# eglrp/PSBA

Hardware: AMD Instinct MI355X
Metric: M-observations/sec through Jacobian+Schur build+solve (ms/LM-iter in ms_per_step) (higher is better)
Workload: dtype f64; 1 GPU; venice-shaped; n_cams=52, n_pts=64053, n_obs=345364, lm=levmar, TR hand-off disabled, parallelism=points sharded x1

## Files before the change

### include/psba_hip.h

```cpp
#ifndef PSBA_HIP_H
#define PSBA_HIP_H

#ifdef __cplusplus
extern "C" {
#endif

typedef struct psba_ctx *psba_handle;

#define PSBA_OK 0
#define PSBA_NOT_SPD 1
#define PSBA_SINGULAR_V 2
#define PSBA_PCG_MAXIT 4
#define PSBA_E_INVALID (-1)
#define PSBA_E_HIP (-2)
#define PSBA_E_RCCL (-3)
#define PSBA_E_IO (-4)
#define PSBA_E_NOMEM (-5)
#define PSBA_E_STATE (-6)

#define PSBA_ITER_TURN_TO_LM 1
#define PSBA_ITER_TURN_TO_TR 2
#define PSBA_ITER_CONTINUE 3
#define PSBA_ITER_ERR 4
#define PSBA_ITER_DP_NO_CHANGE 5
#define PSBA_ITER_ERR_SMALL_ENOUGH 6
#define PSBA_ITER_PASS 7

#define PSBA_PARAMS_CUR 0
#define PSBA_PARAMS_NEW 1

int psba_create(int device, psba_handle *out);
int psba_destroy(psba_handle h);
const char *psba_last_error(psba_handle h);
const char *psba_version(void);

int psba_upload_problem(psba_handle h, int nCams, int n3Dpts, int n2Dprojs, const double *Kparas,
                        const double *impts, const double *initrot, const double *camsEx,
                        const double *pts3D, const int *iidx, const int *jidx);
int psba_set_params(psba_handle h, const double *camsEx, const double *pts3D);
int psba_reset_params(psba_handle h);
int psba_get_params(psba_handle h, int which, double *camsEx, double *pts3D);
int psba_get_dims(psba_handle h, int *nCams, int *n3Dpts, int *n2Dprojs);

#define PSBA_CAMERA_FIXED_K 0
#define PSBA_CAMERA_FREE_K 1
int psba_set_camera_model(psba_handle h, int model);
int psba_camera_block(psba_handle h, int *cnp);

int psba_set_distortion(psba_handle h, const double *kc);
int psba_set_obs_covariance(psba_handle h, const double *cov);
int psba_lens_model(psba_handle h, int *has_distortion, int *has_covariance);

#define PSBA_LOSS_NONE 0
#define PSBA_LOSS_HUBER 1
#define PSBA_LOSS_CAUCHY 2
#define PSBA_LOSS_SOFT_L1 3
int psba_set_robust_loss(psba_handle h, int kind, double scale);
int psba_robust_loss(psba_handle h, int *kind, double *scale);
int psba_obs_sq_residuals(psba_handle h, int which, double *s);
int psba_schur_path(psba_handle h, int *path);


int psba_residual(psba_handle h, int which, double *cost);
int psba_linearize(psba_handle h, double coeff, double coeff_g);
int psba_max_diag(psba_handle h, double *out);
int psba_begin(psba_handle h, double coeff, double coeff_g, double *cost, double *max_diag);
int psba_schur_assemble(psba_handle h, double mu);
int psba_schur_reduce(psba_handle h);
int psba_schur_solve(psba_handle h);

typedef struct {
  int status;
  double dp_l2;
  double gain_den;
  double new_cost;
  double newp_l2;
} psba_try_scalars;

int psba_backsub(psba_handle h, double mu, psba_try_scalars *out);
int psba_backsub_async(psba_handle h, double mu);
int psba_linearize_ahead(psba_handle h);
int psba_backsub_wait(psba_handle h, psba_try_scalars *out);
int psba_accept(psba_handle h);

int psba_compute_exQT(psba_handle h, int which, double *ex);
int psba_compute_jacobiQT(psba_handle h, double *jac_A, double *jac_B);
int psba_compute_U(psba_handle h, double coeff, double *out);
int psba_compute_V(psba_handle h, double coeff, double *out);
int psba_maxElmOfUV(psba_handle h, double *out);
int psba_update_UV(psba_handle h, double mu, double *U, double *V);
int psba_restore_UVdiag(psba_handle h);
int psba_compute_Vinv(psba_handle h, double *Vinv );
int psba_compute_Wblks(psba_handle h, double coeff, double *Wblks);
int psba_compute_Yblks(psba_handle h, double *Yblks);
int psba_compute_S(psba_handle h, double *S );
// ... 35 lines not shown
int psba_set_step(psba_handle h, const double *dp);
int psba_cholmod_lambda(psba_handle h, int reassemble, double *lambda, double *info3);

typedef struct {
  int max_iter;
  int start_itno;
  int verbose;
  int log_cap;
  double init_lambda;
} psba_tr_options;

typedef struct {
  int flag;
  int iters;
  int tries;
  int chol_fail;
  double init_err, final_err, lambda, delta;
  int n_log;
  double seconds;
} psba_tr_result;

void psba_tr_default_options(psba_tr_options *o);
int psba_trust_region(psba_handle h, const psba_tr_options *opts, psba_tr_result *res, double *log);

typedef struct {
  int flag, iters, lm_calls, tr_calls;
  double init_err, final_err, seconds;
} psba_solve_result;
int psba_solve(psba_handle h, int max_iter, int verbose, psba_solve_result *res);

int psba_partition_points(int n3Dpts, const int *iidx, int n2Dprojs, int nranks, int *pt_begin);
int psba_comm_unique_id(void *id128);
int psba_comm_init(psba_handle h, int nranks, int rank, const void *id128);
int psba_comm_rank(psba_handle h, int *nranks, int *rank);
int psba_set_rank_layout(psba_handle h, int nranks, int rank);
int psba_reduce_buffer_size(psba_handle h, long long *n_doubles);
int psba_get_reduce_buffer(psba_handle h, double *out);
int psba_set_reduce_buffer(psba_handle h, const double *in);

typedef struct {
  int nCams, n3Dpts, n2Dprojs;
  double *Kparas, *impts, *initrot, *camsEx, *pts3D;
  int *iidx, *jidx;
} psba_problem;
int psba_read_problem(const char *cams_file, const char *pts_file, const double *fixedK,
                      psba_problem *out);
void psba_free_problem(psba_problem *p);
typedef struct {
  psba_problem base;
  double *kc, *cov;
} psba_problem_ex;
int psba_read_problem_ex(const char *cams_file, const char *pts_file, const double *fixedK, psba_problem_ex *out);
void psba_free_problem_ex(psba_problem_ex *p);
int psba_write_problem(const char *cams_file, const char *pts_file, int nCams, int n3Dpts, int n2Dprojs,
                       const double *Kparas, const double *initrot, const double *camsEx, const double *pts3D,
                       const double *impts, const int *iidx, const int *jidx, int with_K);
int psba_convert_bal(const char *bal_file, const char *cams_out, const char *pts_out, double *max_abs_k);
int psba_convert_bal_kd(const char *bal_file, const char *cams_out, const char *pts_out);

#define PSBA_K_LINEARIZE 0
#define PSBA_K_SCHUR 1
#define PSBA_K_CHOLESKY 2
#define PSBA_K_BACKSUB 3
#define PSBA_K_RESIDUAL 4
#define PSBA_K_ALLREDUCE 5
#define PSBA_K_SCHUR_REDUCE 6
#define PSBA_K_COUNT 7
int psba_profile_enable(psba_handle h, int on);
int psba_profile_reset(psba_handle h);
int psba_profile_get(psba_handle h, int kernel, double *total_ms, int *launches);
int psba_algorithmic_bytes(psba_handle h, int kernel, double *bytes);

#define PSBA_SOLVER_DENSE 0
#define PSBA_SOLVER_PCG 1
int psba_set_solver(psba_handle h, int solver, double tol, int max_iter);
int psba_pcg_info(psba_handle h, int *iters, double *relres, long long *blocks, long long *dense_blocks);
int psba_get_sparse_S(psba_handle h, int *jk, double *val, double *ea);
int psba_set_sparse_S(psba_handle h, const double *val, const double *ea);
int psba_sparse_pattern(int nCams, int n3Dpts, int n2Dprojs, const int *iidx, const int *jidx, unsigned char *flags);
int psba_set_sparse_pattern(psba_handle h, const unsigned char *flags, long long n);

int psba_chol_dist_shape(psba_handle h, int *n32, int *NB, int *sharded);
int psba_chol_shape(psba_handle h, int *out8);
int psba_chol_dist_exchange_plan(int n32, int NB, int nranks, int JE, long long *out4, int cap);
int psba_chol_dist_begin(psba_handle h);
int psba_chol_dist_superpanel(psba_handle h, int J);
int psba_chol_dist_block(psba_handle h, int B, int set, double *buf, long long *n_doubles);
int psba_chol_dist_finish(psba_handle h);

typedef struct psba_schur_plan *psba_schur_plan_t;
psba_schur_plan_t psba_schur_plan_create(int nCams, int n3Dpts, int n2Dprojs, const int *iidx,
                                         const int *jidx);
int psba_schur_plan_info(psba_schur_plan_t p, long long info[8]);
int psba_schur_plan_copy(psba_schur_plan_t p, unsigned long long *items, long long *wg,
                         int *blockpos, int *glo);
void psba_schur_plan_destroy(psba_schur_plan_t p);

typedef struct psba_owner_plan *psba_owner_plan_t;
psba_owner_plan_t psba_owner_plan_create(int nCams, int n3Dpts, int n2Dprojs, const int *iidx, const int *jidx,
                                         const unsigned char *pattern);
int psba_owner_plan_info(psba_owner_plan_t p, long long info[4]);
int psba_owner_plan_copy(psba_owner_plan_t p, long long *waves, int *units, int *prod, int *blocks, int *diag_slot);
void psba_owner_plan_destroy(psba_owner_plan_t p);

#ifdef PSBA_BUILD_EXPERIMENTS
typedef struct psba_ring_plan *psba_ring_plan_t;
psba_ring_plan_t psba_ring_plan_create(int nCams, int n3Dpts, int n2Dprojs, const int *iidx,
                                       const int *jidx);
int psba_ring_plan_info(psba_ring_plan_t p, long long info[16]);
int psba_ring_plan_copy(psba_ring_plan_t p, long long *wg, int *steps, unsigned *entries, int *ops,
                        int *jobs, int *lane_blk, int *blk_lane0, int *rb);
void psba_ring_plan_destroy(psba_ring_plan_t p);
#endif

#ifdef __cplusplus
}
#endif
#endif
```

### psba_amd/capi.py

```python
import ctypes as C
import os

import numpy as np

_HERE = os.path.dirname(os.path.abspath(__file__))
lib_path = os.environ.get("PSBA_LIB") or os.path.join(_HERE, "libpsba_hip.so")

if not os.path.exists(lib_path):
    raise ImportError(
        f"{lib_path} is missing: build the HIP extension first (python -m psba_amd.build, or "
        "__graft_entry__.build()). psba_amd has no CPU fallback.")
lib = C.CDLL(lib_path)

PSBA_OK, PSBA_NOT_SPD, PSBA_SINGULAR_V = 0, 1, 2
PARAMS_CUR, PARAMS_NEW = 0, 1
LOSS_NONE, LOSS_HUBER, LOSS_CAUCHY, LOSS_SOFT_L1 = 0, 1, 2, 3
ITER_TURN_TO_LM, ITER_TURN_TO_TR, ITER_CONTINUE, ITER_ERR = 1, 2, 3, 4
ITER_DP_NO_CHANGE, ITER_ERR_SMALL_ENOUGH, ITER_PASS = 5, 6, 7
K_LINEARIZE, K_SCHUR, K_CHOLESKY, K_BACKSUB, K_RESIDUAL, K_ALLREDUCE, K_SCHUR_REDUCE = range(7)
KERNEL_NAMES = ["linearize", "schur", "cholesky", "backsub", "residual", "allreduce", "schur_reduce"]

_h = C.c_void_p
_dp = C.POINTER(C.c_double)
_ip = C.POINTER(C.c_int)
# ... 50 lines not shown
    ("psba_set_params", C.c_int, [_h, _dp, _dp]),
    ("psba_reset_params", C.c_int, [_h]),
    ("psba_get_params", C.c_int, [_h, C.c_int, _dp, _dp]),
    ("psba_get_dims", C.c_int, [_h, _ip, _ip, _ip]),
    ("psba_schur_path", C.c_int, [_h, C.POINTER(C.c_int)]),
    ("psba_residual", C.c_int, [_h, C.c_int, _dp]),
    ("psba_linearize", C.c_int, [_h, C.c_double, C.c_double]),
    ("psba_max_diag", C.c_int, [_h, _dp]),
    ("psba_begin", C.c_int, [_h, C.c_double, C.c_double, _dp, _dp]),
    ("psba_schur_assemble", C.c_int, [_h, C.c_double]),
    ("psba_schur_reduce", C.c_int, [_h]),
    ("psba_schur_solve", C.c_int, [_h]),
    ("psba_backsub", C.c_int, [_h, C.c_double, C.POINTER(TryScalars)]),
    ("psba_backsub_async", C.c_int, [_h, C.c_double]),
    ("psba_linearize_ahead", C.c_int, [_h]),
    ("psba_backsub_wait", C.c_int, [_h, C.POINTER(TryScalars)]),
    ("psba_accept", C.c_int, [_h]),
    ("psba_compute_exQT", C.c_int, [_h, C.c_int, _dp]),
    ("psba_compute_jacobiQT", C.c_int, [_h, _dp, _dp]),
    ("psba_compute_U", C.c_int, [_h, C.c_double, _dp]),
    ("psba_compute_V", C.c_int, [_h, C.c_double, _dp]),
    ("psba_maxElmOfUV", C.c_int, [_h, _dp]),
    ("psba_update_UV", C.c_int, [_h, C.c_double, _dp, _dp]),
    ("psba_restore_UVdiag", C.c_int, [_h]),
    ("psba_compute_Vinv", C.c_int, [_h, _dp]),
    ("psba_compute_Wblks", C.c_int, [_h, C.c_double, _dp]),
    ("psba_compute_Yblks", C.c_int, [_h, _dp]),
    ("psba_compute_S", C.c_int, [_h, _dp]),
    ("psba_compute_g", C.c_int, [_h, C.c_double, _dp]),
    ("psba_compute_ea", C.c_int, [_h, _dp]),
    ("psba_SPDinv_matVec", C.c_int, [_h, _dp]),
    ("psba_compute_eb", C.c_int, [_h, _dp]),
    ("psba_compute_dpb", C.c_int, [_h, _dp]),
    ("psba_compute_newp", C.c_int, [_h, _dp]),
    ("psba_update_p", C.c_int, [_h, _dp]),
    ("psba_lm_default_options", None, [C.POINTER(LmOptions)]),
    ("psba_levmar", C.c_int, [_h, C.POINTER(LmOptions), C.POINTER(LmResult), _dp]),
    ("psba_partition_points", C.c_int, [C.c_int, _ip, C.c_int, C.c_int, _ip]),
    ("psba_comm_unique_id", C.c_int, [C.c_void_p]),
    ("psba_comm_init", C.c_int, [_h, C.c_int, C.c_int, C.c_void_p]),
    ("psba_comm_rank", C.c_int, [_h, _ip, _ip]),
    ("psba_set_rank_layout", C.c_int, [_h, C.c_int, C.c_int]),
    ("psba_reduce_buffer_size", C.c_int, [_h, C.POINTER(C.c_longlong)]),
    ("psba_get_reduce_buffer", C.c_int, [_h, _dp]),
    ("psba_set_reduce_buffer", C.c_int, [_h, _dp]),
    ("psba_read_problem", C.c_int, [C.c_char_p, C.c_char_p, _dp, C.POINTER(CProblem)]),
    ("psba_free_problem", None, [C.POINTER(CProblem)]),
    ("psba_profile_enable", C.c_int, [_h, C.c_int]),
    ("psba_profile_reset", C.c_int, [_h]),
    ("psba_profile_get", C.c_int, [_h, C.c_int, _dp, _ip]),
    ("psba_algorithmic_bytes", C.c_int, [_h, C.c_int, _dp]),
    ("psba_compute_Jmultiply", C.c_int, [_h, _dp, _dp]),
    ("psba_jmul_dots", C.c_int, [_h, _dp, _dp, _dp]),
    ("psba_get_gradient", C.c_int, [_h, _dp]),
    ("psba_get_dp", C.c_int, [_h, _dp]),
    ("psba_set_step", C.c_int, [_h, _dp]),
    ("psba_cholmod_lambda", C.c_int, [_h, C.c_int, _dp, _dp]),
    ("psba_tr_default_options", None, [C.POINTER(TrOptions)]),
    ("psba_trust_region", C.c_int, [_h, C.POINTER(TrOptions), C.POINTER(TrResult), _dp]),
    ("psba_solve", C.c_int, [_h, C.c_int, C.c_int, C.POINTER(SolveResult)]),
    ("psba_write_problem", C.c_int, [C.c_char_p, C.c_char_p, C.c_int, C.c_int, C.c_int, _dp, _dp, _dp, _dp, _dp, _ip, _ip, C.c_int]),
    ("psba_convert_bal", C.c_int, [C.c_char_p, C.c_char_p, C.c_char_p, _dp]),
    ("psba_allreduce_scalars", C.c_int, [_h, _dp, C.c_int]),
    ("psba_set_solver", C.c_int, [_h, C.c_int, C.c_double, C.c_int]),
    ("psba_pcg_info", C.c_int, [_h, _ip, _dp, C.POINTER(C.c_longlong), C.POINTER(C.c_longlong)]),
    ("psba_get_sparse_S", C.c_int, [_h, _ip, _dp, _dp]),
    ("psba_set_sparse_S", C.c_int, [_h, _dp, _dp]),
    ("psba_sparse_pattern", C.c_int, [C.c_int, C.c_int, C.c_int, _ip, _ip, C.POINTER(C.c_ubyte)]),
    ("psba_set_sparse_pattern", C.c_int, [_h, C.POINTER(C.c_ubyte), C.c_longlong]),
    ("psba_set_camera_model", C.c_int, [_h, C.c_int]),
    ("psba_camera_block", C.c_int, [_h, _ip]),
    ("psba_set_distortion", C.c_int, [_h, _dp]),
    ("psba_set_obs_covariance", C.c_int, [_h, _dp]),
    ("psba_lens_model", C.c_int, [_h, _ip, _ip]),
    ("psba_set_robust_loss", C.c_int, [_h, C.c_int, C.c_double]),
    ("psba_robust_loss", C.c_int, [_h, _ip, _dp]),
    ("psba_obs_sq_residuals", C.c_int, [_h, C.c_int, _dp]),
    ("psba_read_problem_ex", C.c_int, [C.c_char_p, C.c_char_p, _dp, C.POINTER(CProblemEx)]),
    ("psba_free_problem_ex", None, [C.POINTER(CProblemEx)]),
    ("psba_convert_bal_kd", C.c_int, [C.c_char_p, C.c_char_p, C.c_char_p]),
    ("psba_chol_dist_exchange_plan", C.c_int, [C.c_int, C.c_int, C.c_int, C.c_int, C.POINTER(C.c_longlong), C.c_int]),
    ("psba_chol_dist_shape", C.c_int, [_h, _ip, _ip, _ip]),
    ("psba_chol_shape", C.c_int, [_h, _ip]),
    ("psba_chol_dist_begin", C.c_int, [_h]),
    ("psba_chol_dist_superpanel", C.c_int, [_h, C.c_int]),
    ("psba_chol_dist_block", C.c_int, [_h, C.c_int, C.c_int, _dp, C.POINTER(C.c_longlong)]),
    ("psba_chol_dist_finish", C.c_int, [_h]),
    ("psba_schur_plan_create", C.c_void_p, [C.c_int, C.c_int, C.c_int, _ip, _ip]),
    ("psba_schur_plan_info", C.c_int, [C.c_void_p, C.POINTER(C.c_longlong)]),
    ("psba_schur_plan_copy", C.c_int, [C.c_void_p, C.POINTER(C.c_ulonglong), C.POINTER(C.c_longlong), _ip, _ip]),
    ("psba_schur_plan_destroy", None, [C.c_void_p]),
    ("psba_owner_plan_create", C.c_void_p, [C.c_int, C.c_int, C.c_int, _ip, _ip, C.POINTER(C.c_ubyte)]),
    ("psba_owner_plan_info", C.c_int, [C.c_void_p, C.POINTER(C.c_longlong)]),
    ("psba_owner_plan_copy", C.c_int, [C.c_void_p, C.POINTER(C.c_longlong), _ip, _ip, _ip, _ip]),
    ("psba_owner_plan_destroy", None, [C.c_void_p]),
]
EXPERIMENT_SIGNATURES = [
    ("psba_ring_plan_create", C.c_void_p, [C.c_int, C.c_int, C.c_int, _ip, _ip]),
    ("psba_ring_plan_info", C.c_int, [C.c_void_p, C.POINTER(C.c_longlong)]),
    ("psba_ring_plan_copy", C.c_int, [C.c_void_p, C.POINTER(C.c_longlong), _ip, C.POINTER(C.c_uint), _ip, _ip, _ip, _ip, _ip]),
    ("psba_ring_plan_destroy", None, [C.c_void_p]),
]
HAS_EXPERIMENTS = hasattr(lib, "psba_ring_plan_create")
for _name, _res, _args in SIGNATURES + (EXPERIMENT_SIGNATURES if HAS_EXPERIMENTS else []):
    _f = getattr(lib, _name)
    _f.restype = _res
    _f.argtypes = _args


class PsbaError(RuntimeError):
    def __init__(self, code, msg):
        super().__init__(f"psba error {code}: {msg}")
        self.code = code


def _d(a):
    return None if a is None else a.ctypes.data_as(_dp)


def _i(a):
    return None if a is None else a.ctypes.data_as(_ip)


def _c(a, dt=np.float64):
    return np.ascontiguousarray(a, dtype=dt)


class Problem(dict):
    """K[nC,5] initrot[nC,4] cams[nC,6] pts[nP,3] impts[nO,2] iidx[nO] jidx[nO] nC nP nO."""


def sparse_pattern(prob):
    nC = int(prob["nC"])
    flags = np.zeros(nC * (nC + 1) // 2, dtype=np.uint8)
    ii = np.ascontiguousarray(prob["iidx"], dtype=np.int32)
    jj = np.ascontiguousarray(prob["jidx"], dtype=np.int32)
    rc = lib.psba_sparse_pattern(nC, int(prob["nP"]), int(prob["nO"]), _i(ii), _i(jj),
                                 flags.ctypes.data_as(C.POINTER(C.c_ubyte)))
    if rc != 0:
        raise PsbaError(rc, "psba_sparse_pattern failed")
    return flags


def _problem_from(cp):
    nC, nP, nO = cp.nCams, cp.n3Dpts, cp.n2Dprojs
    arr = lambda p, n, shape: np.ctypeslib.as_array(p, shape=(n,)).copy().reshape(shape)
    return Problem(K=arr(cp.Kparas, 5 * nC, (nC, 5)), initrot=arr(cp.initrot, 4 * nC, (nC, 4)),
                  cams=arr(cp.camsEx, 6 * nC, (nC, 6)), pts=arr(cp.pts3D, 3 * nP, (nP, 3)),
                  impts=arr(cp.impts, 2 * nO, (nO, 2)), iidx=arr(cp.iidx, nO, (nO,)).astype(np.int32),
                  jidx=arr(cp.jidx, nO, (nO,)).astype(np.int32), nC=nC, nP=nP, nO=nO)


def read_problem(cams_file, pts_file, fixedK=None):
    cp = CProblem()
    k = None if fixedK is None else _c(fixedK)
    rc = lib.psba_read_problem(os.fsencode(cams_file), os.fsencode(pts_file), _d(k), C.byref(cp))
    if rc != 0:
        raise PsbaError(rc, f"psba_read_problem({cams_file}, {pts_file}) failed")
    out = _problem_from(cp)
    lib.psba_free_problem(C.byref(cp))
    return out


def read_problem_ex(cams_file, pts_file, fixedK=None):
    cp = CProblemEx()
    k = None if fixedK is None else _c(fixedK)
# ... 5 lines not shown
    out["kc"] = np.ctypeslib.as_array(cp.kc, shape=(5 * nC,)).copy().reshape(nC, 5) if cp.kc else None
    out["cov"] = np.ctypeslib.as_array(cp.cov, shape=(4 * nO,)).copy().reshape(nO, 2, 2) if cp.cov else None
    lib.psba_free_problem_ex(C.byref(cp))
    return out


def write_problem(cams_file, pts_file, prob, cams=None, pts=None, with_K=True):
    c = _c(prob["cams"] if cams is None else cams)
    p = _c(prob["pts"] if pts is None else pts)
    K, rot, im = _c(prob["K"]), _c(prob["initrot"]), _c(prob["impts"])
    ii, jj = _c(prob["iidx"], np.int32), _c(prob["jidx"], np.int32)
    rc = lib.psba_write_problem(cams_file.encode(), pts_file.encode(), int(prob["nC"]), int(prob["nP"]),
                                int(prob["nO"]), _d(K), _d(rot), _d(c), _d(p), _d(im), _i(ii), _i(jj), int(with_K))
    if rc != 0:
        raise PsbaError(rc, f"psba_write_problem({cams_file}, {pts_file}) failed")


def convert_bal(bal_file, cams_out, pts_out):
    k = C.c_double()
    rc = lib.psba_convert_bal(bal_file.encode(), cams_out.encode(), pts_out.encode(), C.byref(k))
    if rc != 0:
        raise PsbaError(rc, f"psba_convert_bal({bal_file}) failed")
    return k.value


def convert_bal_kd(bal_file, cams_out, pts_out):
    rc = lib.psba_convert_bal_kd(bal_file.encode(), cams_out.encode(), pts_out.encode())
    if rc != 0:
        raise PsbaError(rc, f"psba_convert_bal_kd({bal_file}) failed")


def partition_points(n_pts, iidx, nranks):
    iidx = _c(iidx, np.int32)
    out = np.zeros(nranks + 1, dtype=np.int32)
    rc = lib.psba_partition_points(int(n_pts), _i(iidx), int(iidx.size), int(nranks), _i(out))
    if rc != 0:
        raise PsbaError(rc, "psba_partition_points failed")
    return out


def schur_plan(n_cams, n_pts, iidx, jidx):
    iidx = _c(iidx, np.int32)
    jidx = _c(jidx, np.int32)
    p = lib.psba_schur_plan_create(int(n_cams), int(n_pts), int(iidx.size), _i(iidx), _i(jidx))
    if not p:
        raise PsbaError(-1, "psba_schur_plan_create failed")
    try:
        info = (C.c_longlong * 8)()
        lib.psba_schur_plan_info(p, info)
        groups, nwg, nslots, products, slab, nblocks, run_tasks, pair_items = (int(x) for x in info)
        items = np.zeros(nslots, dtype=np.uint64)
        wg = np.zeros((nwg, 8), dtype=np.int64)
        blockpos = np.zeros(nblocks, dtype=np.int32)
        glo = np.zeros(groups + 1, dtype=np.int32)
        lib.psba_schur_plan_copy(p, items.ctypes.data_as(C.POINTER(C.c_ulonglong)),
                                 wg.ctypes.data_as(C.POINTER(C.c_longlong)), _i(blockpos), _i(glo))
    finally:
        lib.psba_schur_plan_destroy(p)
    return dict(groups=groups, items=items, wg=wg, blockpos=blockpos, glo=glo, products=products,
                slab_doubles=slab, run_tasks=run_tasks, pair_items=pair_items)


def owner_plan(n_cams, n_pts, iidx, jidx, pattern=None):
    iidx = _c(iidx, np.int32)
    jidx = _c(jidx, np.int32)
    pat = None if pattern is None else np.ascontiguousarray(pattern, dtype=np.uint8)
    pp = None if pat is None else pat.ctypes.data_as(C.POINTER(C.c_ubyte))
    p = lib.psba_owner_plan_create(int(n_cams), int(n_pts), int(iidx.size), _i(iidx), _i(jidx), pp)
    if not p:
        raise PsbaError(-1, "psba_owner_plan_create failed")
    try:
        info = (C.c_longlong * 4)()
        lib.psba_owner_plan_info(p, info)
        nw, rows, products, nblk = (int(x) for x in info)
        waves = np.zeros((nw, 2), dtype=np.int64)
        units = np.zeros((64 * nw, 4), dtype=np.int32)
        prod = np.zeros((64 * rows, 2), dtype=np.int32)
        blocks = np.zeros((nblk, 2), dtype=np.int32)
        diag = np.zeros(int(n_cams), dtype=np.int32)
        lib.psba_owner_plan_copy(p, waves.ctypes.data_as(C.POINTER(C.c_longlong)), _i(units), _i(prod), _i(blocks), _i(diag))
    finally:
        lib.psba_owner_plan_destroy(p)
    return dict(waves=waves, units=units, prod=prod.reshape(rows, 64, 2), blocks=blocks, diag_slot=diag, products=products)


def chol_dist_exchange_plan(n32, NB, nranks, JE):
    out = np.zeros((64, 4), dtype=np.int64)
    n = lib.psba_chol_dist_exchange_plan(int(n32), int(NB), int(nranks), int(JE), out.ctypes.data_as(C.POINTER(C.c_longlong)), 64)
    if n < 0:
        raise PsbaError(n, "psba_chol_dist_exchange_plan failed")
    return [tuple(int(v) for v in row) for row in out[:n]]


def ring_plan(n_cams, n_pts, iidx, jidx):
    if not HAS_EXPERIMENTS:
        raise PsbaError(-6, "the ring route is an experiment: build with PSBA_BUILD_EXPERIMENTS=1")
    iidx = _c(iidx, np.int32)
    jidx = _c(jidx, np.int32)
    p = lib.psba_ring_plan_create(int(n_cams), int(n_pts), int(iidx.size), _i(iidx), _i(jidx))
    if not p:
        raise PsbaError(-1, "psba_ring_plan_create failed")
    try:
        info = (C.c_longlong * 16)()
        lib.psba_ring_plan_info(p, info)
        (nR, nS, nwg, nsteps, nent, nops, njob, products, slots, lanes, pages, yslots, lat, nlb, nbl0, loaded) = (int(x) for x in info)
        if nwg == 0:
            return None
        wg = np.zeros((nwg, 13), dtype=np.int64)
        steps = np.zeros((nsteps, 4), dtype=np.int32)
        entries = np.zeros(nent, dtype=np.uint32)
        ops = np.zeros((nops, 2), dtype=np.int32)
        jobs = np.zeros((njob, 4), dtype=np.int32)
        lane_blk = np.zeros(nlb, dtype=np.int32)
        blk_lane0 = np.zeros(nbl0, dtype=np.int32)
        rb = np.zeros(nR + 1, dtype=np.int32)
        lib.psba_ring_plan_copy(p, wg.ctypes.data_as(C.POINTER(C.c_longlong)), _i(steps),
                                entries.ctypes.data_as(C.POINTER(C.c_uint)), _i(ops), _i(jobs), _i(lane_blk),
                                _i(blk_lane0), _i(rb))
    finally:
        lib.psba_ring_plan_destroy(p)
    return dict(nR=nR, nS=nS, wg=wg, steps=steps, entries=entries, ops=ops, jobs=jobs, lane_blk=lane_blk,
                blk_lane0=blk_lane0, rb=rb, products=products, lane_steps=slots, lanes=lanes, slots=pages,
                page=yslots, lat=lat, loaded_recs=loaded)


def shard_problem(prob, nranks, rank):
    bounds = partition_points(prob["nP"], prob["iidx"], nranks)
    p0, p1 = int(bounds[rank]), int(bounds[rank + 1])
    iidx = np.asarray(prob["iidx"])
    sel = (iidx >= p0) & (iidx < p1)
    out = Problem(K=prob["K"], initrot=prob["initrot"], cams=prob["cams"], pts=prob["pts"][p0:p1],
                  impts=np.asarray(prob["impts"])[sel], iidx=(iidx[sel] - p0).astype(np.int32),
                  jidx=np.asarray(prob["jidx"])[sel].astype(np.int32), nC=prob["nC"], nP=p1 - p0,
                  nO=int(sel.sum()))
    if "kc" in prob:
        out["kc"] = prob["kc"]
    if "cov" in prob:
        out["cov"] = None if prob["cov"] is None else np.asarray(prob["cov"])[sel]
    return out


class Psba:

    def __init__(self, device=0):
        self._h = _h()
        rc = lib.psba_create(int(device), C.byref(self._h))
        if rc != 0:
            raise PsbaError(rc, lib.psba_last_error(None).decode())
        self.nC = self.nP = self.nO = 0

    def close(self):
        if self._h:
            lib.psba_destroy(self._h)
            self._h = _h()

    def __del__(self):
        try:
            self.close()
        except Exception:
            pass

    def _ck(self, rc):
        if rc < 0:
            raise PsbaError(rc, lib.psba_last_error(self._h).decode())
        return rc

# ... 134 lines not shown
        U, V = np.empty(36 * self.nC), np.empty(9 * self.nP)
        self._ck(lib.psba_update_UV(self._h, mu, _d(U), _d(V)))
        return U, V

    def restore_UVdiag(self):
        self._ck(lib.psba_restore_UVdiag(self._h))

    def compute_Vinv(self):
        return self._out(lib.psba_compute_Vinv, 9 * self.nP)

    def compute_Wblks(self, coeff=1.0):
        return self._out(lib.psba_compute_Wblks, 18 * self.nO, coeff)[1]

    def compute_Yblks(self):
        return self._out(lib.psba_compute_Yblks, 18 * self.nO)[1]

    def compute_S(self):
        return self._out(lib.psba_compute_S, self.nA * self.nA)[1].reshape(self.nA, self.nA)

    def compute_g(self, coeff=1.0):
        return self._out(lib.psba_compute_g, self.nT, coeff)[1]

    def compute_ea(self):
        return self._out(lib.psba_compute_ea, self.nA)[1]

    def SPDinv_matVec(self):
        return self._out(lib.psba_SPDinv_matVec, self.nA)

    def compute_eb(self):
        return self._out(lib.psba_compute_eb, self.nB)[1]

    def compute_dpb(self):
        return self._out(lib.psba_compute_dpb, self.nT)[1]

    def compute_newp(self):
        return self._out(lib.psba_compute_newp, self.nT)[1]

    def update_p(self):
        return self._out(lib.psba_update_p, self.nT)[1]

    def levmar(self, max_iter=50, tr_handoff=False, verbose=False, log_cap=512, start_itno=0, init_mu=0.0):
        opts = LmOptions(max_iter, int(tr_handoff), int(verbose), log_cap, start_itno, init_mu)
        res = LmResult()
        log = np.zeros((max(log_cap, 1), 5))
        self._ck(lib.psba_levmar(self._h, C.byref(opts), C.byref(res), _d(log)))
        return res, log[: res.n_log].copy()

    def set_solver(self, solver, tol=0.0, max_iter=0):
        self._ck(lib.psba_set_solver(self._h, int(solver), float(tol), int(max_iter)))

    def pcg_info(self):
        it, rr, nb, nd = C.c_int(), C.c_double(), C.c_longlong(), C.c_longlong()
        self._ck(lib.psba_pcg_info(self._h, C.byref(it), C.byref(rr), C.byref(nb), C.byref(nd)))
        return it.value, rr.value, nb.value, nd.value

    def get_sparse_S(self):
        nb = self.pcg_info()[2]
        jk = np.empty((nb, 2), dtype=np.int32)
        val = np.empty((nb, 6, 6))
        ea = np.empty(6 * self.nC)
        self._ck(lib.psba_get_sparse_S(self._h, _i(jk), _d(val), _d(ea)))
        return jk, val, ea

    def set_sparse_S(self, val, ea):
        val = np.ascontiguousarray(val, dtype=np.float64)
        ea = np.ascontiguousarray(ea, dtype=np.float64)
        self._ck(lib.psba_set_sparse_S(self._h, _d(val), _d(ea)))

    def set_sparse_pattern(self, flags):
        flags = np.ascontiguousarray(flags, dtype=np.uint8)
        self._ck(lib.psba_set_sparse_pattern(self._h, flags.ctypes.data_as(C.POINTER(C.c_ubyte)), flags.size))

    def chol_dist_shape(self):
        n32, nb, sh = C.c_int(), C.c_int(), C.c_int()
        self._ck(lib.psba_chol_dist_shape(self._h, C.byref(n32), C.byref(nb), C.byref(sh)))
        return n32.value, nb.value, bool(sh.value)

    def chol_shape(self):
        out = (C.c_int * 8)()
        self._ck(lib.psba_chol_shape(self._h, out))
        keys = ("n32", "fused", "fused2", "blocked", "NB", "diag_only", "lookahead", "single")
        return {k: (int(v) if k in ("n32", "NB") else bool(v)) for k, v in zip(keys, out)}

    def chol_dist_begin(self):
        self._ck(lib.psba_chol_dist_begin(self._h))

    def chol_dist_superpanel(self, J):
        self._ck(lib.psba_chol_dist_superpanel(self._h, int(J)))

    def chol_dist_get_block(self, B):
        n = C.c_longlong()
        self._ck(lib.psba_chol_dist_block(self._h, int(B), 0, None, C.byref(n)))
        buf = np.empty(n.value)
        self._ck(lib.psba_chol_dist_block(self._h, int(B), 0, _d(buf), C.byref(n)))
        return buf

    def chol_dist_set_block(self, B, buf):
        n = C.c_longlong()
        self._ck(lib.psba_chol_dist_block(self._h, int(B), 1, _d(_c(buf)), C.byref(n)))

    def chol_dist_finish(self):
        self._ck(lib.psba_chol_dist_finish(self._h))

    def compute_Jmultiply(self, x):
        return self._out(lambda h, out: lib.psba_compute_Jmultiply(h, _d(_c(x)), out), 2 * self.nO)[1]

    def jmul_dots(self, x1, x2=None):
        out = np.empty(3)
        a1 = _c(x1)
        a2 = None if x2 is None else _c(x2)
        self._ck(lib.psba_jmul_dots(self._h, _d(a1), _d(a2), _d(out)))
        return out

    def get_gradient(self):
        return self._out(lib.psba_get_gradient, self.nT)[1]

    def get_dp(self):
        return self._out(lib.psba_get_dp, self.nT)[1]

    def set_step(self, dp):
        self._ck(lib.psba_set_step(self._h, _d(_c(dp))))

    def cholmod_lambda(self, reassemble=True):
        lam, info = C.c_double(), np.empty(3)
        self._ck(lib.psba_cholmod_lambda(self._h, int(reassemble), C.byref(lam), _d(info)))
        return lam.value, info

    def trust_region(self, max_iter=50, start_itno=0, verbose=False, log_cap=512, init_lambda=0.0):
        opts = TrOptions(max_iter, start_itno, int(verbose), log_cap, init_lambda)
        res = TrResult()
        log = np.zeros((max(log_cap, 1), 6))
        self._ck(lib.psba_trust_region(self._h, C.byref(opts), C.byref(res), _d(log)))
        return res, log[: res.n_log].copy()

    def solve(self, max_iter=50, verbose=False):
        res = SolveResult()
        self._ck(lib.psba_solve(self._h, max_iter, int(verbose), C.byref(res)))
        return res

    @staticmethod
    def comm_unique_id():
        buf = C.create_string_buffer(128)
        rc = lib.psba_comm_unique_id(buf)
        if rc != 0:
            raise PsbaError(rc, "psba_comm_unique_id failed")
        return buf.raw

    def comm_init(self, nranks, rank, uid):
        buf = C.create_string_buffer(uid, 128)
        self._ck(lib.psba_comm_init(self._h, nranks, rank, buf))

    def set_rank_layout(self, nranks, rank):
        self._ck(lib.psba_set_rank_layout(self._h, nranks, rank))

    def reduce_buffer_size(self):
        n = C.c_longlong()
        self._ck(lib.psba_reduce_buffer_size(self._h, C.byref(n)))
        return n.value

    def get_reduce_buffer(self):
        out = np.empty(self.reduce_buffer_size())
        self._ck(lib.psba_get_reduce_buffer(self._h, _d(out)))
        return out

    def set_reduce_buffer(self, buf):
        b = _c(buf).reshape(-1)
# ... 19 lines not shown
```

### psba_amd/csrc/kernels_backsub.hip

```cpp
#include <cstdlib>

#include "camera_model.h"
#include "psba_internal.h"

namespace psba {

struct BackArgs {
  const double *W, *PV, *camconst, *cams, *pts, *impts, *ga;
  const int *iidx, *jidx, *ptr;
  const int4 *tile_desc;
  double *dp;
  double *newcams, *newpts;
  double *scal;
  double *dbg_eb;
  const int *status;
  double mu;
  double coeff;
  int nC, nA, nTiles;
  int cam_terms;
  int mode;
  const double *kc, *wl;
};

template <bool DUMP, bool RECOMP, int LM>
__global__ __launch_bounds__(TILE_OBS) void k_backsub(BackArgs p, RobustLoss rl) {
  __shared__ double sT[TILE_OBS][3];
  __shared__ double sNP[TILE_OBS][3];
  __shared__ double sRed[4][4];
  const int tid = threadIdx.x;
  double s_dp = 0.0, s_den = 0.0, s_cost = 0.0, s_np = 0.0;

  if (blockIdx.x == 0) {
    if (tid == 0) {
      p.scal[SC_STATUS_V] = (p.status[0] == p.status[3]) ? 1.0 : 0.0;
      p.scal[SC_STATUS_SPD] = (p.status[1] == p.status[3]) ? 1.0 : 0.0;
    }
    for (int t = tid; t < p.nA; t += TILE_OBS) {
      const double d = p.dp[t], c = p.cams[t] + d;
      p.newcams[t] = c;
      s_den += d * p.ga[t];
      if (p.cam_terms) {
        s_dp += d * d;
        s_den += p.mu * d * d;
        s_np += c * c;
      }
    }
  }

  int tile = blockIdx.x;
  int4 dsc = tile < p.nTiles ? p.tile_desc[tile] : make_int4(0, 0, 0, 0);
  int i = 0, j = 0;
  if (dsc.z + tid < dsc.w) {
    i = p.iidx[dsc.z + tid];
    j = p.jidx[dsc.z + tid];
  }
  for (; tile < p.nTiles; tile += gridDim.x) {
    const int p0 = dsc.x, p1 = dsc.y, o0 = dsc.z, o1 = dsc.w;
    const int a = o0 + tid;
    const int tn = tile + gridDim.x;
    const int4 dn = tn < p.nTiles ? p.tile_desc[tn] : make_int4(0, 0, 0, 0);
    int pb0 = 0, pb1 = 0;
    if (p0 + tid < p1) {
      pb0 = p.ptr[p0 + tid] - o0;
      pb1 = p.ptr[p0 + tid + 1] - o0;
    }
    __syncthreads();
    double cc[9], cam[6], da[6], kc[5], wl[3];
    constexpr bool MEAS = RECOMP && (LM & LENS_ROBUST) != 0;
    double2 m = make_double2(0.0, 0.0);
    if (RECOMP && a < o1) {
#pragma unroll
      for (int k = 0; k < 9; k++) cc[k] = p.camconst[9 * j + k];
      lens_load_kc<LM>(p.kc, j, kc);
      lens_load_w<LM>(p.wl, a, wl);
      if (MEAS) m = reinterpret_cast<const double2 *>(p.impts)[a];
#pragma unroll
      for (int k = 0; k < 6; k++) {
        cam[k] = p.cams[6 * j + k];
        da[k] = p.dp[6 * j + k];
      }
    }
    if (a < o1 && p.mode != 2) {
      double t0 = 0.0, t1 = 0.0, t2 = 0.0;
      if (RECOMP) {
        double M[3], e[2], A[12], B[6];
#pragma unroll
        for (int k = 0; k < 3; k++) M[k] = p.pts[3 * (size_t)i + k];
        lens_linearize<LM>(cc, cam, M, kc, wl, rl, m.x, m.y, e, A, B);
        double s0 = 0.0, s1 = 0.0;
#pragma unroll
        for (int k = 0; k < 6; k++) {
          s0 += A[k] * da[k];
          s1 += A[6 + k] * da[k];
        }
        t0 = p.coeff * (B[0] * s0 + B[3] * s1);
        t1 = p.coeff * (B[1] * s0 + B[4] * s1);
        t2 = p.coeff * (B[2] * s0 + B[5] * s1);
      } else {
        const double *w = p.W + 18 * (size_t)a;
        const double *dw = p.dp + 6 * j;
#pragma unroll
        for (int k = 0; k < 6; k++) {
          const double dk = dw[k];
          t0 += w[3 * k] * dk;
          t1 += w[3 * k + 1] * dk;
          t2 += w[3 * k + 2] * dk;
        }
      }
      sT[tid][0] = t0;
      sT[tid][1] = t1;
      sT[tid][2] = t2;
    }
    __syncthreads();
    if (p0 + tid < p1) {
      const int ip = p0 + tid;
      const double *pv = p.PV + 9 * (size_t)ip;
      const int b0 = pb0, b1 = pb1;
      const double g0 = pv[6], g1 = pv[7], g2 = pv[8];
// ... 247 lines not shown
```

### psba_amd/csrc/kernels_chol_graph.hip

```cpp
#include <cstdlib>

#include "chol_factor32.h"
#include "psba_internal.h"

namespace psba {

template <class Arr>
__device__ __forceinline__ void stage_block32(Arr &dst, const double *src, size_t rs, int tid) {
  const int r = tid / GB, c = tid % GB;
  double v[4];
#pragma unroll
  for (int q = 0; q < 4; q++) v[q] = src[(size_t)(r + 8 * q) * rs + c];
#pragma unroll
  for (int q = 0; q < 4; q++) dst[r + 8 * q][c] = v[q];
}

__global__ __launch_bounds__(256) void k_cholg_diag(const double *Lw, double *Lx, int ld, int j, double *linv,
                                                    int *status, long long *tim) {
  __shared__ Factor32Lds s;
  const int tid = threadIdx.x;
  if (tid < 4) s.flag[tid] = 0;
  if (tid == 4) s.fail = 0;
  if (tim && tid == 0) tim[0] = (long long)__builtin_amdgcn_s_memtime();
  stage_block32(s.D, Lw + (size_t)j * ld + j, (size_t)ld, tid);
  __syncthreads();
  if (tim && tid == 0) tim[1] = (long long)__builtin_amdgcn_s_memtime();
  if (tim)
    factor32<true>(s, tid, tim);
  else
    factor32<false>(s, tid);
  if (tim && tid == 0) tim[2] = (long long)__builtin_amdgcn_s_memtime();
  double *li = linv + (size_t)(j / GB) * GB * GB;
  for (int t = tid; t < GB * GB; t += 256) {
    const int r = t / GB, c = t % GB;
    Lx[(size_t)(j + r) * ld + j + c] = f32_L(s, r, c);
    li[t] = f32_Linv(s, r, c);
  }
  if (tid == 0 && s.fail) status[1] = status[3];
  if (tim && tid == 0) tim[15] = (long long)__builtin_amdgcn_s_memtime();
}

__device__ __forceinline__ void trsm_tile(const double *Lw, int ld, int j, int T, int nT, const double *Li,
                                          int li, int lk, d4 &xl, d4 &xr) {
  const double4 *b0p = reinterpret_cast<const double4 *>(Li + (size_t)li * GB + 8 * lk);
  const double4 *b1p = reinterpret_cast<const double4 *>(Li + (size_t)(16 + li) * GB + 8 * lk);
  const double4 p0 = b0p[0], p1 = b0p[1], q0 = b1p[0], q1 = b1p[1];
  double4 a0, a1;
  const int e = T - nT;
  if (e >= j / 16) {
    const int k1 = 16 * (e - j / 16) + li - 8 * lk;
    a0 = make_double4(k1 == 0, k1 == 1, k1 == 2, k1 == 3);
    a1 = make_double4(k1 == 4, k1 == 5, k1 == 6, k1 == 7);
  } else {
    const double4 *ap = reinterpret_cast<const double4 *>(Lw + (size_t)(16 * T + li) * ld + j + 8 * lk);
    a0 = ap[0];
    a1 = ap[1];
  }
  d4 x0 = {0, 0, 0, 0}, x1 = {0, 0, 0, 0}, y0 = {0, 0, 0, 0}, y1 = {0, 0, 0, 0};
  x0 = __builtin_amdgcn_mfma_f64_16x16x4f64(a0.x, p0.x, x0, 0, 0, 0);
  y0 = __builtin_amdgcn_mfma_f64_16x16x4f64(a0.x, q0.x, y0, 0, 0, 0);
  x1 = __builtin_amdgcn_mfma_f64_16x16x4f64(a0.y, p0.y, x1, 0, 0, 0);
  y1 = __builtin_amdgcn_mfma_f64_16x16x4f64(a0.y, q0.y, y1, 0, 0, 0);
  x0 = __builtin_amdgcn_mfma_f64_16x16x4f64(a0.z, p0.z, x0, 0, 0, 0);
  y0 = __builtin_amdgcn_mfma_f64_16x16x4f64(a0.z, q0.z, y0, 0, 0, 0);
  x1 = __builtin_amdgcn_mfma_f64_16x16x4f64(a0.w, p0.w, x1, 0, 0, 0);
  y1 = __builtin_amdgcn_mfma_f64_16x16x4f64(a0.w, q0.w, y1, 0, 0, 0);
  x0 = __builtin_amdgcn_mfma_f64_16x16x4f64(a1.x, p1.x, x0, 0, 0, 0);
  y0 = __builtin_amdgcn_mfma_f64_16x16x4f64(a1.x, q1.x, y0, 0, 0, 0);
  x1 = __builtin_amdgcn_mfma_f64_16x16x4f64(a1.y, p1.y, x1, 0, 0, 0);
  y1 = __builtin_amdgcn_mfma_f64_16x16x4f64(a1.y, q1.y, y1, 0, 0, 0);
  x0 = __builtin_amdgcn_mfma_f64_16x16x4f64(a1.z, p1.z, x0, 0, 0, 0);
  y0 = __builtin_amdgcn_mfma_f64_16x16x4f64(a1.z, q1.z, y0, 0, 0, 0);
  x1 = __builtin_amdgcn_mfma_f64_16x16x4f64(a1.w, p1.w, x1, 0, 0, 0);
  y1 = __builtin_amdgcn_mfma_f64_16x16x4f64(a1.w, q1.w, y1, 0, 0, 0);
  xl = x0 + x1;
  xr = y0 + y1;
}

__device__ __forceinline__ void store_x_tile(double *Lx, int ld, int j, int T, int li, int lk, const d4 &xl,
                                             const d4 &xr) {
#pragma unroll
  for (int r = 0; r < 4; r++) {
    Lx[(size_t)(16 * T + lk + 4 * r) * ld + j + li] = xl[r];
    Lx[(size_t)(16 * T + lk + 4 * r) * ld + j + 16 + li] = xr[r];
  }
}

__global__ __launch_bounds__(256) void k_cholg_trsm(const double *Lw, double *Lx, int ld, int j, int nT,
                                                    int nTall, const double *linv) {
  const int lane = threadIdx.x & 63, wave = threadIdx.x >> 6;
  const int li = lane & 15, lk = lane >> 4;
  const int T = (j + GB) / 16 + blockIdx.x * 4 + wave;
  if (T >= nTall) return;
  d4 xl, xr;
  trsm_tile(Lw, ld, j, T, nT, linv + (size_t)(j / GB) * GB * GB, li, lk, xl, xr);
  store_x_tile(Lx, ld, j, T, li, lk, xl, xr);
}

struct Row8 {
  double v[8];
};
__device__ __forceinline__ Row8 load_row8(const double *p) {
  const double4 a = reinterpret_cast<const double4 *>(p)[0], b = reinterpret_cast<const double4 *>(p)[1];
  return {{a.x, a.y, a.z, a.w, b.x, b.y, b.z, b.w}};
}
__device__ __forceinline__ d4 update_mfma(d4 c0, const Row8 &a, const Row8 &b) {
  d4 c1 = {0, 0, 0, 0};
#pragma unroll
  for (int t = 0; t < 8; t += 2) {
    c0 = __builtin_amdgcn_mfma_f64_16x16x4f64(-a.v[t], b.v[t], c0, 0, 0, 0);
    c1 = __builtin_amdgcn_mfma_f64_16x16x4f64(-a.v[t + 1], b.v[t + 1], c1, 0, 0, 0);
  }
  return c0 + c1;
}
__device__ __forceinline__ d4 load_c_tile(const double *Lw, int ld, int TR, int TC, int li, int lk) {
  d4 c;
#pragma unroll
  for (int r = 0; r < 4; r++) c[r] = Lw[(size_t)(16 * TR + lk + 4 * r) * ld + 16 * TC + li];
  return c;
}
__device__ __forceinline__ void store_c_tile(double *Lw, int ld, int TR, int TC, int li, int lk, const d4 &c) {
#pragma unroll
  for (int r = 0; r < 4; r++) Lw[(size_t)(16 * TR + lk + 4 * r) * ld + 16 * TC + li] = c[r];
}
__device__ __forceinline__ bool tile_of_index(long long idx, int T0, int nT, int nId, int &TR, int &TC,
                                              bool &fresh) {
  const long long M = (nT - 1) - T0;
  const long long ntri = M * (M + 1) / 2;
  fresh = false;
  if (idx >= ntri + M + nId * M) return false;
  if (idx < ntri) {
    int m = (int)((sqrt(8.0 * (double)idx + 1.0) - 1.0) * 0.5);
    while ((long long)(m + 1) * (m + 2) / 2 <= idx) m++;
    while ((long long)m * (m + 1) / 2 > idx) m--;
    TR = T0 + m;
    TC = T0 + (int)(idx - (long long)m * (m + 1) / 2);
  } else if (idx < ntri + M) {
    TR = nT - 1;
    TC = T0 + (int)(idx - ntri);
  } else {
    const long long k = idx - ntri - M;
    const int e = (int)(k / M);
    TR = nT + e;
    TC = T0 + (int)(k % M);
    fresh = e >= T0 - 2;
  }
  return true;
}

__device__ __forceinline__ d4 update_tile(const double *Lw, const double *Lx, int ld, int j, int TR, int TC,
                                          int li, int lk) {
  const Row8 a = load_row8(Lx + (size_t)(16 * TR + li) * ld + j + 8 * lk);
  const Row8 b = load_row8(Lx + (size_t)(16 * TC + li) * ld + j + 8 * lk);
  return update_mfma(load_c_tile(Lw, ld, TR, TC, li, lk), a, b);
}

__device__ __forceinline__ void factor_next_block(Factor32Lds &s, double *Lx, int ld, int jn, double *linv,
                                            int *status, int tid, bool store_L = true) {
  factor32(s, tid);
  double *lio = linv + (size_t)(jn / GB) * GB * GB;
  for (int t = tid; t < GB * GB; t += 256) {
    const int r = t / GB, c = t % GB;
    if (store_L) Lx[(size_t)(jn + r) * ld + jn + c] = f32_L(s, r, c);
    lio[t] = f32_Linv(s, r, c);
  }
  if (tid == 0 && s.fail) status[1] = status[3];
}

__global__ __launch_bounds__(256) void k_cholg_update(double *Lw, double *Lx, int ld, int j, int nT,
                                                      double *linv, int *status) {
  __shared__ Factor32Lds s;
  const int tid = threadIdx.x, lane = tid & 63, wave = tid >> 6;
  const int li = lane & 15, lk = lane >> 4;
  const int T0 = (j + GB) / 16;
  if (blockIdx.x == 0) {
    if (tid < 4) s.flag[tid] = 0;
    if (tid == 4) s.fail = 0;
    if (wave < 3) {
      const int TR = T0 + (wave > 0), TC = T0 + (wave > 1);
      const d4 c = update_tile(Lw, Lx, ld, j, TR, TC, li, lk);
#pragma unroll
      for (int r = 0; r < 4; r++) s.D[16 * (TR - T0) + lk + 4 * r][16 * (TC - T0) + li] = c[r];
    }
    __syncthreads();
    factor_next_block(s, Lx, ld, j + GB, linv, status, tid);
    return;
  }
  int TR, TC;
  bool fresh;
  if (!tile_of_index((long long)(blockIdx.x - 1) * 4 + wave + 3, T0, nT, 0, TR, TC, fresh)) return;
  store_c_tile(Lw, ld, TR, TC, li, lk, update_tile(Lw, Lx, ld, j, TR, TC, li, lk));
}


__device__ __forceinline__ d4 update_tile_k(const double *Lw, const double *Lx, int ld, int J, int KW, int TR,
                                            int TC, int li, int lk) {
  d4 c = load_c_tile(Lw, ld, TR, TC, li, lk);
  for (int kk = 0; kk < KW; kk += GB) {
    const Row8 a = load_row8(Lx + (size_t)(16 * TR + li) * ld + J + kk + 8 * lk);
    const Row8 b = load_row8(Lx + (size_t)(16 * TC + li) * ld + J + kk + 8 * lk);
    c = update_mfma(c, a, b);
  }
  return c;
}

__global__ __launch_bounds__(256) void k_cholg_update_cols(double *Lw, double *Lx, int ld, int j, int nT, int TE,
                                                           double *linv, int *status) {
  __shared__ Factor32Lds s;
  const int tid = threadIdx.x, lane = tid & 63, wave = tid >> 6;
  const int li = lane & 15, lk = lane >> 4;
  const int T0 = (j + GB) / 16;
  if (blockIdx.x == 0) {
    if (tid < 4) s.flag[tid] = 0;
    if (tid == 4) s.fail = 0;
    if (wave < 3) {
      const int TR = T0 + (wave > 0), TC = T0 + (wave > 1);
      const d4 c = update_tile(Lw, Lx, ld, j, TR, TC, li, lk);
#pragma unroll
      for (int r = 0; r < 4; r++) s.D[16 * (TR - T0) + lk + 4 * r][16 * (TC - T0) + li] = c[r];
    }
    __syncthreads();
    factor_next_block(s, Lx, ld, j + GB, linv, status, tid);
    return;
  }
  long long idx = (long long)(blockIdx.x - 1) * 4 + wave;
  int TC = T0;
  while (TC < TE && idx >= nT - TC) {
    idx -= nT - TC;
    TC++;
  }
  if (TC >= TE) return;
  const int TR = TC + (int)idx;
  if (TR <= T0 + 1 && TC <= T0 + 1) return;
  store_c_tile(Lw, ld, TR, TC, li, lk, update_tile(Lw, Lx, ld, j, TR, TC, li, lk));
}

__global__ __launch_bounds__(256) void k_cholg_update_wide(double *Lw, double *Lx, int ld, int J, int KW, int nT,
                                                           int Tw, double *linv, int *status, int ncolb) {
  __shared__ Factor32Lds s;
  const int tid = threadIdx.x, lane = tid & 63, wave = tid >> 6;
  const int li = lane & 15, lk = lane >> 4;
  if (blockIdx.x == 0) {
    if (tid < 4) s.flag[tid] = 0;
    if (tid == 4) s.fail = 0;
    if (wave < 3) {
      const int TR = Tw + (wave > 0), TC = Tw + (wave > 1);
      const d4 c = update_tile_k(Lw, Lx, ld, J, KW, TR, TC, li, lk);
// ... 101 lines not shown
  }
  WIDE4_FENCE();
  d4 c[4][4];
#pragma unroll
  for (int a = 0; a < 4; a++)
#pragma unroll
    for (int b = 0; b < 4; b++)
      if (on[a][b]) c[a][b] = load_c_tile(Lw, ld, TR0 + a, TC0 + b, li, lk);
  WIDE4_FENCE();
  WIDE4_MFMAS(a1, b1);
#undef WIDE4_FENCE
#undef WIDE4_MFMAS
#undef WIDE4_MFMAS_FIRST
#undef WIDE4_LOAD
#pragma unroll
  for (int a = 0; a < 4; a++)
#pragma unroll
    for (int b = 0; b < 4; b++)
      if (on[a][b]) store_c_tile(Lw, ld, TR0 + a, TC0 + b, li, lk, c[a][b] - acc[a][b]);
}

__global__ __launch_bounds__(256) void k_cholg_update_wide4(double *Lw, double *Lx, int ld, int J, int KW, int nT,
                                                            int Tw, double *linv, int *status, int nranks, int rank,
                                                            int part, int ncolb) {
  __shared__ Factor32Lds s;
  const int tid = threadIdx.x, lane = tid & 63;
  const int wave = __builtin_amdgcn_readfirstlane(tid >> 6);
  const int li = lane & 15, lk = lane >> 4;
  if (blockIdx.x == 0) {
    if (nranks > 0 || part == 2) return;
    if (tid < 4) s.flag[tid] = 0;
    if (tid == 4) s.fail = 0;
    if (wave < 3) {
      const int TR = Tw + (wave > 0), TC = Tw + (wave > 1);
      const d4 c = update_tile_k(Lw, Lx, ld, J, KW, TR, TC, li, lk);
#pragma unroll
      for (int r = 0; r < 4; r++) s.D[16 * (TR - Tw) + lk + 4 * r][16 * (TC - Tw) + li] = c[r];
    }
    __syncthreads();
    factor_next_block(s, Lx, ld, 16 * Tw, linv, status, tid);
    return;
  }
  const int nTl = nT - 1 - Tw;
  const long long MR = (nTl + 3) / 4;
  const long long ntri = part == 1 ? MR * ncolb : MR * (MR + 1) / 2;
  const long long idx = (long long)(blockIdx.x - 1) * 4 + wave;
  if (idx >= ntri) {
    const long long e = idx - ntri;
    if (e >= nTl || (part == 1 && e >= 4 * ncolb)) return;
    if (nranks > 0 && (Tw + (int)e) / 4 % nranks != rank) return;
    const int TC = Tw + (int)e;
    store_c_tile(Lw, ld, nT - 1, TC, li, lk, update_tile_k(Lw, Lx, ld, J, KW, nT - 1, TC, li, lk));
    return;
  }
  int m, mc;
  if (part == 1) {
    m = __builtin_amdgcn_readfirstlane((int)(idx / ncolb));
    mc = __builtin_amdgcn_readfirstlane((int)(idx % ncolb));
    if (mc > m) return;
  } else {
    const long long nfull = MR * (MR - 1) / 2;
    if (idx < nfull) {
      m = (int)((sqrt(8.0 * (double)idx + 1.0) - 1.0) * 0.5);
      while ((long long)(m + 1) * (m + 2) / 2 <= idx) m++;
      while ((long long)m * (m + 1) / 2 > idx) m--;
      mc = __builtin_amdgcn_readfirstlane((int)(idx - (long long)m * (m + 1) / 2));
      m = __builtin_amdgcn_readfirstlane(m + 1);
    } else {
      m = mc = __builtin_amdgcn_readfirstlane((int)(idx - nfull));
    }
  }

  if (nranks > 0 && (Tw / 4 + mc) % nranks != rank) return;
  const int TR0 = Tw + 4 * m, TC0 = Tw + 4 * mc;
  const int last = nT - 2;
  const int Tx = (nranks > 0 || part == 2) ? -4 : Tw;
  if (mc < m && TR0 + 3 <= last && (m > 0))
    wide4_block<true>(Lw, Lx, ld, J, KW, Tx, last, TR0, TC0, li, lk);
  else
    wide4_block<false>(Lw, Lx, ld, J, KW, Tx, last, TR0, TC0, li, lk);
}

constexpr int XS = 34;
__global__ __launch_bounds__(256) void k_cholg_panel(double *Lw, double *Lx, int ld, int j, int nT, int nId, int TE,
                                                     double *linv, int *status, int factor_next) {
  __shared__ Factor32Lds s;
  __shared__ double sX[4][2][16][XS];
  const int tid = threadIdx.x, lane = tid & 63, wave = tid >> 6;
  const int li = lane & 15, lk = lane >> 4;
  const int T0 = (j + GB) / 16;
  const double *Li = linv + (size_t)(j / GB) * GB * GB;
  if (blockIdx.x == 0) {
    if (tid < 4) s.flag[tid] = 0;
    if (tid == 4) s.fail = 0;
    const int tr = (wave > 0), tc = (wave > 1);
    d4 c = {0, 0, 0, 0};
    if (wave < 3) c = load_c_tile(Lw, ld, T0 + tr, T0 + tc, li, lk);
    {
      const int xr = wave >> 1, half = wave & 1;
      const Row8 a = load_row8(Lw + (size_t)(16 * (T0 + xr) + li) * ld + j + 8 * lk);
      const Row8 b = load_row8(Li + (size_t)(16 * half + li) * GB + 8 * lk);
      d4 x0 = {0, 0, 0, 0}, x1 = {0, 0, 0, 0};
#pragma unroll
      for (int t = 0; t < 8; t += 2) {
        x0 = __builtin_amdgcn_mfma_f64_16x16x4f64(a.v[t], b.v[t], x0, 0, 0, 0);
        x1 = __builtin_amdgcn_mfma_f64_16x16x4f64(a.v[t + 1], b.v[t + 1], x1, 0, 0, 0);
      }
      const d4 x = x0 + x1;
#pragma unroll
      for (int r = 0; r < 4; r++) {
        sX[0][xr][lk + 4 * r][16 * half + li] = x[r];
        if (nId == 0) Lx[(size_t)(16 * (T0 + xr) + lk + 4 * r) * ld + j + 16 * half + li] = x[r];
      }
    }
    __syncthreads();
    if (wave < 3) {
      const Row8 a = load_row8(&sX[0][tr][li][8 * lk]), b = load_row8(&sX[0][tc][li][8 * lk]);
      c = update_mfma(c, a, b);
      if (!factor_next) {
        store_c_tile(Lw, ld, T0 + tr, T0 + tc, li, lk, c);
      } else {
#pragma unroll
        for (int r = 0; r < 4; r++) s.D[16 * tr + lk + 4 * r][16 * tc + li] = c[r];
      }
    }
    if (!factor_next) return;
    __syncthreads();
    factor_next_block(s, Lx, ld, j + GB, linv, status, tid, nId == 0);
    return;
  }
  int TR, TC;
  bool fresh = false;
  if (TE >= 0) {
    long long idx = (long long)(blockIdx.x - 1) * 4 + wave;
    TC = T0;
    while (TC < TE && idx >= nT - TC) {
      idx -= nT - TC;
      TC++;
    }
    if (TC >= TE) return;
    TR = TC + (int)idx;
    if (TR <= T0 + 1 && TC <= T0 + 1) return;
  } else if (!tile_of_index((long long)(blockIdx.x - 1) * 4 + wave + 3, T0, nT, nId, TR, TC, fresh)) {
    return;
  }
  d4 c = {0, 0, 0, 0};
  if (!fresh) c = load_c_tile(Lw, ld, TR, TC, li, lk);
  d4 xl, xr;
  trsm_tile(Lw, ld, j, TR, nT, Li, li, lk, xl, xr);
  if (TC == T0 && (nId == 0 || TR >= nT - 1)) store_x_tile(Lx, ld, j, TR, li, lk, xl, xr);
#pragma unroll
  for (int r = 0; r < 4; r++) {
    sX[wave][0][lk + 4 * r][li] = xl[r];
    sX[wave][0][lk + 4 * r][16 + li] = xr[r];
  }
  if (TC != TR) {
    trsm_tile(Lw, ld, j, TC, nT, Li, li, lk, xl, xr);
#pragma unroll
    for (int r = 0; r < 4; r++) {
      sX[wave][1][lk + 4 * r][li] = xl[r];
      sX[wave][1][lk + 4 * r][16 + li] = xr[r];
    }
  }
  const Row8 a = load_row8(&sX[wave][0][li][8 * lk]);
  const Row8 b = load_row8(&sX[wave][TC != TR][li][8 * lk]);
  store_c_tile(Lw, ld, TR, TC, li, lk, update_mfma(c, a, b));
}

template <int NBK>
__global__ __launch_bounds__(256) void k_cholg_trsm_block(const double *Lw, double *Lx, int ld, int J, int T_first,
                                                          int nTall, const double *linv) {
  __shared__ double sX[4][16][XS];
  const int lane = threadIdx.x & 63, wave = threadIdx.x >> 6;
  const int li = lane & 15, lk = lane >> 4;
  const int T = T_first + blockIdx.x * 4 + wave;
  if (T >= nTall) return;
  Row8 X[NBK];
#pragma unroll
  for (int k = 0; k < NBK; k++) {
    const int j = J + GB * k;
    d4 cl, cr;
#pragma unroll
    for (int r = 0; r < 4; r++) {
      cl[r] = Lw[(size_t)(16 * T + lk + 4 * r) * ld + j + li];
      cr[r] = Lw[(size_t)(16 * T + lk + 4 * r) * ld + j + 16 + li];
    }
#pragma unroll
    for (int k2 = 0; k2 < k; k2++) {
      const double *Lkk = Lx + (size_t)j * ld + J + GB * k2;
      const Row8 b0 = load_row8(Lkk + (size_t)li * ld + 8 * lk), b1 = load_row8(Lkk + (size_t)(16 + li) * ld + 8 * lk);
      cl = update_mfma(cl, X[k2], b0);
      cr = update_mfma(cr, X[k2], b1);
    }
#pragma unroll
    for (int r = 0; r < 4; r++) {
      sX[wave][lk + 4 * r][li] = cl[r];
      sX[wave][lk + 4 * r][16 + li] = cr[r];
    }
    const Row8 a = load_row8(&sX[wave][li][8 * lk]);
    const double *Li = linv + (size_t)(j / GB) * GB * GB;
    const Row8 p = load_row8(Li + (size_t)li * GB + 8 * lk), q = load_row8(Li + (size_t)(16 + li) * GB + 8 * lk);
    d4 x0 = {0, 0, 0, 0}, x1 = {0, 0, 0, 0}, y0 = {0, 0, 0, 0}, y1 = {0, 0, 0, 0};
#pragma unroll
    for (int t = 0; t < 8; t += 2) {
      x0 = __builtin_amdgcn_mfma_f64_16x16x4f64(a.v[t], p.v[t], x0, 0, 0, 0);
      y0 = __builtin_amdgcn_mfma_f64_16x16x4f64(a.v[t], q.v[t], y0, 0, 0, 0);
      x1 = __builtin_amdgcn_mfma_f64_16x16x4f64(a.v[t + 1], p.v[t + 1], x1, 0, 0, 0);
      y1 = __builtin_amdgcn_mfma_f64_16x16x4f64(a.v[t + 1], q.v[t + 1], y1, 0, 0, 0);
    }
    const d4 xl = x0 + x1, xr = y0 + y1;
    store_x_tile(Lx, ld, j, T, li, lk, xl, xr);
#pragma unroll
    for (int r = 0; r < 4; r++) {
      sX[wave][lk + 4 * r][li] = xl[r];
      sX[wave][lk + 4 * r][16 + li] = xr[r];
    }
    X[k] = load_row8(&sX[wave][li][8 * lk]);
  }
}

template <int NBK>
__global__ __launch_bounds__(256, NBK <= 12 ? 2 : 1) void k_cholg_trsm_block4(const double *Lw, double *Lx, int ld, int J, int T_first,
                                                           int nTall, const double *linv) {
  __shared__ double sA[4][16][XS];
  __shared__ double sX[2][16][XS];
  const int lane = threadIdx.x & 63;
  const int wave = __builtin_amdgcn_readfirstlane(threadIdx.x >> 6);
  const int li = lane & 15, lk = lane >> 4;
  const int T = T_first + blockIdx.x;
  if (T >= nTall) return;
  constexpr int NQ = (NBK + 3) / 4;
  d4 cl[NQ], cr[NQ];
#pragma unroll
  for (int q = 0; q < NQ; q++) {
    const int k = 4 * q + wave, j = J + GB * k;
    if (k < NBK) {
#pragma unroll
      for (int r = 0; r < 4; r++) {
        cl[q][r] = Lw[(size_t)(16 * T + lk + 4 * r) * ld + j + li];
        cr[q][r] = Lw[(size_t)(16 * T + lk + 4 * r) * ld + j + 16 + li];
      }
    }
  }
  auto finish = [&](int q, int k, const Row8 &p, const Row8 &q8) {
    const int j = J + GB * k;
#pragma unroll
    for (int r = 0; r < 4; r++) {
      sA[wave][lk + 4 * r][li] = cl[q][r];
      sA[wave][lk + 4 * r][16 + li] = cr[q][r];
// ... 153 lines not shown
__global__ __launch_bounds__(256) void k_cholg_back_multi(double *Lw , int ld, int n, int n32,
                                                          int j0, int nb, double *x, const double *linv, int *status) {
  __shared__ double sLi[BACK_NB][GB][GB + 1];
  __shared__ double sL[BACK_NB * (BACK_NB - 1) / 2][GB][GB + 1];
  __shared__ double sY[BACK_NB * GB], sX[BACK_NB * GB], sQ[8][GB], sQ2[2][128];
  const int tid = threadIdx.x;
  double *y = Lw + (size_t)n32 * ld;
  double vLi[BACK_NB][4], vL[BACK_NB * (BACK_NB - 1) / 2][4];
  const int tr = tid / GB, tc = tid % GB;
#pragma unroll
  for (int b = 0; b < BACK_NB; b++) {
    const double *Li = linv + (size_t)(j0 / GB + (b < nb ? b : 0)) * GB * GB;
#pragma unroll
    for (int q = 0; q < 4; q++) vLi[b][q] = Li[tid + 256 * q];
#pragma unroll
    for (int bp = 0; bp < b; bp++) {
      const double *L = Lw + (size_t)(j0 + (b < nb ? b : 0) * GB) * ld + j0 + bp * GB;
#pragma unroll
      for (int q = 0; q < 4; q++) vL[b * (b - 1) / 2 + bp][q] = L[(size_t)(tr + 8 * q) * ld + tc];
    }
  }
  const double vy = tid < nb * GB ? y[j0 + tid] : 0.0;
  __shared__ double sP[BACK_NB][64];
  const int w = tid >> 6, lane = tid & 63;
  const int c = blockIdx.x * 64 + lane;
  const bool mine = c < j0 && w < nb;
  const double *L = Lw + (size_t)(j0 + w * GB) * ld + (mine ? c : 0);
  double pre[GB];
#pragma unroll
  for (int r = 0; r < GB; r++) pre[r] = mine ? L[(size_t)r * ld] : 0.0;
  if (tid < nb * GB) sY[tid] = vy;
#pragma unroll
  for (int b = 0; b < BACK_NB; b++) {
#pragma unroll
    for (int q = 0; q < 4; q++) sLi[b][tr + 8 * q][tc] = vLi[b][q];
#pragma unroll
    for (int bp = 0; bp < b; bp++)
#pragma unroll
      for (int q = 0; q < 4; q++) sL[b * (b - 1) / 2 + bp][tr + 8 * q][tc] = vL[b * (b - 1) / 2 + bp][q];
  }
  __syncthreads();
  for (int b = nb - 1; b >= 0; b--) {
    {
      const int cc = tid & 31, pp = tid >> 5;
      const double q0 = sLi[b][4 * pp][cc] * sY[b * GB + 4 * pp], q1 = sLi[b][4 * pp + 1][cc] * sY[b * GB + 4 * pp + 1];
      const double q2 = sLi[b][4 * pp + 2][cc] * sY[b * GB + 4 * pp + 2], q3 = sLi[b][4 * pp + 3][cc] * sY[b * GB + 4 * pp + 3];
      sQ[pp][cc] = (q0 + q1) + (q2 + q3);
    }
    __syncthreads();
    if (tid < GB) {
      const double v = ((sQ[0][tid] + sQ[1][tid]) + (sQ[2][tid] + sQ[3][tid])) + ((sQ[4][tid] + sQ[5][tid]) + (sQ[6][tid] + sQ[7][tid]));
      sX[b * GB + tid] = v;
      if (blockIdx.x == 0) {
        if (j0 + b * GB + tid < n) x[j0 + b * GB + tid] = v;
        if (!isfinite(v)) status[1] = status[3];
      }
    }
    __syncthreads();
    {
      const int o = tid & 127, half = tid >> 7;
      if (o < b * GB) {
        const int bp = o / GB, cc = o % GB;
        double a4[4] = {0.0, 0.0, 0.0, 0.0};
#pragma unroll
        for (int r = 0; r < GB / 2; r++)
          a4[r & 3] += sL[b * (b - 1) / 2 + bp][GB / 2 * half + r][cc] * sX[b * GB + GB / 2 * half + r];
        sQ2[half][o] = (a4[0] + a4[1]) + (a4[2] + a4[3]);
      }
    }
    __syncthreads();
    if (tid < b * GB) sY[tid] -= sQ2[0][tid] + sQ2[1][tid];
    __syncthreads();
  }
  double a4[4] = {0.0, 0.0, 0.0, 0.0};
#pragma unroll
  for (int r = 0; r < GB; r++) a4[r & 3] += pre[r] * sX[(w < nb ? w : 0) * GB + r];
  sP[w][lane] = mine ? (a4[0] + a4[1]) + (a4[2] + a4[3]) : 0.0;
  __syncthreads();
  if (w == 0 && c < j0) y[c] -= (sP[0][lane] + sP[1][lane]) + (sP[2][lane] + sP[3][lane]);
}

template <int NZ>
__global__ __launch_bounds__(256) void k_cholg_solve(const double *Lw, const double *Lx, int ld, int n, int n32,
                                                    double *x, const double *linv, int *status) {
  __shared__ double sLi[GB][GB + 1], sV[GB], sW[GB];
  const int tid = threadIdx.x, lane = tid & 63, i = blockIdx.x * 4 + (tid >> 6);
  const int jl = n32 - GB;
  const double *Li = linv + (size_t)(jl / GB) * GB * GB;
  stage_block32(sLi, Li, GB, tid);
  const double rk = tid < GB ? Lw[(size_t)n32 * ld + jl + tid] : 0.0;
  const bool row = i < n;
  const double *y = Lx + (size_t)n32 * ld;
  const double *z = Lx + (size_t)(n32 + 16 + (row ? i : 0)) * ld;
  double zv[NZ], yv[NZ];
#pragma unroll
  for (int m = 0; m < NZ; m++) {
    const int c = lane + 64 * m;
    const bool on = row && c < jl && c >= (i & ~15);
    zv[m] = on ? z[c] : 0.0;
    yv[m] = on ? y[c] : 0.0;
  }
  double rt = 0.0;
  if (row && lane < GB) rt = i >= jl ? (double)(lane == i - jl) : Lw[(size_t)(n32 + 16 + i) * ld + jl + lane];
  if (tid < GB) sV[tid] = rk;
  __syncthreads();
  double v = 0.0;
  if (tid < GB) {
    double a4[4] = {0.0, 0.0, 0.0, 0.0};
#pragma unroll
    for (int k = 0; k < GB; k++) a4[k & 3] += sLi[tid][k] * sV[k];
    v = (a4[0] + a4[1]) + (a4[2] + a4[3]);
  }
  __syncthreads();
  if (tid < GB) sV[tid] = v;
  __syncthreads();
  if (tid < GB) {
    double a4[4] = {0.0, 0.0, 0.0, 0.0};
#pragma unroll
    for (int c = 0; c < GB; c++) a4[c & 3] += sLi[c][tid] * sV[c];
    sW[tid] = (a4[0] + a4[1]) + (a4[2] + a4[3]);
  }
  __syncthreads();
  if (!row) return;
  double acc = lane < GB ? rt * sW[lane] : 0.0;
#pragma unroll
  for (int m = 0; m < NZ; m++) acc += zv[m] * yv[m];
#pragma unroll
  for (int off = 32; off > 0; off >>= 1) acc += __shfl_xor(acc, off, 64);
  if (lane == 0) {
    x[i] = acc;
    if (!isfinite(acc)) status[1] = status[3];
  }
}

#ifdef PSBA_BUILD_EXPERIMENTS
constexpr int TAIL_MAX = 4;
struct TailLds {
  Factor32Lds s;
  double B[TAIL_MAX * (TAIL_MAX + 1) / 2][GB][GB + 1];
  double Li[TAIL_MAX][GB][GB + 1];
  double r[TAIL_MAX * GB], q[16][GB];
};
__device__ __forceinline__ int tail_idx(int r, int c) { return r * (r + 1) / 2 + c; }

__device__ __forceinline__ d4 tail_abt(const double (*A)[GB + 1], const double (*M)[GB + 1], int ti, int tj, int li, int lk) {
  d4 c0 = {0, 0, 0, 0}, c1 = {0, 0, 0, 0};
#pragma unroll
  for (int t = 0; t < 8; t += 2) {
    c0 = __builtin_amdgcn_mfma_f64_16x16x4f64(A[16 * ti + li][4 * t + lk], M[16 * tj + li][4 * t + lk], c0, 0, 0, 0);
    c1 = __builtin_amdgcn_mfma_f64_16x16x4f64(A[16 * ti + li][4 * t + 4 + lk], M[16 * tj + li][4 * t + 4 + lk], c1, 0, 0, 0);
  }
  return c0 + c1;
}

template <bool TRANS>
__device__ __forceinline__ double tail_matvec(const double (*M)[GB + 1], const double *v, int lane) {
  const int r = lane & 31, h = lane >> 5;
  double a4[4] = {0.0, 0.0, 0.0, 0.0};
#pragma unroll
  for (int k = 0; k < 16; k++) a4[k & 3] += (TRANS ? M[16 * h + k][r] : M[r][16 * h + k]) * v[16 * h + k];
  const double a = (a4[0] + a4[1]) + (a4[2] + a4[3]);
  return a + __shfl_xor(a, 32, 64);
}

struct TailBackground {
  TailLds *t;
  int b, nt, lane;
  __device__ __forceinline__ void operator()(int w) const {
    if (b < 0) return;
// ... 237 lines not shown
    const dim3 g((nT - JE / 16 + 3) / 4), b(256);
    if (nbk == 4) hipLaunchKernelGGL(k_cholg_trsm_block<4>, g, b, 0, s, Lw, Lx, ld, J, JE / 16, nT, linv);
    if (nbk == 8) hipLaunchKernelGGL(k_cholg_trsm_block<8>, g, b, 0, s, Lw, Lx, ld, J, JE / 16, nT, linv);
    if (nbk == 12) hipLaunchKernelGGL(k_cholg_trsm_block<12>, g, b, 0, s, Lw, Lx, ld, J, JE / 16, nT, linv);
    if (nbk == 16) hipLaunchKernelGGL(k_cholg_trsm_block<16>, g, b, 0, s, Lw, Lx, ld, J, JE / 16, nT, linv);
  }
  if (JE < n32) {
    const int Tw = JE / 16;
    if ((getenv("PSBA_CHOL_WIDE2") || (JE - J) % (2 * GB)) && nranks == 0) {
      const long long MR = (nT - 1 - Tw) / 2;
      const long long work = MR * (MR + 1) / 2 - 1 + (nT - 1 - Tw);
      hipLaunchKernelGGL(k_cholg_update_wide, dim3(1 + (unsigned)((work + 3) / 4)), dim3(256), 0, s, Lw, Lx, ld, J,
                         JE - J, nT, Tw, linv, h->status, 0);
    } else if (look) {
      const int ncolb = NB / 64;
      const long long MR = (nT - 1 - Tw + 3) / 4;
      (void)hipEventRecord(ev_steps, s);
      if (ev_far_prev) (void)hipStreamWaitEvent(s, ev_far_prev, 0);
      const long long nnear = MR * ncolb + (4 * ncolb < nT - 1 - Tw ? 4 * ncolb : nT - 1 - Tw);
      const long long MRh = (nT - 1 - Tw) / 2, nnear2 = MRh * (2 * ncolb) - 1 + (4 * ncolb < nT - 1 - Tw ? 4 * ncolb : nT - 1 - Tw);
      long long fine_max = 1000;
      if (const char *e = getenv("PSBA_CHOL_NEAR_FINE_MAX")) fine_max = atoll(e);
      if (nnear2 <= fine_max)
        hipLaunchKernelGGL(k_cholg_update_wide, dim3(1 + (unsigned)((nnear2 + 3) / 4)), dim3(256), 0, s, Lw, Lx, ld, J, JE - J,
                           nT, Tw, linv, h->status, 2 * ncolb);
      else
      hipLaunchKernelGGL(k_cholg_update_wide4, dim3(1 + (unsigned)((nnear + 3) / 4)), dim3(256), 0, s, Lw, Lx, ld, J, JE - J,
                         nT, Tw, linv, h->status, 0, 0, 1, ncolb);
      (void)hipStreamWaitEvent(side, ev_steps, 0);
      const int pause_ticks = getenv("PSBA_CHOL_FAR_PAUSE") ? atoi(getenv("PSBA_CHOL_FAR_PAUSE")) : 300;
      if (pause_ticks > 0 && ev_far_prev) hipLaunchKernelGGL(k_cholg_pause, dim3(1), dim3(64), 0, side, (long long)pause_ticks);
      const int Tw2 = Tw + 4 * ncolb;
      if (Tw2 < nT - 1) {
        const long long MR2 = (nT - 1 - Tw2 + 3) / 4;
        const unsigned grid = 1 + (unsigned)((MR2 * (MR2 + 1) / 2 + (nT - 1 - Tw2) + 3) / 4);
        hipLaunchKernelGGL(k_cholg_update_wide4, dim3(grid), dim3(256), 0, side, Lw, Lx, ld, J, JE - J, nT, Tw2, linv,
                           h->status, 0, 0, 2, ncolb);
      }
      (void)hipEventRecord(ev_far, side);
    } else {
      const long long MR = (nT - 1 - Tw + 3) / 4;
      const unsigned grid = 1 + (unsigned)((MR * (MR + 1) / 2 + (nT - 1 - Tw) + 3) / 4);
      hipLaunchKernelGGL(k_cholg_update_wide4, dim3(grid), dim3(256), 0, s, Lw, Lx, ld, J, JE - J, nT, Tw, linv,
                         h->status, nranks, rank, 0, 0);
    }
  }
}

static void enqueue_backward(psba_ctx *h, hipStream_t s) {
  const int n32 = h->n32, ld = h->n32;
  double *Lx = h->chol_L, *linv = h->chol_ws;
  if (!getenv("PSBA_CHOL_BACK_ONE_WG")) {
    if (getenv("PSBA_CHOL_BACK_SINGLE")) {
      for (int j = n32 - GB; j >= 0; j -= GB)
        hipLaunchKernelGGL(k_cholg_back_panel, dim3(j / 256 + 1), dim3(256), 0, s, Lx, ld, h->d.nA, n32, j, h->dp,
                           linv, h->status);
    } else {
      for (int R = n32 / GB; R > 0;) {
        const int nb = R < BACK_NB ? R : BACK_NB, j0 = (R - nb) * GB;
        hipLaunchKernelGGL(k_cholg_back_multi, dim3(j0 / 64 + 1), dim3(256), 0, s, Lx, ld, h->d.nA, n32, j0, nb,
                           h->dp, linv, h->status);
        R -= nb;
      }
    }
  } else {
    int thr = (n32 + 63) / 64 * 64;
    if (thr > 512) thr = 512;
    hipLaunchKernelGGL(k_cholg_backward, dim3(1), dim3(thr), 0, s, Lx, ld, h->d.nA, n32, h->dp, linv, h->status);
  }
}

__global__ __launch_bounds__(256) void k_cholg_cols(double *Lw, int ld, int row0, int nrows, int col0, int ncols, double *buf,
                                                    int set) {
  const long long t = (long long)blockIdx.x * 256 + threadIdx.x;
  if (t >= (long long)nrows * ncols) return;
  const int r = (int)(t / ncols), cc = (int)(t % ncols);
  double *at = Lw + (size_t)(row0 + r) * ld + col0 + cc;
  if (set)
    *at = buf[t];
  else
    buf[t] = *at;
}

static void enqueue_chain(psba_ctx *h, hipStream_t s, bool skip_diag) {
  const int n32 = h->n32, ld = h->n32, nT = n32 / 16 + 1;
  double *Lw = h->red, *Lx = h->chol_L, *linv = h->chol_ws;
  const ChainShape c = chain_shape(h);
  const bool fused = c.fused, blocked = c.blocked, fused2 = c.fused2;
  int tail = 0;
#ifdef PSBA_BUILD_EXPERIMENTS
  if (const char *e = getenv("PSBA_CHOL_TAIL")) tail = fused && atoi(e) >= 0 && atoi(e) <= TAIL_MAX && atoi(e) <= n32 / GB ? atoi(e) : 0;
#endif
  const int jl = n32 - GB * tail;
  if (!skip_diag && !(tail > 0 && jl == 0))
    hipLaunchKernelGGL(k_cholg_diag, dim3(1), dim3(256), 0, s, Lw, Lx, ld, 0, linv, h->status, h->chol_tim);
  bool look = chain_lookahead(c);
  if (look) {
    if (!h->chol_side) {
      int least = 0, greatest = 0;
      (void)hipDeviceGetStreamPriorityRange(&least, &greatest);
      if (hipStreamCreateWithPriority(&h->chol_side, hipStreamNonBlocking, getenv("PSBA_CHOL_SIDE_PRIO_DEFAULT") ? 0 : least) != hipSuccess)
        look = false;
    }
    const size_t need = 2 * (size_t)(n32 / c.NB + 2);
    while (look && h->chol_events.size() < need) {
      hipEvent_t e;
      const unsigned flags = getenv("PSBA_CHOL_EVENT_SYSFENCE") ? hipEventDisableTiming : hipEventDisableTiming | hipEventReleaseToDevice;
      if (hipEventCreateWithFlags(&e, flags) != hipSuccess) {
        look = false;
        break;
      }
      h->chol_events.push_back(e);
    }
  }
  {
    hipEvent_t far_prev = nullptr;
    int k = 0;
    for (int J = 0; blocked && J < n32; J += c.NB, k++) {
      if (!look) {
        enqueue_superpanel(h, s, c, J, 0, 0);
        continue;
      }
      const bool has_update = J + c.NB < n32;
      enqueue_superpanel(h, s, c, J, 0, 0, true, h->chol_side, h->chol_events[2 * k], far_prev, h->chol_events[2 * k + 1]);
      if (has_update) far_prev = h->chol_events[2 * k + 1];
    }
    if (far_prev) (void)hipStreamWaitEvent(s, far_prev, 0);
  }
  for (int j = 0; !blocked && j < n32; j += GB) {
    const bool last = j + GB >= n32;
    const int T0 = (j + GB) / 16;
    const long long M = (nT - 1) - T0;
    if (tail > 0 && j >= jl) break;
    if (last && fused) break;
    if (last || !(fused || fused2)) {
      const int nTall = nT;
      hipLaunchKernelGGL(k_cholg_trsm, dim3((nTall - T0 + 3) / 4), dim3(256), 0, s, Lw, Lx, ld, j, nT, nTall, linv);
      if (!last) {
        const int grid = 1 + (int)((M * (M + 1) / 2 + M - 3 + 3) / 4);
        hipLaunchKernelGGL(k_cholg_update, dim3(grid), dim3(256), 0, s, Lw, Lx, ld, j, nT, linv, h->status);
      }
    } else {
      const int nId = fused ? T0 : 0;
      const int grid = 1 + (int)((M * (M + 1) / 2 + M + (long long)nId * M - 3 + 3) / 4);
      hipLaunchKernelGGL(k_cholg_panel, dim3(grid), dim3(256), 0, s, Lw, Lx, ld, j, nT, nId, -1, linv, h->status,
                         tail > 0 && j + GB >= jl ? 0 : 1);
    }
  }
#ifdef PSBA_BUILD_EXPERIMENTS
  if (fused && tail > 0) {
    const size_t lds = sizeof(TailLds);
    static bool attr_set = false;
    if (!attr_set) {
      (void)hipFuncSetAttribute((const void *)k_cholg_tail<10>, hipFuncAttributeMaxDynamicSharedMemorySize, (int)lds);
      (void)hipFuncSetAttribute((const void *)k_cholg_tail<16>, hipFuncAttributeMaxDynamicSharedMemorySize, (int)lds);
      attr_set = true;
    }
    if (n32 <= 640)
      hipLaunchKernelGGL(k_cholg_tail<10>, dim3((h->d.nA + 7) / 8), dim3(512), lds, s, Lw, Lx, ld, h->d.nA, n32, tail, h->dp,
                         h->status, h->chol_tim);
    else
      hipLaunchKernelGGL(k_cholg_tail<16>, dim3((h->d.nA + 7) / 8), dim3(512), lds, s, Lw, Lx, ld, h->d.nA, n32, tail, h->dp,
                         h->status, h->chol_tim);
  } else
#endif
  if (fused) {
    if (n32 <= 640)
      hipLaunchKernelGGL(k_cholg_solve<10>, dim3((h->d.nA + 3) / 4), dim3(256), 0, s, Lw, Lx, ld, h->d.nA, n32, h->dp,
                         linv, h->status);
    else
      hipLaunchKernelGGL(k_cholg_solve<16>, dim3((h->d.nA + 3) / 4), dim3(256), 0, s, Lw, Lx, ld, h->d.nA, n32, h->dp,
                         linv, h->status);
  } else {
    enqueue_backward(h, s);
  }
}

int chol_dist_shape(psba_ctx *h, int *NB, int *blocked) {
  const ChainShape c = chain_shape(h);
  *NB = c.NB;
  *blocked = c.blocked && c.NB % 64 == 0;
  return PSBA_OK;
}

int chol_shape(psba_ctx *h, int *out) {
  const ChainShape c = chain_shape(h);
  const int n32 = h->n32;
  out[0] = n32;
  out[1] = c.fused;
  out[2] = c.fused2;
  out[3] = c.blocked;
  out[4] = c.NB;
  out[5] = c.blocked && steps_diag_only(n32, 0, c.NB < n32 ? c.NB : n32);
  out[6] = chain_lookahead(c);
  out[7] = getenv("PSBA_CHOL_SINGLE") != nullptr;
  return PSBA_OK;
}

int chol_dist_begin(psba_ctx *h) {
  if (!h->diag_done)
    hipLaunchKernelGGL(k_cholg_diag, dim3(1), dim3(256), 0, h->stream, h->red, h->chol_L, h->n32, 0, h->chol_ws, h->status,
                       h->chol_tim);
  h->diag_done = false;
  PSBA_HIP(h, hipGetLastError());
  return PSBA_OK;
}

int chol_dist_superpanel(psba_ctx *h, int J) {
  const ChainShape c = chain_shape(h);
  if (J > 0)
    hipLaunchKernelGGL(k_cholg_diag, dim3(1), dim3(256), 0, h->stream, h->red, h->chol_L, h->n32, J, h->chol_ws, h->status,
                       h->chol_tim);
  enqueue_superpanel(h, h->stream, c, J, h->nranks, h->rank);
  PSBA_HIP(h, hipGetLastError());
  return PSBA_OK;
}

int chol_dist_block(psba_ctx *h, int B, double *buf_dev, int set) {
  const int row0 = 64 * B, nrows = h->n32 + 1 - row0, ncols = h->n32 - row0 < 64 ? h->n32 - row0 : 64;
  const long long n = (long long)nrows * ncols;
  hipLaunchKernelGGL(k_cholg_cols, dim3((unsigned)((n + 255) / 256)), dim3(256), 0, h->stream, h->red, h->n32, row0, nrows,
                     64 * B, ncols, buf_dev, set);
  PSBA_HIP(h, hipGetLastError());
  return PSBA_OK;
}

int chol_dist_finish(psba_ctx *h) {
  enqueue_backward(h, h->stream);
  PSBA_HIP(h, hipGetLastError());
  return PSBA_OK;
}

int chol_dist_exchange_plan(int n32, int NB, int nranks, int JE, long long (*out)[4], int cap) {
  if (JE >= n32 || NB <= 0 || nranks <= 0) return 0;
  const int B0 = JE / 64, B1 = ((JE + NB < n32 ? JE + NB : n32) + 63) / 64;
  int k = 0;
  for (int B = B0; B < B1; B++, k++) {
    if (k >= cap) return -1;
    const long long cols = n32 - 64 * B < 64 ? n32 - 64 * B : 64;
    out[k][0] = B;
    out[k][1] = B % nranks;
    out[k][2] = B - B0;
    out[k][3] = (long long)(n32 + 1 - 64 * B) * cols;
  }
  return k;
}

static int chol_dist_comm(psba_ctx *h) {
  const ChainShape c = chain_shape(h);
  const int n32 = h->n32;
  const size_t per = (size_t)(n32 + 1) * 64;
  if (!h->dist_buf) {
    if (hipMalloc((void **)&h->dist_buf, sizeof(double) * per * (size_t)(c.NB / 64 + 1)) != hipSuccess)
      return fail(h, PSBA_E_HIP, "no memory for the column exchange buffers");
  }
  int rc = chol_dist_begin(h);
  for (int J = 0; J < n32 && rc == PSBA_OK; J += c.NB) {
    rc = chol_dist_superpanel(h, J);
    const int JE = J + c.NB;
    if (JE >= n32 || rc != PSBA_OK) break;
    long long plan[64][4];
    const int nb = chol_dist_exchange_plan(n32, c.NB, h->nranks, JE, plan, 64);
    if (nb < 0 || nb > c.NB / 64 + 1) return fail(h, PSBA_E_INVALID, "column exchange: %d blocks for a super-panel of %d columns", nb, c.NB);
    for (int k = 0; k < nb && rc == PSBA_OK; k++)
      if (plan[k][1] == h->rank) rc = chol_dist_block(h, (int)plan[k][0], h->dist_buf + (size_t)plan[k][2] * per, 0);
    if (ncclGroupStart() != ncclSuccess) return fail(h, PSBA_E_RCCL, "ncclGroupStart failed");
    bool sent = true;
    for (int k = 0; k < nb && sent; k++) {
      double *b = h->dist_buf + (size_t)plan[k][2] * per;
      sent = ncclBroadcast(b, b, (size_t)plan[k][3], ncclDouble, (int)plan[k][1], h->comm, h->stream) == ncclSuccess;
    }
    if (ncclGroupEnd() != ncclSuccess || !sent)
      return fail(h, PSBA_E_RCCL, "ncclBroadcast failed in the column exchange");
    for (int k = 0; k < nb && rc == PSBA_OK; k++)
      if (plan[k][1] != h->rank) rc = chol_dist_block(h, (int)plan[k][0], h->dist_buf + (size_t)plan[k][2] * per, 1);
  }
  if (rc == PSBA_OK) rc = chol_dist_finish(h);
  return rc;
}

int launch_chol_graph(psba_ctx *h) {
  if (h->comm && (h->nranks > 1 || getenv("PSBA_CHOL_DIST_FORCE")) && !getenv("PSBA_CHOL_REPLICATED")) {
    int NB, blocked;
    chol_dist_shape(h, &NB, &blocked);
    if (blocked) {
      ProfScope ps(h, PSBA_K_CHOLESKY);
      return chol_dist_comm(h);
    }
  }
  const int v = h->diag_done ? 1 : 0;
  h->diag_done = false;
  if (h->n32 > 2048 || !getenv("PSBA_CHOL_GRAPH") || getenv("PSBA_CHOL_NO_GRAPH")) {
    ProfScope ps(h, PSBA_K_CHOLESKY);
    enqueue_chain(h, h->stream, v == 1);
    PSBA_HIP(h, hipGetLastError());
    return PSBA_OK;
  }
  if (!h->chol_graph[v] || h->chol_graph_n32[v] != h->n32 || h->chol_graph_red[v] != h->red) {
    if (h->chol_graph[v]) {
      (void)hipGraphExecDestroy(h->chol_graph[v]);
      h->chol_graph[v] = nullptr;
    }
    hipGraph_t g = nullptr;
    PSBA_HIP(h, hipStreamBeginCapture(h->stream, hipStreamCaptureModeThreadLocal));
    enqueue_chain(h, h->stream, v == 1);
    PSBA_HIP(h, hipStreamEndCapture(h->stream, &g));
    hipError_t e = hipGraphInstantiate(&h->chol_graph[v], g, nullptr, nullptr, 0);
    (void)hipGraphDestroy(g);
    if (e != hipSuccess) {
      h->chol_graph[v] = nullptr;
      return fail(h, PSBA_E_HIP, "hipGraphInstantiate failed: %s", hipGetErrorString(e));
    }
    h->chol_graph_n32[v] = h->n32;
    h->chol_graph_red[v] = h->red;
  }
  {
    ProfScope ps(h, PSBA_K_CHOLESKY);
    PSBA_HIP(h, hipGraphLaunch(h->chol_graph[v], h->stream));
  }
  return PSBA_OK;
}

}
```

### psba_amd/csrc/kernels_freek.hip

```cpp
#include "camera_model.h"
#include "psba_internal.h"
#include "schur_common.h"

namespace psba {

constexpr int FK_W = 3 * FK_CNP;
constexpr int FK_ACC = FK_CNP * (FK_CNP + 1) / 2 + FK_CNP;

struct FkArgs {
  const double *camconst, *cams, *pts, *impts;
  const int *iidx, *jidx, *ptr;
  double *W, *PV, *camacc;
  double coeff;
  int nO;
  const double *pub_src;
  double *pub_dst;
  double pub_stamp;
};

__device__ __forceinline__ void fk_load(const FkArgs &p, int a, int &i, int &j, double *cam, double *q0, double *M, double2 &m) {
  i = p.iidx[a];
  j = p.jidx[a];
#pragma unroll
  for (int k = 0; k < FK_CNP; k++) cam[k] = p.cams[FK_CNP * (size_t)j + k];
// ... 88 lines not shown
#pragma unroll
  for (int off = 32; off > 0; off >>= 1) m = fmax(m, __shfl_down(m, off, 64));
  if ((threadIdx.x & 63) == 0) sRed[threadIdx.x >> 6] = m;
  __syncthreads();
  if (threadIdx.x == 0) {
    m = fmax(fmax(sRed[0], sRed[1]), fmax(sRed[2], sRed[3]));
    atomicMax(reinterpret_cast<unsigned long long *>(out), (unsigned long long)__double_as_longlong(m));
  }
}

__global__ __launch_bounds__(256) void k_fk_schur(const double *W, const double *PV, const int *iidx, const int *jidx,
                                                  const int *ptr, double *S, double *ea, int ld, double mu, int nO,
                                                  int *status, int try_id) {
  for (int a = blockIdx.x * blockDim.x + threadIdx.x; a < nO; a += gridDim.x * blockDim.x) {
    const int i = iidx[a], ja = jidx[a];
    const double *pv = PV + 9 * (size_t)i;
    double v[6], vi[6];
#pragma unroll
    for (int k = 0; k < 6; k++) v[k] = pv[k];
    v[0] += mu;
    v[3] += mu;
    v[5] += mu;
    if (sym3_inverse(v, vi)) status[0] = try_id;
    const double g0 = pv[6], g1 = pv[7], g2 = pv[8];
    const double *w = W + FK_W * (size_t)a;
    double Y[FK_W];
#pragma unroll
    for (int r = 0; r < FK_CNP; r++) {
      const double w0 = w[3 * r], w1 = w[3 * r + 1], w2 = w[3 * r + 2];
      Y[3 * r] = w0 * vi[0] + w1 * vi[1] + w2 * vi[2];
      Y[3 * r + 1] = w0 * vi[1] + w1 * vi[3] + w2 * vi[4];
      Y[3 * r + 2] = w0 * vi[2] + w1 * vi[4] + w2 * vi[5];
      atomicAdd(&ea[FK_CNP * ja + r], -(Y[3 * r] * g0 + Y[3 * r + 1] * g1 + Y[3 * r + 2] * g2));
    }
    for (int b = ptr[i]; b <= a; b++) {
      double *Sblk = S + (size_t)(FK_CNP * ja) * ld + FK_CNP * jidx[b];
      const double *wb = W + FK_W * (size_t)b;
      for (int c = 0; c < FK_CNP; c++) {
        const double w0 = wb[3 * c], w1 = wb[3 * c + 1], w2 = wb[3 * c + 2];
#pragma unroll
        for (int r = 0; r < FK_CNP; r++)
          atomicAdd(&Sblk[(size_t)r * ld + c], -(Y[3 * r] * w0 + Y[3 * r + 1] * w1 + Y[3 * r + 2] * w2));
      }
    }
  }
}

__global__ __launch_bounds__(256) void k_fk_finalize(double *S, double *ea, const double *U, const double *ga, double mu,
                                                     int nA, int n32, double *scal, int *status, int try_id) {
  if (blockIdx.x == 0 && threadIdx.x < 4 * SC_NPART) scal[SC_PART + threadIdx.x] = 0.0;
  if (blockIdx.x == 0 && threadIdx.x == 64) status[3] = try_id;
  const size_t n2 = (size_t)nA * nA;
  const size_t gtid = (size_t)blockIdx.x * blockDim.x + threadIdx.x, gsize = (size_t)gridDim.x * blockDim.x;
  for (size_t t = gtid; t < n2; t += gsize) {
    const int r = (int)(t / nA), c = (int)(t % nA);
    const int kb = r / FK_CNP, lb = c / FK_CNP;
    const size_t at = (size_t)r * n32 + c;
    if (lb > kb) {
      S[at] = S[(size_t)c * n32 + r];
    } else if (lb == kb) {
      double v = S[at] + U[(size_t)FK_CNP * FK_CNP * kb + FK_CNP * (r - FK_CNP * kb) + (c - FK_CNP * lb)];
      if (r == c) v += mu;
      S[at] = v;
    }
  }
  for (size_t t = gtid; t < (size_t)nA; t += gsize) ea[t] += ga[t];
  write_padding(S, nA, n32, 1.0, gtid, gsize);
}

struct FkBackArgs {
  const double *W, *PV, *camconst, *cams, *pts, *impts, *ga;
  const int *jidx, *ptr;
  double *dp, *newcams, *newpts, *scal;
  const int *status;
  double mu;
  int nC, nA, nP;
};
__global__ __launch_bounds__(256) void k_fk_backsub_cams(FkBackArgs p) {
  __shared__ double sRed[3][4];
  double s_dp = 0.0, s_den = 0.0, s_np = 0.0;
  if (blockIdx.x == 0 && threadIdx.x == 0) {
    p.scal[SC_STATUS_V] = (p.status[0] == p.status[3]) ? 1.0 : 0.0;
    p.scal[SC_STATUS_SPD] = (p.status[1] == p.status[3]) ? 1.0 : 0.0;
  }
  for (int t = blockIdx.x * blockDim.x + threadIdx.x; t < p.nA; t += gridDim.x * blockDim.x) {
    const double d = p.dp[t], c = p.cams[t] + d;
    p.newcams[t] = c;
    s_dp += d * d;
    s_den += d * (p.mu * d + p.ga[t]);
    s_np += c * c;
  }
  double v3[3] = {s_dp, s_den, s_np};
#pragma unroll
  for (int q = 0; q < 3; q++) {
    double v = v3[q];
#pragma unroll
    for (int off = 32; off > 0; off >>= 1) v += __shfl_down(v, off, 64);
    if ((threadIdx.x & 63) == 0) sRed[q][threadIdx.x >> 6] = v;
  }
  __syncthreads();
  if (threadIdx.x == 0) {
    double *dst = p.scal + SC_PART + 4 * (blockIdx.x % SC_NPART);
    atomicAdd(&dst[0], sRed[0][0] + sRed[0][1] + sRed[0][2] + sRed[0][3]);
    atomicAdd(&dst[1], sRed[1][0] + sRed[1][1] + sRed[1][2] + sRed[1][3]);
    atomicAdd(&dst[3], sRed[2][0] + sRed[2][1] + sRed[2][2] + sRed[2][3]);
  }
}
__global__ __launch_bounds__(256) void k_fk_backsub_pts(FkBackArgs p) {
  __shared__ double sRed[4][4];
  double s_dp = 0.0, s_den = 0.0, s_cost = 0.0, s_np = 0.0;
  for (int i = blockIdx.x * blockDim.x + threadIdx.x; i < p.nP; i += gridDim.x * blockDim.x) {
    const double *pv = p.PV + 9 * (size_t)i;
    const int o0 = p.ptr[i], o1 = p.ptr[i + 1];
    double e0 = pv[6], e1 = pv[7], e2 = pv[8];
    for (int a = o0; a < o1; a++) {
      const double *w = p.W + FK_W * (size_t)a;
      const double *da = p.dp + FK_CNP * (size_t)p.jidx[a];
#pragma unroll
      for (int k = 0; k < FK_CNP; k++) {
        e0 -= w[3 * k] * da[k];
        e1 -= w[3 * k + 1] * da[k];
        e2 -= w[3 * k + 2] * da[k];
      }
    }
    double v[6], vi[6];
#pragma unroll
    for (int k = 0; k < 6; k++) v[k] = pv[k];
    v[0] += p.mu;
    v[3] += p.mu;
    v[5] += p.mu;
    sym3_inverse(v, vi);
    const double d[3] = {vi[0] * e0 + vi[1] * e1 + vi[2] * e2, vi[1] * e0 + vi[3] * e1 + vi[4] * e2,
                         vi[2] * e0 + vi[4] * e1 + vi[5] * e2};
    double n3[3];
#pragma unroll
    for (int q = 0; q < 3; q++) {
      n3[q] = p.pts[3 * (size_t)i + q] + d[q];
      p.dp[p.nA + 3 * (size_t)i + q] = d[q];
      p.newpts[3 * (size_t)i + q] = n3[q];
      s_dp += d[q] * d[q];
      s_den += d[q] * (p.mu * d[q] + pv[6 + q]);
      s_np += n3[q] * n3[q];
    }
    for (int a = o0; a < o1; a++) {
      const int j = p.jidx[a];
      double cam[FK_CNP], q0[4], r0, r1;
#pragma unroll
      for (int k = 0; k < FK_CNP; k++) cam[k] = p.newcams[FK_CNP * (size_t)j + k];
#pragma unroll
      for (int k = 0; k < 4; k++) q0[k] = p.camconst[9 * (size_t)j + 5 + k];
      const double2 m = reinterpret_cast<const double2 *>(p.impts)[a];
      residual_obs(cam, q0, cam + 5, n3, m.x, m.y, r0, r1);
      s_cost += r0 * r0 + r1 * r1;
    }
  }
  double v4[4] = {s_dp, s_den, s_cost, s_np};
#pragma unroll
  for (int q = 0; q < 4; q++) {
    double v = v4[q];
#pragma unroll
    for (int off = 32; off > 0; off >>= 1) v += __shfl_down(v, off, 64);
    if ((threadIdx.x & 63) == 0) sRed[q][threadIdx.x >> 6] = v;
  }
  __syncthreads();
  if (threadIdx.x < 4) {
    const double v = sRed[threadIdx.x][0] + sRed[threadIdx.x][1] + sRed[threadIdx.x][2] + sRed[threadIdx.x][3];
// ... 121 lines not shown
```

### psba_amd/csrc/lm_loop.cpp

```cpp
#include <chrono>
#include <cmath>
#include <cstdio>

#include "psba_internal.h"

extern "C" {

void psba_lm_default_options(psba_lm_options *o) {
  if (!o) return;
  o->max_iter = 50;
  o->tr_handoff = 1;
  o->verbose = 0;
  o->log_cap = 0;
  o->start_itno = 0;
  o->init_mu = 0.0;
}

int psba_levmar(psba_handle h, const psba_lm_options *opts, psba_lm_result *res, double *log) {
  if (!h || !opts || !res) return PSBA_E_INVALID;
  const double STOP = 1e-12;
  const double EPS_SQ = 1e-12 * 1e-12;
  const double tau = opts->init_mu != 0.0 ? opts->init_mu : 1e-3;
  *res = psba_lm_result();
  auto t_begin = std::chrono::steady_clock::now();
  int rc;
#define LM_TRY(x)          \
  do {                     \
    rc = (x);              \
    if (rc < 0) return rc; \
  } while (0)

  double ex_L2 = 0, new_ex_L2 = 0, p_L2 = 0, dp_L2 = 0, mu = 0, rho = 0;
  int nu = 2, gooditer = 0, tries = 0, nlog = 0;
  bool first = true;
  int flag = PSBA_ITER_CONTINUE;
  int itno = opts->start_itno;

  double maxdiag0 = 0;
  LM_TRY(psba_begin(h, 1.0, 1.0, &ex_L2, &maxdiag0));
  res->init_err = ex_L2;

  for (; itno < opts->max_iter && flag == PSBA_ITER_CONTINUE; itno++) {
    LM_TRY(psba_linearize(h, 1.0, 1.0));
    if (first) {
      mu = tau * maxdiag0;
      res->mu0 = mu;
      first = false;
      p_L2 = 1e+3;
      nu = 2;
    }
    while (true) {
      tries++;
      psba_try_scalars sc;
      LM_TRY(psba_schur_assemble(h, mu));
      LM_TRY(psba_schur_reduce(h));
      LM_TRY(psba_schur_solve(h));
      if (rc == PSBA_PCG_MAXIT) {
        res->pcg_unconverged++;
        if (opts->verbose) {
          int it = 0;
          double rr = 0;
          psba_pcg_info(h, &it, &rr, nullptr, nullptr);
          printf("itno=%d\t\tpcg: %d iterations without reaching the tolerance, relres=%.3e\n", itno, it, rr);
        }
      }
      LM_TRY(psba_backsub_async(h, mu));
      if (itno + 1 < opts->max_iter) LM_TRY(psba_linearize_ahead(h));
      LM_TRY(psba_backsub_wait(h, &sc));
      if (!(sc.status & PSBA_NOT_SPD)) {
        dp_L2 = sc.dp_l2;
        if (dp_L2 < p_L2 * STOP * STOP) {
          flag = PSBA_ITER_DP_NO_CHANGE;
          break;
        }
        if (dp_L2 >= (p_L2 + STOP) / EPS_SQ) {
          flag = PSBA_ITER_ERR;
          break;
        }
        new_ex_L2 = sc.new_cost;
        rho = (ex_L2 - new_ex_L2) / sc.gain_den;
        if (opts->verbose)
          printf("itno=%d\t\tErr=%.15E\t\trho=%f\t\tmu=%f\n", itno, new_ex_L2, rho, mu);
        if (log && nlog < opts->log_cap) {
          double *row = log + 5 * nlog++;
          row[0] = itno; row[1] = new_ex_L2; row[2] = rho; row[3] = mu; row[4] = rho > 0 ? 1 : 0;
        }
        if (rho > 0) {
          double tmp = 2 * rho - 1;
          tmp = 1.0 - tmp * tmp * tmp;
          mu = mu * ((tmp >= (1.0 / 3.0)) ? tmp : (1.0 / 3.0));
          nu = 2;
          LM_TRY(psba_accept(h));
          p_L2 = sc.newp_l2;
          ex_L2 = new_ex_L2;
          if (std::fabs(rho - 1) < (1.0 / 5.0)) {
            gooditer++;
            if (opts->tr_handoff && gooditer >= 5) {
              flag = PSBA_ITER_TURN_TO_TR;
              break;
            }
          } else {
            gooditer = 0;
          }
          break;
        }
      } else {
        gooditer = 0;
        if (log && nlog < opts->log_cap) {
          double *row = log + 5 * nlog++;
          row[0] = itno; row[1] = NAN; row[2] = NAN; row[3] = mu; row[4] = -1;
        }
      }
      mu *= nu;
      const double nu2 = 2.0 * nu;
      if (nu2 <= nu || nu2 > 1e9) {
        flag = PSBA_ITER_ERR;
        break;
      }
      nu = (int)nu2;
    }
    if (ex_L2 <= STOP) flag = PSBA_ITER_ERR_SMALL_ENOUGH;
  }
#undef LM_TRY
  if (hipStreamSynchronize(h->stream) != hipSuccess) return PSBA_E_HIP;
  res->flag = flag;
  res->iters = itno;
  res->tries = tries;
  res->final_err = ex_L2;
  res->mu_final = mu;
  res->n_log = nlog;
  res->seconds = std::chrono::duration<double>(std::chrono::steady_clock::now() - t_begin).count();
  return flag;
}

}
```

### psba_amd/csrc/psba_api.cpp

```cpp
#include <algorithm>
#include <cmath>
#include <cstdarg>
#include <cstdio>
#include <cstdlib>
#include <cstring>
#include <string>
#include <new>
#include <vector>

#include "camera_model.h"
#include "psba_internal.h"

using namespace psba;

static thread_local std::string g_create_err;

namespace psba {

int fail(psba_ctx *h, int code, const char *fmt, ...) {
  char buf[1024];
  va_list ap;
  va_start(ap, fmt);
  vsnprintf(buf, sizeof buf, fmt, ap);
  va_end(ap);
// ... 67 lines not shown
static void dev_free(T *&p) {
  if (p) (void)hipFree(p);
  p = nullptr;
}

static void free_problem_buffers(psba_ctx *h) {
  for (int v = 0; v < 2; v++)
    if (h->chol_graph[v]) {
      (void)hipGraphExecDestroy(h->chol_graph[v]);
      h->chol_graph[v] = nullptr;
    }
  dev_free(h->camconst);
  dev_free(h->cams[0]);
  dev_free(h->cams[1]);
  dev_free(h->pts[0]);
  dev_free(h->pts[1]);
  dev_free(h->impts);
  dev_free(h->lens_kc);
  dev_free(h->lens_w);
  dev_free(h->obs_s);
  h->lens = 0;
  h->loss_kind = PSBA_LOSS_NONE;
  h->loss_c = 1.0;
  dev_free(h->iidx);
  dev_free(h->jidx);
  dev_free(h->ptr);
  dev_free(h->params0);
  dev_free(h->tile_pt);
  dev_free(h->tile_desc);
  dev_free(h->long_pts);
  h->nLong = 0;
  dev_free(h->W);
  dev_free(h->W_alt);
  dev_free(h->PV_alt);
  dev_free(h->U_alt);
  dev_free(h->ga_alt);
  dev_free(h->PV);
  dev_free(h->U);
  dev_free(h->ga);
  dev_free(h->campart);
  dev_free(h->camacc);
  dev_free(h->cam_obs);
  dev_free(h->cam_units);
  h->nCamUnits = 0;
  dev_free(h->red);
  dev_free(h->items);
  dev_free(h->wg);
  dev_free(h->posblock);
  dev_free(h->gtab);
  dev_free(h->diag0);
  dev_free(h->redp);
  dev_free(h->slab);
#ifdef PSBA_BUILD_EXPERIMENTS
  dev_free(h->ring_wg);
  dev_free(h->ring_steps);
  dev_free(h->ring_entries);
  dev_free(h->ring_ops);
  dev_free(h->ring_jobs);
  dev_free(h->ring_bl0);
  dev_free(h->ring_canon);
  dev_free(h->ring_slab);
  dev_free(h->ring_pvi);
#endif
  h->ring_nWg = h->ring_nS = 0;
  dev_free(h->bs_val);
  h->bs_ea = nullptr;
  dev_free(h->bs_jk);
  dev_free(h->bs_diag);
  dev_free(h->bs_rowptr);
  dev_free(h->bs_rowent);
  dev_free(h->pcg_vec);
  dev_free(h->pcg_minv);
  dev_free(h->pcg_scal);
  h->bs_nblk = 0;
  dev_free(h->own_prod);
  dev_free(h->own_waves);
  dev_free(h->own_units);
  h->own_nwaves = 0;
  dev_free(h->dp);
  dev_free(h->trv[0]);
  dev_free(h->trv[1]);
  dev_free(h->jmul_out);
  dev_free(h->chol_ws);
  dev_free(h->dist_buf);
  dev_free(h->chol_L);
  dev_free(h->dbg_ex);
  dev_free(h->dbg_JA);
  dev_free(h->dbg_JB);
  dev_free(h->dbg_Y);
  dev_free(h->dbg_Vinv);
  dev_free(h->dbg_eb);
  h->uploaded = h->linearized = h->assembled = h->solved = h->backsubbed = false;
}

extern "C" {

const char *psba_version(void) { return "psba_hip 0.1 (gfx950, fp64)"; }

const char *psba_last_error(psba_handle h) { return h ? h->err.c_str() : g_create_err.c_str(); }

static hipError_t create_main_stream(hipStream_t *s) {
  int least = 0, greatest = 0;
  if (getenv("PSBA_STREAM_PRIO_DEFAULT") || hipDeviceGetStreamPriorityRange(&least, &greatest) != hipSuccess)
    return hipStreamCreateWithFlags(s, hipStreamNonBlocking);
  return hipStreamCreateWithPriority(s, hipStreamNonBlocking, greatest);
}

int psba_create(int device, psba_handle *out) {
  if (!out) return PSBA_E_INVALID;
  *out = nullptr;
  int ndev = 0;
  hipError_t e = hipGetDeviceCount(&ndev);
  if (e != hipSuccess || ndev == 0)
    return fail(nullptr, PSBA_E_HIP, "no HIP device available (%s); this library has no CPU path",
                e == hipSuccess ? "device count 0" : hipGetErrorString(e));
  if (device < 0 || device >= ndev)
    return fail(nullptr, PSBA_E_INVALID, "device %d out of range (%d devices)", device, ndev);
  psba_ctx *h = new psba_ctx();
  h->device = device;
  if ((e = hipSetDevice(device)) != hipSuccess ||
      (e = create_main_stream(&h->stream)) != hipSuccess ||
      (e = hipMalloc((void **)&h->scal, sizeof(double) * NSCAL)) != hipSuccess ||
      (e = hipHostMalloc((void **)&h->h_scal, sizeof(double) * (NSCAL + 8))) != hipSuccess ||
      (e = hipEventCreateWithFlags(&h->scal_event, hipEventDisableTiming)) != hipSuccess) {
    int rc = fail(nullptr, PSBA_E_HIP, "psba_create: %s", hipGetErrorString(e));
    delete h;
    return rc;
  }
  if (hipHostGetDevicePointer((void **)&h->h_scal_dev, h->h_scal, 0) != hipSuccess) h->h_scal_dev = nullptr;
  h->status = reinterpret_cast<int *>(h->scal + 8);
  h->h_status = reinterpret_cast<int *>(h->h_scal + 8);
  (void)hipMemsetAsync(h->scal, 0, sizeof(double) * NSCAL, h->stream);
  (void)hipStreamSynchronize(h->stream);
  h->h_scal[NSCAL] = 0.0;
  *out = h;
  return PSBA_OK;
}

int psba_destroy(psba_handle h) {
  CHECK_H(h);
  (void)hipSetDevice(h->device);
  if (h->stream) (void)hipStreamSynchronize(h->stream);
  if (h->stream2) (void)hipStreamSynchronize(h->stream2);
  if (h->comm) ncclCommDestroy(h->comm);
  if (h->k3_event) (void)hipEventDestroy(h->k3_event);
  for (hipEvent_t e : h->chol_events) (void)hipEventDestroy(e);
  if (h->chol_side) {
    (void)hipStreamSynchronize(h->chol_side);
    (void)hipStreamDestroy(h->chol_side);
  }
  if (h->stream2) (void)hipStreamDestroy(h->stream2);
  free_problem_buffers(h);
  dev_free(h->scal);
  if (h->h_scal) (void)hipHostFree(h->h_scal);
  if (h->pcg_host) (void)hipHostFree(h->pcg_host);
  if (h->scal_event) (void)hipEventDestroy(h->scal_event);
  for (auto &s : h->spans) {
    (void)hipEventDestroy(s.a);
    (void)hipEventDestroy(s.b);
  }
  if (h->stream) (void)hipStreamDestroy(h->stream);
  delete h;
  return PSBA_OK;
}

int psba_schur_path(psba_handle h, int *path) {
// ... 187 lines not shown
  d.nP = n3Dpts;
  d.nO = n2Dprojs;
  const int cnp = h->cnp;
  if (cnp != 6 && (h->solver == PSBA_SOLVER_PCG || h->nranks > 1 || h->comm))
    return fail(h, PSBA_E_INVALID, "free intrinsics: dense solver, single rank only");
  d.nA = cnp * nCams;
  d.nB = 3 * n3Dpts;
  d.nT = d.nA + d.nB;
  d.nTilesAll = (int)tile_pt.size() - 1;
  d.nTiles = d.nTilesAll - (int)long_pts.size();
  if (d.nTiles < 1) d.nTiles = 1;
  d.maxTrack = maxTrack;
  const size_t cam_lds_max = getenv("PSBA_LIN_LDS_ACC") ? 96 * 1024 : 48 * 1024;
  h->cam_global = cnp == 6 && ((size_t)CAM_ACC * nCams * sizeof(double) > cam_lds_max || getenv("PSBA_LIN_GLOBAL_ACC"));
  h->d = d;
  h->nPart = d.nTiles < 768 ? d.nTiles : 768;
  if (const char *e = getenv("PSBA_LIN_GRID")) h->nPart = atoi(e) > 0 && atoi(e) < d.nTiles ? atoi(e) : d.nTiles;
  h->cur = 0;

  std::vector<double> cc((size_t)nCams * 9);
  for (int j = 0; j < nCams; j++) {
    for (int k = 0; k < 5; k++) cc[(size_t)9 * j + k] = Kparas[5 * j + k];
    for (int k = 0; k < 4; k++) cc[(size_t)9 * j + 5 + k] = initrot[4 * j + k];
  }
  TRY(dev_alloc(h, &h->camconst, cc.size()));
  TRY(dev_alloc(h, &h->cams[0], (size_t)d.nA));
  TRY(dev_alloc(h, &h->cams[1], (size_t)d.nA));
  TRY(dev_alloc(h, &h->pts[0], (size_t)d.nB));
  TRY(dev_alloc(h, &h->pts[1], (size_t)d.nB));
  TRY(dev_alloc(h, &h->params0, (size_t)d.nT));
  TRY(dev_alloc(h, &h->impts, (size_t)2 * d.nO));
  TRY(dev_alloc(h, &h->iidx, (size_t)d.nO));
  TRY(dev_alloc(h, &h->jidx, (size_t)d.nO));
  TRY(dev_alloc(h, &h->ptr, (size_t)d.nP + 1));
  TRY(dev_alloc(h, &h->tile_pt, tile_pt.size()));
  TRY(dev_alloc(h, &h->tile_desc, (size_t)d.nTiles));
  h->nLong = (int)long_pts.size();
  if (h->nLong) {
    TRY(dev_alloc(h, &h->long_pts, long_pts.size()));
    PSBA_HIP(h, hipMemcpy(h->long_pts, long_pts.data(), sizeof(int) * long_pts.size(), hipMemcpyHostToDevice));
  }
  TRY(dev_alloc(h, &h->W, (size_t)3 * cnp * d.nO));
  TRY(dev_alloc(h, &h->W_alt, (size_t)3 * cnp * d.nO));
  TRY(dev_alloc(h, &h->PV, (size_t)9 * d.nP));
  TRY(dev_alloc(h, &h->PV_alt, (size_t)9 * d.nP));
  PSBA_HIP(h, hipMemsetAsync(h->PV, 0, sizeof(double) * 9 * (size_t)d.nP, h->stream));
  PSBA_HIP(h, hipMemsetAsync(h->PV_alt, 0, sizeof(double) * 9 * (size_t)d.nP, h->stream));
  TRY(dev_alloc(h, &h->U, (size_t)cnp * cnp * d.nC));
  TRY(dev_alloc(h, &h->U_alt, (size_t)cnp * cnp * d.nC));
  TRY(dev_alloc(h, &h->ga, (size_t)d.nA));
  TRY(dev_alloc(h, &h->ga_alt, (size_t)d.nA));
  h->ahead = h->lin_is_ahead = false;
  TRY(dev_alloc(h, &h->campart, (h->cam_global || cnp != 6) ? 1 : (size_t)(h->nPart + 1) * d.nC * CAM_ACC));
  if (cnp != 6) TRY(dev_alloc(h, &h->camacc, (size_t)d.nC * (cnp * (cnp + 1) / 2 + cnp)));
  if (h->cam_global) {
    TRY(dev_alloc(h, &h->camacc, (size_t)d.nC * CAM_ACC));
    std::vector<int> cptr((size_t)nCams + 1, 0), cobs((size_t)n2Dprojs);
    for (int a = 0; a < n2Dprojs; a++) cptr[(size_t)jidx[a] + 1]++;
    for (int j = 0; j < nCams; j++) cptr[(size_t)j + 1] += cptr[j];
    {
      std::vector<int> at(cptr.begin(), cptr.end() - 1);
      for (int a = 0; a < n2Dprojs; a++) cobs[(size_t)at[jidx[a]]++] = a;
    }
    std::vector<int4> units;
    const int LSEG = 256;
    for (int j = 0; j < nCams; j++)
      for (int f = cptr[j]; f < cptr[(size_t)j + 1]; f += LSEG)
        units.push_back(make_int4(j, f, std::min(f + LSEG, cptr[(size_t)j + 1]), 0));
    h->nCamUnits = (int)units.size();
    TRY(dev_alloc(h, &h->cam_obs, cobs.size()));
    TRY(dev_alloc(h, &h->cam_units, units.size()));
    PSBA_HIP(h, hipMemcpy(h->cam_obs, cobs.data(), sizeof(int) * cobs.size(), hipMemcpyHostToDevice));
    PSBA_HIP(h, hipMemcpy(h->cam_units, units.data(), sizeof(int4) * units.size(), hipMemcpyHostToDevice));
  }
  h->n32 = (d.nA + 31) / 32 * 32;
  const bool sparse = h->solver == PSBA_SOLVER_PCG;
  const size_t dense = sparse ? 1 : (size_t)(2 * h->n32 + 16) * h->n32;
  TRY(dev_alloc(h, &h->red, dense));
  PSBA_HIP(h, hipMemsetAsync(h->red, 0, sizeof(double) * dense, h->stream));
  TRY(dev_alloc(h, &h->dp, (size_t)(d.nT > 36 * d.nC ? d.nT : 36 * d.nC)));
  TRY(dev_alloc(h, &h->chol_ws, (size_t)((d.nA + 31) / 32) * 1024));
  TRY(dev_alloc(h, &h->chol_L, dense));
  PSBA_HIP(h, hipMemsetAsync(h->chol_L, 0, sizeof(double) * dense, h->stream));
  if (getenv("PSBA_CHOL_TIMING") && !h->chol_tim) TRY(dev_alloc(h, &h->chol_tim, 32));
  if (sparse) {
    OwnerPlanHost op;
    std::vector<unsigned char> pat;
    if (h->nranks > 1 || (h->comm && getenv("PSBA_SPARSE_PATTERN_FORCE"))) {
      const size_t nBlk = (size_t)nCams * (nCams + 1) / 2;
      if (h->comm) {
        pat.resize(nBlk);
        TRY(sparse_pattern(nCams, n2Dprojs, iidx, jidx, ptr.data(), pat.data()));
        unsigned char *dev = nullptr;
        PSBA_HIP(h, hipMalloc((void **)&dev, nBlk));
        hipError_t e1 = hipMemcpyAsync(dev, pat.data(), nBlk, hipMemcpyHostToDevice, h->stream);
        ncclResult_t e2 = e1 == hipSuccess ? ncclAllReduce(dev, dev, nBlk, ncclUint8, ncclMax, h->comm, h->stream) : ncclSuccess;
        if (e1 == hipSuccess && e2 == ncclSuccess) e1 = hipMemcpyAsync(pat.data(), dev, nBlk, hipMemcpyDeviceToHost, h->stream);
        if (e1 == hipSuccess && e2 == ncclSuccess) e1 = hipStreamSynchronize(h->stream);
        (void)hipFree(dev);
        if (e2 != ncclSuccess) return fail(h, PSBA_E_RCCL, "all-reduce of the block pattern: %s", ncclGetErrorString(e2));
        PSBA_HIP(h, e1);
      } else {
        if (h->bs_pattern.size() != nBlk)
          return fail(h, PSBA_E_STATE, "PSBA_SOLVER_PCG with a rank layout and no communicator: psba_set_sparse_pattern "
                                       "(the union of psba_sparse_pattern over the ranks) before psba_upload_problem");
        pat = h->bs_pattern;
      }
    }
    TRY(build_owner_plan(nCams, n2Dprojs, iidx, jidx, ptr.data(), op, pat.empty() ? nullptr : pat.data()));
    h->nGroups = 0;
    h->packedN = 36 * (size_t)nCams * (nCams + 1) / 2;
    TRY(dev_alloc(h, &h->own_prod, op.prod.size()));
    TRY(dev_alloc(h, &h->own_waves, op.waves.size()));
    TRY(dev_alloc(h, &h->own_units, op.units.size()));
    PSBA_HIP(h, hipMemcpy(h->own_prod, op.prod.data(), sizeof(int2) * op.prod.size(), hipMemcpyHostToDevice));
    PSBA_HIP(h, hipMemcpy(h->own_waves, op.waves.data(), sizeof(OwnerWave) * op.waves.size(), hipMemcpyHostToDevice));
    PSBA_HIP(h, hipMemcpy(h->own_units, op.units.data(), sizeof(OwnerUnit) * op.units.size(), hipMemcpyHostToDevice));
    h->own_nwaves = (int)op.waves.size();
    h->own_products = op.products;
    h->bs_nblk = (long long)op.blocks.size();
    TRY(dev_alloc(h, &h->bs_val, (size_t)36 * op.blocks.size() + (size_t)d.nA));
    h->bs_ea = h->bs_val + (size_t)36 * op.blocks.size();
    TRY(dev_alloc(h, &h->bs_jk, op.blocks.size()));
    TRY(dev_alloc(h, &h->bs_diag, op.diag_slot.size()));
    PSBA_HIP(h, hipMemcpy(h->bs_jk, op.blocks.data(), sizeof(int2) * op.blocks.size(), hipMemcpyHostToDevice));
    PSBA_HIP(h, hipMemcpy(h->bs_diag, op.diag_slot.data(), sizeof(int) * op.diag_slot.size(), hipMemcpyHostToDevice));
    {
      std::vector<int> rp((size_t)nCams + 1, 0);
      for (const int2 &b : op.blocks) {
        rp[(size_t)b.x + 1]++;
        if (b.x != b.y) rp[(size_t)b.y + 1]++;
      }
      for (int j = 0; j < nCams; j++) rp[(size_t)j + 1] += rp[(size_t)j];
      std::vector<int2> ent((size_t)rp[(size_t)nCams]);
      std::vector<int> at(rp.begin(), rp.end() - 1);
      for (size_t sl = 0; sl < op.blocks.size(); sl++) {
        const int2 b = op.blocks[sl];
        if (b.x == b.y) {
          ent[(size_t)at[(size_t)b.x]++] = make_int2((int)sl, b.x | (2 << 28));
        } else {
          ent[(size_t)at[(size_t)b.x]++] = make_int2((int)sl, b.y);
          ent[(size_t)at[(size_t)b.y]++] = make_int2((int)sl, b.x | (1 << 28));
        }
      }
      TRY(dev_alloc(h, &h->bs_rowptr, rp.size()));
      TRY(dev_alloc(h, &h->bs_rowent, ent.size()));
      PSBA_HIP(h, hipMemcpy(h->bs_rowptr, rp.data(), sizeof(int) * rp.size(), hipMemcpyHostToDevice));
      PSBA_HIP(h, hipMemcpy(h->bs_rowent, ent.data(), sizeof(int2) * ent.size(), hipMemcpyHostToDevice));
    }
    TRY(dev_alloc(h, &h->pcg_vec, (size_t)5 * d.nA));
    TRY(dev_alloc(h, &h->pcg_minv, (size_t)36 * d.nC));
    TRY(dev_alloc(h, &h->pcg_scal, (size_t)(16 + 4 * 64)));
    if (!h->pcg_host && hipHostMalloc((void **)&h->pcg_host, sizeof(double) * 16) != hipSuccess)
      return fail(h, PSBA_E_NOMEM, "no pinned memory for the PCG scalars");
    if (getenv("PSBA_SCHUR_PLAN_INFO"))
      fprintf(stderr, "[psba] block-sparse S: %lld of %lld blocks of the lower block triangle (%.1f %%), %lld products\n",
              h->bs_nblk, (long long)nCams * (nCams + 1) / 2, 100.0 * (double)h->bs_nblk / ((double)nCams * (nCams + 1) / 2),
              op.products);
  }
#ifdef PSBA_BUILD_EXPERIMENTS
  if (!sparse) {
    RingPlanHost rp;
    TRY(build_ring_plan(nCams, n3Dpts, n2Dprojs, iidx, jidx, ptr.data(), rp));
    if (rp.nWg > 0) {
      h->packedN = 36 * (size_t)nCams * (nCams + 1) / 2;
      h->nGroups = 0;
      h->ring_nWg = rp.nWg;
// ... 220 lines not shown
                          h->comm, h->stream));
  } else {
    TRY(launch_max_diag(h));
  }
  return PSBA_OK;
}

int psba_begin(psba_handle h, double coeff, double coeff_g, double *cost, double *max_diag) {
  CHECK_H(h);
  NEED(h, h->uploaded, "no problem uploaded");
  TRY(enqueue_residual(h, PSBA_PARAMS_CUR));
  h->coeff = coeff;
  h->coeff_g = coeff_g;
  TRY(launch_linearize(h, false));
  h->linearized = true;
  h->assembled = h->solved = h->backsubbed = false;
  h->ahead = false;
  TRY(enqueue_max_diag(h));
  TRY(fetch_scalars(h));
  if (cost) *cost = h->h_scal[SC_COST];
  if (max_diag) *max_diag = h->h_scal[SC_MAXDIAG];
  h->lin_is_ahead = true;
  return PSBA_OK;
}

int psba_max_diag(psba_handle h, double *out) {
  CHECK_H(h);
  NEED(h, h->linearized, "psba_linearize first");
  TRY(enqueue_max_diag(h));
  TRY(fetch_scalars(h));
  if (out) *out = h->h_scal[SC_MAXDIAG];
  return PSBA_OK;
}

int psba_schur_assemble(psba_handle h, double mu) {
  CHECK_H(h);
  NEED(h, h->linearized, "psba_linearize first");
  h->mu = mu;
  TRY(launch_schur(h, mu, false));
  h->assembled = true;
  h->solved = h->backsubbed = false;
  return PSBA_OK;
}

static int allreduce_schur(psba_ctx *h) {
  if (h->solver == PSBA_SOLVER_PCG) {
    if (h->comm)
      RCCL(h, ncclAllReduce(h->bs_val, h->bs_val, (size_t)36 * h->bs_nblk + h->d.nA, ncclDouble, ncclSum, h->comm, h->stream));
    return PSBA_OK;
  }
  if (h->packed_pending) {
    if (h->comm)
      RCCL(h, ncclAllReduce(h->redp, h->redp, h->packed_doubles, ncclDouble, ncclSum, h->comm, h->stream));
    TRY(launch_schur_expand(h));
    h->packed_pending = false;
  } else if (h->comm) {
    const size_t n = (size_t)(h->n32 + 1) * h->n32;
    RCCL(h, ncclAllReduce(h->red, h->red, n, ncclDouble, ncclSum, h->comm, h->stream));
  }
  return PSBA_OK;
}

int psba_schur_reduce(psba_handle h) {
  CHECK_H(h);
  NEED(h, h->assembled, "psba_schur_assemble first");
  if (!h->comm) return PSBA_OK;
  ProfScope ps(h, PSBA_K_ALLREDUCE);
  TRY(allreduce_schur(h));
  return PSBA_OK;
}

int psba_schur_solve(psba_handle h) {
  CHECK_H(h);
  NEED(h, h->assembled, "psba_schur_assemble first");
  if (h->packed_pending) TRY(allreduce_schur(h));
  if (h->solver == PSBA_SOLVER_PCG) {
    TRY(launch_pcg_solve(h));
    h->assembled = false;
    h->solved = true;
    return h->pcg_exhausted ? PSBA_PCG_MAXIT : PSBA_OK;
  }
  TRY(launch_chol_solve(h));
  if (h->chol_tim) {
    long long t[32];
    PSBA_HIP(h, hipMemcpyAsync(t, h->chol_tim, sizeof t, hipMemcpyDeviceToHost, h->stream));
    PSBA_HIP(h, hipStreamSynchronize(h->stream));
    fprintf(stderr, "chol stamps (cycles since the first):");
    for (int k = 1; k < 32; k++) fprintf(stderr, " %lld", t[k] ? t[k] - t[0] : 0);
    fprintf(stderr, "\n");
  }
  h->assembled = false;
  h->solved = true;
  return PSBA_OK;
}

static int publish_scalars(psba_ctx *h, hipStream_t s) {
  if (h->h_scal_dev && !getenv("PSBA_SCAL_MEMCPY"))
    TRY(launch_publish_scal(h, s));
  else
    PSBA_HIP(h, hipMemcpyAsync(h->h_scal, h->scal, sizeof(double) * NSCAL, hipMemcpyDeviceToHost, s));
  PSBA_HIP(h, hipEventRecord(h->scal_event, s));
  return PSBA_OK;
}

int psba_backsub_async(psba_handle h, double mu) {
  CHECK_H(h);
  NEED(h, h->solved, "psba_schur_solve first");
  TRY(launch_backsub(h, mu, false));
  hipStream_t s = h->stream;
  if (h->comm) {
    if (h->stream2 && getenv("PSBA_COMM_SIDE_STREAM")) {
      PSBA_HIP(h, hipEventRecord(h->k3_event, h->stream));
      PSBA_HIP(h, hipStreamWaitEvent(h->stream2, h->k3_event, 0));
      s = h->stream2;
      h->scal_side = true;
    }
    RCCL(h, ncclAllReduce(h->scal + SC_PART, h->scal + SC_PART, 4 * SC_NPART + 2, ncclDouble, ncclSum, h->comm, s));
  }
  h->publish_in_k1 = false;
  h->publish_deferred = !h->comm && h->h_scal_dev && !getenv("PSBA_SCAL_MEMCPY") && !getenv("PSBA_SCAL_KERNEL");
  if (!h->publish_deferred) TRY(publish_scalars(h, s));
  h->solved = false;
  h->backsub_pending = true;
  h->ahead = false;
  return PSBA_OK;
}

int psba_linearize_ahead(psba_handle h) {
  CHECK_H_NOJOIN(h);
  NEED(h, h->backsub_pending || h->backsubbed, "psba_backsub_async / psba_backsub first");
  const bool carry = h->backsub_pending && h->publish_deferred;
  if (carry) h->pub_seq += 1.0;
  TRY(launch_linearize(h, false, true, carry));
  if (carry) {
    h->publish_deferred = false;
    h->publish_in_k1 = true;
  }
  h->ahead = true;
  return PSBA_OK;
}

int psba_backsub_wait(psba_handle h, psba_try_scalars *out) {
  CHECK_H_NOJOIN(h);
  NEED(h, h->backsub_pending, "psba_backsub_async first");
  if (h->publish_deferred) {
    TRY(publish_scalars(h, h->stream));
    h->publish_deferred = false;
  }
  if (h->publish_in_k1) {
    volatile double *stamp = h->h_scal + NSCAL;
    long long spin = 0;
    while (*stamp != h->pub_seq && ++spin < 200000000LL) {
      if ((spin & 0xfffff) == 0 && hipStreamQuery(h->stream) != hipErrorNotReady) break;
    }
    if (*stamp != h->pub_seq) {
      PSBA_HIP(h, hipStreamSynchronize(h->stream));
      if (*stamp != h->pub_seq) return fail(h, PSBA_E_HIP, "the try's scalars did not reach the host");
    }
    __sync_synchronize();
    h->publish_in_k1 = false;
  } else {
    for (int spin = 0; spin < 20000 && hipEventQuery(h->scal_event) == hipErrorNotReady; spin++) {
    }
    PSBA_HIP(h, hipEventSynchronize(h->scal_event));
  }
  h->scal_side = false;
  h->backsub_pending = false;
  for (int q = 0; q < 4; q++) {
    double v = 0.0;
    for (int s = 0; s < SC_NPART; s++) v += h->h_scal[SC_PART + 4 * s + q];
    h->h_scal[SC_DP_L2 + q] = v;
  }
  const int st0 = h->h_scal[SC_STATUS_V] > 0.0 ? h->try_id : 0;
  const int st1 = h->h_scal[SC_STATUS_SPD] > 0.0 ? h->try_id : 0;
  h->backsubbed = true;
  if (out) {
    out->status = (st1 == h->try_id ? PSBA_NOT_SPD : 0) | (st0 == h->try_id ? PSBA_SINGULAR_V : 0);
    out->dp_l2 = h->h_scal[SC_DP_L2];
    out->gain_den = h->h_scal[SC_GAIN_DEN];
    out->new_cost = h->h_scal[SC_NEW_COST];
    out->newp_l2 = h->h_scal[SC_NEWP_L2];
  }
  return PSBA_OK;
}

int psba_backsub(psba_handle h, double mu, psba_try_scalars *out) {
  TRY(psba_backsub_async(h, mu));
  return psba_backsub_wait(h, out);
}

int psba_accept(psba_handle h) {
  CHECK_H(h);
  NEED(h, h->backsubbed, "psba_backsub first");
  h->cur = 1 - h->cur;
  h->linearized = h->assembled = h->solved = h->backsubbed = false;
  if (h->ahead) {
    std::swap(h->W, h->W_alt);
    std::swap(h->PV, h->PV_alt);
    std::swap(h->U, h->U_alt);
    std::swap(h->ga, h->ga_alt);
  }
  h->lin_is_ahead = h->ahead;
  h->ahead = false;
  return PSBA_OK;
}


static int d2h(psba_ctx *h, void *dst, const void *src, size_t bytes);

int psba_chol_dist_shape(psba_handle h, int *n32, int *NB, int *sharded) {
  CHECK_H(h);
  NEED(h, h->uploaded, "no problem uploaded");
  int nb = 0, bl = 0;
  TRY(chol_dist_shape(h, &nb, &bl));
  if (n32) *n32 = h->n32;
  if (NB) *NB = nb;
  if (sharded) *sharded = bl;
  return PSBA_OK;
}
int psba_chol_shape(psba_handle h, int *out8) {
  CHECK_H(h);
  NEED(h, h->uploaded, "no problem uploaded");
  if (!out8) return fail(h, PSBA_E_INVALID, "psba_chol_shape: null pointer");
  return chol_shape(h, out8);
}
int psba_chol_dist_exchange_plan(int n32, int NB, int nranks, int JE, long long *out4, int cap) {
  if (!out4 || cap <= 0) return PSBA_E_INVALID;
  return psba::chol_dist_exchange_plan(n32, NB, nranks, JE, reinterpret_cast<long long(*)[4]>(out4), cap);
}
int psba_chol_dist_begin(psba_handle h) {
  CHECK_H(h);
  NEED(h, h->assembled, "psba_schur_assemble (and the reduction over ranks) first");
  if (h->packed_pending) {
    TRY(launch_schur_expand(h));
    h->packed_pending = false;
  }
  return chol_dist_begin(h);
}
int psba_chol_dist_superpanel(psba_handle h, int J) {
  CHECK_H(h);
  NEED(h, h->assembled, "psba_schur_assemble first");
  if (J < 0 || J >= h->n32) return fail(h, PSBA_E_INVALID, "super-panel column %d out of range", J);
  return chol_dist_superpanel(h, J);
}
int psba_chol_dist_block(psba_handle h, int B, int set, double *buf, long long *n_doubles) {
  CHECK_H(h);
  NEED(h, h->assembled, "psba_schur_assemble first");
  if (B < 0 || 64 * B >= h->n32) return fail(h, PSBA_E_INVALID, "column block %d out of range", B);
  const int ncols = h->n32 - 64 * B < 64 ? h->n32 - 64 * B : 64;
  const long long n = (long long)(h->n32 + 1 - 64 * B) * ncols;
  if (n_doubles) *n_doubles = n;
  if (!buf) return PSBA_OK;
  if (!h->dist_buf) TRY(dev_alloc(h, &h->dist_buf, (size_t)(h->n32 + 1) * 64 * 8));
  if (set) {
    PSBA_HIP(h, hipMemcpyAsync(h->dist_buf, buf, sizeof(double) * (size_t)n, hipMemcpyHostToDevice, h->stream));
    return chol_dist_block(h, B, h->dist_buf, 1);
  }
  TRY(chol_dist_block(h, B, h->dist_buf, 0));
  return d2h(h, buf, h->dist_buf, sizeof(double) * (size_t)n);
}
int psba_chol_dist_finish(psba_handle h) {
  CHECK_H(h);
  NEED(h, h->assembled, "psba_schur_assemble first");
  TRY(chol_dist_finish(h));
  h->assembled = false;
  h->solved = true;
  return PSBA_OK;
}

static int ensure_trv(psba_ctx *h) {
  for (int k = 0; k < 2; k++)
    if (!h->trv[k]) TRY(dev_alloc(h, &h->trv[k], (size_t)h->d.nT));
  return PSBA_OK;
}

int psba_jmul_dots(psba_handle h, const double *x1, const double *x2, double dots[3]) {
  CHECK_H(h);
  NEED(h, h->cnp == 6, "six-parameter camera blocks only (free intrinsics: the fused verbs and psba_levmar)");
  NEED(h, h->uploaded, "no problem uploaded");
  if (!x1 || !dots) return fail(h, PSBA_E_INVALID, "psba_jmul_dots: null pointer");
  TRY(ensure_trv(h));
  const size_t bytes = sizeof(double) * (size_t)h->d.nT;
  PSBA_HIP(h, hipMemcpyAsync(h->trv[0], x1, bytes, hipMemcpyHostToDevice, h->stream));
  if (x2 && x2 != x1) PSBA_HIP(h, hipMemcpyAsync(h->trv[1], x2, bytes, hipMemcpyHostToDevice, h->stream));
  TRY(launch_jmul(h, h->trv[0], (x2 && x2 != x1) ? h->trv[1] : h->trv[0], nullptr, h->scal + SC_TR_DOTS));
  if (h->comm)
    RCCL(h, ncclAllReduce(h->scal + SC_TR_DOTS, h->scal + SC_TR_DOTS, 3, ncclDouble, ncclSum, h->comm, h->stream));
  TRY(fetch_scalars(h));
  for (int k = 0; k < 3; k++) dots[k] = h->h_scal[SC_TR_DOTS + k];
  return PSBA_OK;
}

int psba_set_solver(psba_handle h, int solver, double tol, int max_iter) {
  CHECK_H(h);
  if (solver != PSBA_SOLVER_DENSE && solver != PSBA_SOLVER_PCG) return fail(h, PSBA_E_INVALID, "unknown solver %d", solver);
  NEED(h, !h->uploaded || solver == h->solver, "psba_set_solver before psba_upload_problem (the buffers depend on it)");
  h->solver = solver;
  if (tol > 0) h->pcg_tol = tol;
  if (max_iter > 0) h->pcg_maxit = max_iter;
  return PSBA_OK;
}

int psba_pcg_info(psba_handle h, int *iters, double *relres, long long *blocks, long long *dense_blocks) {
  CHECK_H(h);
  NEED(h, h->uploaded && h->solver == PSBA_SOLVER_PCG, "PSBA_SOLVER_PCG and an uploaded problem");
  if (iters) *iters = h->pcg_iters;
  if (relres) *relres = h->pcg_relres;
// ... 213 lines not shown
int psba_maxElmOfUV(psba_handle h, double *out) { return psba_max_diag(h, out); }

int psba_update_UV(psba_handle h, double mu, double *U, double *V) {
  CHECK_H(h);
  NEED(h, h->cnp == 6, "six-parameter camera blocks only (free intrinsics: the fused verbs and psba_levmar)");
  NEED(h, h->linearized, "linearise first");
  h->mu = mu;
  h->mu_applied = true;
  if (U) {
    TRY(d2h(h, U, h->U, sizeof(double) * 36 * (size_t)h->d.nC));
    for (int t = 0; t < h->d.nA; t++) U[36 * (t / 6) + 7 * (t % 6)] += mu;
  }
  return download_V(h, V, mu);
}

int psba_restore_UVdiag(psba_handle h) {
  CHECK_H(h);
  h->mu_applied = false;
  return PSBA_OK;
}

int psba_compute_Vinv(psba_handle h, double *Vinv) {
  CHECK_H(h);
  TRY(reassemble_dump(h));
  TRY(d2h(h, Vinv, h->dbg_Vinv, sizeof(double) * 9 * (size_t)h->d.nP));
  TRY(fetch_scalars(h));
  return h->h_status[0] == h->try_id ? PSBA_SINGULAR_V : PSBA_OK;
}

int psba_compute_Wblks(psba_handle h, double coeff, double *Wblks) {
  CHECK_H(h);
  NEED(h, h->cnp == 6, "six-parameter camera blocks only (free intrinsics: the fused verbs and psba_levmar)");
  NEED(h, h->uploaded, "no problem uploaded");
  h->coeff = coeff;
  TRY(relinearize_dump(h));
  return d2h(h, Wblks, h->W, sizeof(double) * 18 * (size_t)h->d.nO);
}

int psba_compute_Yblks(psba_handle h, double *Yblks) {
  CHECK_H(h);
  TRY(reassemble_dump(h));
  return d2h(h, Yblks, h->dbg_Y, sizeof(double) * 18 * (size_t)h->d.nO);
}

int psba_compute_S(psba_handle h, double *S) {
  CHECK_H(h);
  TRY(reassemble_dump(h));
  if (!S) return PSBA_OK;
  PSBA_HIP(h, hipMemcpy2DAsync(S, sizeof(double) * h->d.nA, h->red, sizeof(double) * h->n32,
                               sizeof(double) * h->d.nA, h->d.nA, hipMemcpyDeviceToHost, h->stream));
  PSBA_HIP(h, hipStreamSynchronize(h->stream));
  return PSBA_OK;
}

int psba_compute_g(psba_handle h, double coeff, double *g) {
  CHECK_H(h);
  NEED(h, h->cnp == 6, "six-parameter camera blocks only (free intrinsics: the fused verbs and psba_levmar)");
  NEED(h, h->uploaded, "no problem uploaded");
  h->coeff_g = coeff;
  TRY(relinearize_dump(h));
  if (!g) return PSBA_OK;
  TRY(d2h(h, g, h->ga, sizeof(double) * (size_t)h->d.nA));
  std::vector<double> pv((size_t)9 * h->d.nP);
  TRY(d2h(h, pv.data(), h->PV, sizeof(double) * pv.size()));
  for (int i = 0; i < h->d.nP; i++)
    for (int k = 0; k < 3; k++) g[h->d.nA + 3 * (size_t)i + k] = pv[(size_t)9 * i + 6 + k];
  return PSBA_OK;
}

int psba_compute_ea(psba_handle h, double *ea) {
  CHECK_H(h);
  TRY(reassemble_dump(h));
  return d2h(h, ea, h->red + (size_t)h->n32 * h->n32, sizeof(double) * (size_t)h->d.nA);
}

int psba_SPDinv_matVec(psba_handle h, double *dpa) {
  CHECK_H(h);
  NEED(h, h->assembled, "compute_S / compute_ea first");
  TRY(launch_chol_solve(h));
  h->assembled = false;
  h->solved = true;
  TRY(fetch_scalars(h));
  TRY(d2h(h, dpa, h->dp, sizeof(double) * (size_t)h->d.nA));
  return h->h_status[1] == h->try_id ? PSBA_NOT_SPD : PSBA_OK;
}

static int backsub_dump(psba_ctx *h) {
  NEED(h, h->solved, "SPDinv_matVec first");
  TRY(ensure_dbg(h));
  TRY(launch_backsub(h, h->mu_applied ? h->mu : 0.0, true));
  h->backsubbed = true;
  return PSBA_OK;
}

int psba_compute_eb(psba_handle h, double *eb) {
  CHECK_H(h);
  TRY(backsub_dump(h));
  return d2h(h, eb, h->dbg_eb, sizeof(double) * 3 * (size_t)h->d.nP);
}

int psba_compute_dpb(psba_handle h, double *dp) {
  CHECK_H(h);
  TRY(backsub_dump(h));
  return d2h(h, dp, h->dp, sizeof(double) * (size_t)h->d.nT);
}

int psba_compute_newp(psba_handle h, double *new_p) {
  CHECK_H(h);
  NEED(h, h->backsubbed, "compute_dpb first");
  if (!new_p) return PSBA_OK;
  TRY(d2h(h, new_p, h->cams[1 - h->cur], sizeof(double) * (size_t)h->d.nA));
  return d2h(h, new_p + h->d.nA, h->pts[1 - h->cur], sizeof(double) * (size_t)h->d.nB);
}

int psba_update_p(psba_handle h, double *p) {
  CHECK_H(h);
  TRY(psba_accept(h));
  if (!p) return PSBA_OK;
  TRY(d2h(h, p, h->cams[h->cur], sizeof(double) * (size_t)h->d.nA));
  return d2h(h, p + h->d.nA, h->pts[h->cur], sizeof(double) * (size_t)h->d.nB);
}


int psba_partition_points(int n3Dpts, const int *iidx, int n2Dprojs, int nranks, int *pt_begin) {
  if (n3Dpts <= 0 || nranks <= 0 || !iidx || !pt_begin || n2Dprojs < 0) return PSBA_E_INVALID;
  std::vector<long long> cum((size_t)n3Dpts + 1, 0);
  for (int a = 0; a < n2Dprojs; a++) {
    if (iidx[a] < 0 || iidx[a] >= n3Dpts) return PSBA_E_INVALID;
    cum[(size_t)iidx[a] + 1]++;
  }
  for (int i = 0; i < n3Dpts; i++) cum[(size_t)i + 1] += cum[i];
  pt_begin[0] = 0;
  int p = 0;
  for (int r = 1; r < nranks; r++) {
    const long long target = (long long)n2Dprojs * r / nranks;
    while (p < n3Dpts && cum[p] < target) p++;
    int lo = pt_begin[r - 1] + 1, hi = n3Dpts - (nranks - r);
    if (n3Dpts >= nranks) {
      if (p < lo) p = lo;
      if (p > hi) p = hi;
    }
    pt_begin[r] = p;
  }
  pt_begin[nranks] = n3Dpts;
  return PSBA_OK;
}

int psba_comm_unique_id(void *id128) {
  if (!id128) return PSBA_E_INVALID;
  static_assert(sizeof(ncclUniqueId) == 128, "RCCL unique id is 128 bytes");
  ncclUniqueId id;
  if (ncclGetUniqueId(&id) != ncclSuccess) return PSBA_E_RCCL;
  memcpy(id128, &id, sizeof id);
  return PSBA_OK;
}

int psba_comm_init(psba_handle h, int nranks, int rank, const void *id128) {
  CHECK_H(h);
  if (nranks < 1 || rank < 0 || rank >= nranks || !id128)
    return fail(h, PSBA_E_INVALID, "psba_comm_init: bad rank %d / %d", rank, nranks);
  PSBA_HIP(h, hipSetDevice(h->device));
  ncclUniqueId id;
  memcpy(&id, id128, sizeof id);
  RCCL(h, ncclCommInitRank(&h->comm, nranks, id, rank));
  if (!h->stream2) {
    PSBA_HIP(h, hipStreamCreateWithFlags(&h->stream2, hipStreamNonBlocking));
// ... 342 lines not shown
```

### psba_amd/csrc/psba_internal.h

```cpp
#pragma once
#include <hip/hip_runtime.h>
#include <rccl/rccl.h>

#include <string>
#include <vector>

#include "../../include/psba_hip.h"

namespace psba {

constexpr int TILE_OBS = 256;
constexpr int TILE_PTS = 128;
constexpr int MAX_GROUPS = 128;
constexpr int CAM_ACC = 27;
constexpr int NSCAL = 104;
constexpr int SC_NPART = 16;

enum {
  SC_COST = 0,
  SC_DP_L2 = 1,
  SC_GAIN_DEN = 2,
  SC_NEW_COST = 3,
  SC_NEWP_L2 = 4,
  SC_MAXDIAG = 7,
  SC_PART = 16,
  SC_STATUS_V = 80,
  SC_STATUS_SPD = 81,
  SC_TR_DOTS = 84,
  SC_CHOLMOD = 88,
  SC_SUMS = 96,
};

struct Dims {
  int nC = 0, nP = 0, nO = 0;
  int nA = 0, nB = 0, nT = 0;
  int nTiles = 0;
  int nTilesAll = 0;
  int maxTrack = 0;
};

constexpr int ITEM_OBS_BITS = 24, ITEM_PT_BITS = 22, ITEM_BOFF_BITS = 8, ITEM_POS_BITS = 10;
struct SchurWg {
  int group, nblk;
  int obs0, pt0;
  long long item0, item1;
  unsigned long long slab_off;
  long long itemD;
};
constexpr int PAIR_OBS_BITS = 18, PAIR_PT_BITS = 16;
constexpr unsigned long long SCHUR_NULL_ITEM = ~0ull;
struct ReduceGroup {
  int nwg, nblk;
  long long pos0;
  unsigned long long slab;
  unsigned long long pad;
};

struct OwnerWave {
  long long row0;
  int len;
  int pad;
};
struct OwnerUnit {
  int j, k;
  int multi;
  int slot;
};
struct OwnerPlanHost {
  std::vector<int2> prod;
  std::vector<OwnerWave> waves;
  std::vector<OwnerUnit> units;
  std::vector<int2> blocks;
  std::vector<int> diag_slot;
  long long products = 0;
};
#ifdef PSBA_BUILD_EXPERIMENTS
constexpr int RING_LANES = 256;
constexpr int RING_MOVERS = 4;
constexpr int RING_PREPPERS = 4;
constexpr int RING_PREP_JOBS = 32;
constexpr int RING_PAGE = 7;
constexpr int RING_SLOTS = 992;
constexpr int RING_MAXOPS = 16;
constexpr unsigned RING_NULL_ENTRY = 0xFFFFFFFFu;
struct RingStep { int op_begin, op_end, job_begin, job_end; };
struct RingJob {
  int obs, point;
  int slots;
  int earow;
};
struct RingWg {
  int blk0, nblk;
  int row0, nrows;
  int copy, nsteps;
  int nwslots, pad;
  long long step0, ent0, op0, job0, lane0, bl0;
};
struct RingPlanHost {
  int nR = 0, nS = 0, nWg = 0, lat = 2;
  std::vector<int> rb;
  std::vector<RingWg> wgs;
  std::vector<RingStep> steps;
  std::vector<unsigned> entries;
  std::vector<int> ops;
  std::vector<RingJob> jobs;
  std::vector<int> lane_blk;
  std::vector<int> blk_lane0;
  long long products = 0, slots = 0, loaded_recs = 0;
};
#endif
// ... 47 lines not shown
  bool ahead = false;
  bool lin_is_ahead = false;
  double *h_scal_dev = nullptr;
  hipEvent_t scal_event = nullptr;
  hipStream_t stream2 = nullptr;
  hipEvent_t k3_event = nullptr;
  hipStream_t chol_side = nullptr;
  std::vector<hipEvent_t> chol_events;
  bool scal_side = false;
  double *campart = nullptr;
  int nPart = 0;
  bool cam_global = false;
  double *camacc = nullptr;
  int *cam_obs = nullptr;
  int4 *cam_units = nullptr;
  int nCamUnits = 0;
  double *red = nullptr;
  int n32 = 0;
  int nGroups = 0;
  int nWg = 0;
  std::vector<int> gblk0;
  std::vector<int> gnwg;
  std::vector<int> gnblk;
  std::vector<size_t> gslab;
  psba::ReduceGroup *gtab = nullptr;
  psba::SchurWg *wg = nullptr;
  unsigned long long *items = nullptr;
  double *redp = nullptr;
  size_t packed_doubles = 0;
  bool packed_pending = false;
  double *diag0 = nullptr;
  int h_diagpos[21] = {0};
  int h_diaggrp[21] = {0};
  bool diag_done = false;
  int *posblock = nullptr;
  double *slab = nullptr;
  size_t packedN = 0;
  int ring_nWg = 0, ring_nS = 0;
#ifdef PSBA_BUILD_EXPERIMENTS
  psba::RingWg *ring_wg = nullptr;
  psba::RingStep *ring_steps = nullptr;
  unsigned *ring_entries = nullptr;
  int *ring_ops = nullptr;
  psba::RingJob *ring_jobs = nullptr;
  int *ring_bl0 = nullptr;
  int *ring_canon = nullptr;
  double *ring_slab = nullptr;
  double *ring_pvi = nullptr;
  long long ring_products = 0, ring_slots = 0;
  size_t ring_loaded_recs = 0;
  bool ring_attr_set = false;
  long long *chol_tim_ring = nullptr;
#endif
  int solver = 0;
  bool schur_runs = false;
  bool schur_pairs = false;
  int cnp = 6;
  double pcg_tol = 1e-10;
  int pcg_maxit = 500, pcg_iters = 0;
  double pcg_relres = 0.0;
  bool pcg_exhausted = false;
  long long bs_nblk = 0;
  double *bs_val = nullptr;
  double *bs_ea = nullptr;
  int2 *bs_jk = nullptr;
  int *bs_diag = nullptr;
  int *bs_rowptr = nullptr;
  int2 *bs_rowent = nullptr;
  double *pcg_vec = nullptr;
  double *pcg_minv = nullptr;
  double *pcg_scal = nullptr, *pcg_host = nullptr;
  std::vector<unsigned char> bs_pattern;
  int2 *own_prod = nullptr;
  psba::OwnerWave *own_waves = nullptr;
  psba::OwnerUnit *own_units = nullptr;
  int own_nwaves = 0;
  long long own_products = 0;
  double *dp = nullptr;
  double *trv[2] = {nullptr, nullptr};
  double *jmul_out = nullptr;
  hipGraphExec_t chol_graph[2] = {nullptr, nullptr};
  int chol_graph_n32[2] = {0, 0};
  double *chol_graph_red[2] = {nullptr, nullptr};
  long long *chol_tim = nullptr;
  double *chol_L = nullptr;
  double *dist_buf = nullptr;
  double *chol_ws = nullptr;
  double *scal = nullptr;
  int *status = nullptr;
  int try_id = 0;
  double *h_scal = nullptr;
  int *h_status = nullptr;
  double *dbg_ex = nullptr, *dbg_JA = nullptr, *dbg_JB = nullptr, *dbg_Y = nullptr,
         *dbg_Vinv = nullptr, *dbg_eb = nullptr;

  bool lds_attr_set = false, atomic_attr_set = false, chol_attr_set = false, lin_attr_set = false;

  bool uploaded = false, linearized = false, assembled = false, solved = false, backsubbed = false;
  bool backsub_pending = false;
  bool publish_deferred = false, publish_in_k1 = false;
  double pub_seq = 0.0;
  int cur = 0;
  double coeff = 1.0, coeff_g = 1.0, mu = 0.0;
  double coeff_w = 1.0;
  bool mu_applied = false;

  unsigned prof = 0;
  struct Span { hipEvent_t a, b; int kind; };
  std::vector<Span> spans;
  size_t spans_used = 0;
  double prof_ms[PSBA_K_COUNT] = {0};
  int prof_n[PSBA_K_COUNT] = {0};
};

namespace psba {

int fail(psba_ctx *h, int code, const char *fmt, ...);
#define PSBA_HIP(h, call)                                                              \
  do {                                                                                 \
    hipError_t e__ = (call);                                                           \
    if (e__ != hipSuccess)                                                             \
      return psba::fail((h), PSBA_E_HIP, "%s failed: %s (%s:%d)", #call,               \
                        hipGetErrorString(e__), __FILE__, __LINE__);                   \
  } while (0)

struct ProfScope {
  psba_ctx *h;
  int idx = -1;
  ProfScope(psba_ctx *h, int kind);
  ~ProfScope();
};

int launch_linearize(psba_ctx *h, bool dump, bool ahead = false, bool publish = false);
int launch_residual(psba_ctx *h, int which, double *ex_out_dev, double *s_out_dev = nullptr);
int launch_max_diag(psba_ctx *h);
int build_schur_plan(psba_ctx *h, int nCams, int nPts, int nObs, const int *iidx, const int *jidx,
                     const int *ptr, SchurPlanHost &out);
int build_owner_plan(int nCams, int nObs, const int *iidx, const int *jidx, const int *ptr, OwnerPlanHost &out,
                     const unsigned char *pattern = nullptr);
int sparse_pattern(int nCams, int nObs, const int *iidx, const int *jidx, const int *ptr, unsigned char *flags);
#ifdef PSBA_BUILD_EXPERIMENTS
int build_ring_plan(int nCams, int nPts, int nObs, const int *iidx, const int *jidx, const int *ptr, RingPlanHost &out,
                    bool force = false);
int launch_schur_ring(psba_ctx *h, double mu, bool dump);
struct SchurLdsArgs;
bool launch_schur_lds_mode(int mode, dim3 G, dim3 B, size_t lds, hipStream_t s, const SchurLdsArgs &a);
#endif
int launch_schur(psba_ctx *h, double mu, bool dump);
int launch_schur_expand(psba_ctx *h);
int launch_chol_solve(psba_ctx *h);
int launch_linearize_fk(psba_ctx *h, bool ahead, bool publish);
int launch_residual_fk(psba_ctx *h, int which);
int launch_max_diag_fk(psba_ctx *h);
int launch_schur_fk(psba_ctx *h, double mu);
int launch_backsub_fk(psba_ctx *h, double mu);
int launch_bsr_finalize(psba_ctx *h, double mu);
int launch_pcg_solve(psba_ctx *h);
int launch_bsr_gershgorin(psba_ctx *h, double *lambda, double *info3);
int launch_chol_graph(psba_ctx *h);
int chol_dist_shape(psba_ctx *h, int *NB, int *blocked);
int chol_shape(psba_ctx *h, int *out8);
int chol_dist_exchange_plan(int n32, int NB, int nranks, int JE, long long (*out)[4], int cap);
int chol_dist_begin(psba_ctx *h);
int chol_dist_superpanel(psba_ctx *h, int J);
int chol_dist_block(psba_ctx *h, int B, double *buf_dev, int set);
int chol_dist_finish(psba_ctx *h);
int launch_backsub(psba_ctx *h, double mu, bool dump);
int launch_publish_scal(psba_ctx *h, hipStream_t s);
int launch_jmul(psba_ctx *h, const double *x1_dev, const double *x2_dev, double *out1_dev, double *dots_dev);
int launch_pack_g(psba_ctx *h, double *g_dev);
int launch_newp(psba_ctx *h, const double *dp_dev);
int launch_cholmod(psba_ctx *h, double *out4_dev);

}
```

### psba_amd/csrc/tr_loop.cpp

```cpp
#include <chrono>
#include <cmath>
#include <cstdio>
#include <vector>

#include "psba_internal.h"

extern "C" int psba_jmul_dots(psba_handle h, const double *x1, const double *x2, double dots[3]);
extern "C" int psba_get_gradient(psba_handle h, double *g);
extern "C" int psba_get_dp(psba_handle h, double *dp);
extern "C" int psba_set_step(psba_handle h, const double *dp);
extern "C" int psba_cholmod_lambda(psba_handle h, int reassemble, double *lambda, double *info3);
extern "C" int psba_allreduce_scalars(psba_handle h, double *v, int n);

namespace {

template <int K>
int dots(psba_handle h, size_t nA, size_t nT, const double *const (&x)[K], const double *const (&y)[K], double (&out)[K]) {
  double pts[K];
  for (int k = 0; k < K; k++) {
    double c = 0, q = 0;
    for (size_t i = 0; i < nA; i++) c += x[k][i] * y[k][i];
    for (size_t i = nA; i < nT; i++) q += x[k][i] * y[k][i];
    out[k] = c;
    pts[k] = q;
// ... 17 lines not shown
    if (lu > delta) {
      alpha = delta / lu;
      beta = 0;
      len = delta;
    } else if (lb <= delta) {
      alpha = 0;
      beta = 1;
      len = lb;
    } else {
      const double c = uu - delta * delta;
      double disc = ud * ud - dd * c;
      if (std::fabs(disc) < 0.25e-12) disc = 0;
      const double sgm = (-ud + std::sqrt(disc)) / dd;
      alpha = 1 - sgm;
      beta = sgm;
      len = delta;
    }
  }
  return len;
}

}

extern "C" {

void psba_tr_default_options(psba_tr_options *o) {
  if (!o) return;
  o->max_iter = 50;
  o->start_itno = 0;
  o->verbose = 0;
  o->log_cap = 0;
  o->init_lambda = 0.0;
}

int psba_trust_region(psba_handle h, const psba_tr_options *opts, psba_tr_result *res, double *log) {
  if (!h || !opts || !res) return PSBA_E_INVALID;
  if (h->cnp != 6) return PSBA_E_STATE;
  const double EPS2 = 1e-12, MAX_DELTA = 10000;
  *res = psba_tr_result();
  auto t_begin = std::chrono::steady_clock::now();
  int rc;
#define TR_TRY(x)          \
  do {                     \
    rc = (x);              \
    if (rc < 0) return rc; \
  } while (0)
  int nC = 0, nP = 0, nO = 0;
  TR_TRY(psba_get_dims(h, &nC, &nP, &nO));
  const size_t nA = (size_t)6 * nC, nT = nA + (size_t)3 * nP;
  std::vector<double> g(nT), PU(nT), PB(nT), P(nT);
  double dk = 1, lambda = opts->init_lambda, origin_lambda = 0;
  int nu = 2, notgood = 0, good_iters = 0, itno = opts->start_itno, nlog = 0, tries = 0, chol_fail = 0;
  int flag = PSBA_ITER_CONTINUE;
  double ex_L2 = 0;
  TR_TRY(psba_residual(h, PSBA_PARAMS_CUR, &ex_L2));
  res->init_err = ex_L2;
  double final_err = ex_L2;
  bool stop = false;

  for (; itno < opts->max_iter && !stop; itno++) {
    TR_TRY(psba_linearize(h, 2.0, -2.0));
    TR_TRY(psba_get_gradient(h, g.data()));
    double d3[3];
    TR_TRY(psba_jmul_dots(h, g.data(), nullptr, d3));
    double gtg1[1];
    {
      const double *const xs[1] = {g.data()};
      TR_TRY(dots<1>(h, nA, nT, xs, xs, gtg1));
    }
    const double gtBg = 2 * d3[0], gtg = gtg1[0];
    for (size_t i = 0; i < nT; i++) PU[i] = -(g[i] * gtg) / gtBg;
    if (h->solver == PSBA_SOLVER_PCG && lambda == 0.0) {
      double md = 0;
      TR_TRY(psba_max_diag(h, &md));
      lambda = 1e-8 * md;
    }
    bool solved = false;
    while (!solved) {
      psba_try_scalars sc;
      TR_TRY(psba_schur_assemble(h, lambda));
      TR_TRY(psba_schur_reduce(h));
      TR_TRY(psba_schur_solve(h));
      TR_TRY(psba_backsub(h, lambda, &sc));
      if (sc.status & PSBA_NOT_SPD) {
        chol_fail++;
        if (lambda == 0.0) {
          TR_TRY(psba_cholmod_lambda(h, 1, &lambda, nullptr));
        } else {
          lambda = 2 * lambda;
        }
        if (origin_lambda != 0.0) {
          if (nu > 4) {
            flag = PSBA_ITER_TURN_TO_LM;
            final_err = ex_L2;
            stop = true;
            break;
          }
          lambda = lambda * nu;
          nu = nu * 2;
        }
        if (!std::isfinite(lambda) || chol_fail > 200) {
          flag = PSBA_ITER_ERR;
          stop = true;
          break;
        }
        continue;
      }
      TR_TRY(psba_get_dp(h, P.data()));
      for (size_t i = 0; i < nT; i++) PB[i] = -P[i];
      solved = true;
      nu = 2;
      origin_lambda = lambda;
    }
    if (stop) break;
    TR_TRY(psba_jmul_dots(h, PU.data(), PB.data(), d3));
    const double uBu = 2 * d3[0], uBb = 2 * d3[1], bBb = 2 * d3[2];
    double ip[7];
    {
      for (size_t i = 0; i < nT; i++) P[i] = PB[i] - PU[i];
      const double *const xs[7] = {PU.data(), PU.data(), PB.data(), PU.data(), PB.data(), P.data(), PU.data()};
      const double *const ys[7] = {PU.data(), PB.data(), PB.data(), g.data(), g.data(), P.data(), P.data()};
      TR_TRY(dots<7>(h, nA, nT, xs, ys, ip));
    }
    flag = PSBA_ITER_CONTINUE;
    while (flag == PSBA_ITER_CONTINUE) {
      tries++;
      double alpha, beta;
      const double p_norm = tr_step(uBu, uBb, bBb, dk, ip[0], ip[1], ip[2], ip[3], ip[4], ip[5], ip[6], alpha, beta);
      for (size_t i = 0; i < nT; i++) P[i] = alpha * PU[i] + beta * PB[i];
      TR_TRY(psba_set_step(h, P.data()));
      double act = 0;
      TR_TRY(psba_residual(h, PSBA_PARAMS_NEW, &act));
      if (std::fabs((ex_L2 - act) / ex_L2) < EPS2) {
        flag = PSBA_ITER_DP_NO_CHANGE;
        break;
      }
      TR_TRY(psba_jmul_dots(h, P.data(), nullptr, d3));
      const double Jx_norm = 2 * d3[0];
      const double pred = alpha * ip[3] + beta * ip[4] + ex_L2 + Jx_norm / 2;
      const double rho = (ex_L2 - act) / (ex_L2 - pred);
      bool accepted = false;
      if (rho < 0.25 || act > ex_L2) {
        dk = dk / 4;
      } else if (rho >= 0.75 && act < ex_L2) {
        accepted = true;
        dk = std::fmin(2 * dk, MAX_DELTA);
      } else if (rho >= 0.25 && rho < 0.75 && act < ex_L2) {
        accepted = true;
      } else if (std::isnan(rho)) {
        flag = PSBA_ITER_TURN_TO_LM;
        final_err = ex_L2;
        stop = true;
        break;
      }
      if (accepted) {
        flag = PSBA_ITER_PASS;
        TR_TRY(psba_accept(h));
        final_err = act;
      }
      if (opts->verbose)
        printf("itno=%d\tErr:%.15E\tDelta=%f\tRho=%f\tnorm_p=%f\tLambda=%E\n", itno, act, dk, rho, p_norm, lambda);
      if (log && nlog < opts->log_cap) {
        double *row = log + 6 * nlog++;
        row[0] = itno; row[1] = act; row[2] = rho; row[3] = dk; row[4] = lambda; row[5] = accepted ? 1 : 0;
      }
      if (std::fabs((act - ex_L2) / ex_L2) <= EPS2) {
// ... 82 lines not shown
```

Before: 2111 M-obs/s.

## Run dense Cholesky panel chain as one persistent kernel with device-side flags

```diff
diff --git a/include/psba_hip.h b/include/psba_hip.h
--- a/include/psba_hip.h
+++ b/include/psba_hip.h
@@ -11,6 +11,7 @@
 #define PSBA_NOT_SPD 1
 #define PSBA_SINGULAR_V 2
 #define PSBA_PCG_MAXIT 4
+#define PSBA_CHOL_REDO 8
 #define PSBA_E_INVALID (-1)
 #define PSBA_E_HIP (-2)
 #define PSBA_E_RCCL (-3)
@@ -212,6 +213,8 @@
 
 int psba_chol_dist_shape(psba_handle h, int *n32, int *NB, int *sharded);
 int psba_chol_shape(psba_handle h, int *out8);
+int psba_chol_persist_info(psba_handle h, int *out4);
+int psba_chol_persist_plan(int n32, int *out, int cap);
 int psba_chol_dist_exchange_plan(int n32, int NB, int nranks, int JE, long long *out4, int cap);
 int psba_chol_dist_begin(psba_handle h);
 int psba_chol_dist_superpanel(psba_handle h, int J);
diff --git a/psba_amd/capi.py b/psba_amd/capi.py
--- a/psba_amd/capi.py
+++ b/psba_amd/capi.py
@@ -156,6 +156,8 @@
     ("psba_chol_dist_exchange_plan", C.c_int, [C.c_int, C.c_int, C.c_int, C.c_int, C.POINTER(C.c_longlong), C.c_int]),
     ("psba_chol_dist_shape", C.c_int, [_h, _ip, _ip, _ip]),
     ("psba_chol_shape", C.c_int, [_h, _ip]),
+    ("psba_chol_persist_info", C.c_int, [_h, _ip]),
+    ("psba_chol_persist_plan", C.c_int, [C.c_int, _ip, C.c_int]),
     ("psba_chol_dist_begin", C.c_int, [_h]),
     ("psba_chol_dist_superpanel", C.c_int, [_h, C.c_int]),
     ("psba_chol_dist_block", C.c_int, [_h, C.c_int, C.c_int, _dp, C.POINTER(C.c_longlong)]),
@@ -327,6 +329,31 @@
     finally:
         lib.psba_owner_plan_destroy(p)
     return dict(waves=waves, units=units, prod=prod.reshape(rows, 64, 2), blocks=blocks, diag_slot=diag, products=products)
+
+
+def chol_persist_plan(n32):
+    n = lib.psba_chol_persist_plan(int(n32), None, 0)
+    if n < 0:
+        raise PsbaError(n, "psba_chol_persist_plan failed")
+    out = (C.c_int * max(n, 1))()
+    lib.psba_chol_persist_plan(int(n32), out, n)
+    v, recs, i = list(out[:n]), [], 0
+    while i < n:
+        step, wg, nt = v[i], v[i + 1], v[i + 2]
+        i += 3
+        tiles = [(v[i + 2 * q], v[i + 2 * q + 1]) for q in range(nt)]
+        i += 2 * nt
+        nr = v[i]
+        reads = [(v[i + 1 + 2 * q], v[i + 2 + 2 * q]) for q in range(nr)]
+        i += 1 + 2 * nr
+        nw = v[i]
+        waits = [(v[i + 1 + 2 * q], v[i + 2 + 2 * q]) for q in range(nw)]
+        i += 1 + 2 * nw
+        ns = v[i]
+        signals = v[i + 1:i + 1 + ns]
+        i += 1 + ns
+        recs.append(dict(step=step, wg=wg, tiles=tiles, reads=reads, waits=waits, signals=signals))
+    return recs
 
 
 def chol_dist_exchange_plan(n32, NB, nranks, JE):
@@ -627,6 +654,11 @@
         keys = ("n32", "fused", "fused2", "blocked", "NB", "diag_only", "lookahead", "single")
         return {k: (int(v) if k in ("n32", "NB") else bool(v)) for k, v in zip(keys, out)}
 
+    def chol_persist_info(self):
+        out = (C.c_int * 4)()
+        self._ck(lib.psba_chol_persist_info(self._h, out))
+        return dict(legal=bool(out[0]), taken=bool(out[1]), fallbacks=int(out[2]), grid=int(out[3]))
+
     def chol_dist_begin(self):
         self._ck(lib.psba_chol_dist_begin(self._h))
 
diff --git a/psba_amd/csrc/kernels_backsub.hip b/psba_amd/csrc/kernels_backsub.hip
--- a/psba_amd/csrc/kernels_backsub.hip
+++ b/psba_amd/csrc/kernels_backsub.hip
@@ -34,6 +34,7 @@
     if (tid == 0) {
       p.scal[SC_STATUS_V] = (p.status[0] == p.status[3]) ? 1.0 : 0.0;
       p.scal[SC_STATUS_SPD] = (p.status[1] == p.status[3]) ? 1.0 : 0.0;
+      p.scal[SC_STATUS_PERSIST] = (p.status[4] == p.status[3]) ? 1.0 : 0.0;
     }
     for (int t = tid; t < p.nA; t += TILE_OBS) {
       const double d = p.dp[t], c = p.cams[t] + d;
diff --git a/psba_amd/csrc/kernels_chol_graph.hip b/psba_amd/csrc/kernels_chol_graph.hip
--- a/psba_amd/csrc/kernels_chol_graph.hip
+++ b/psba_amd/csrc/kernels_chol_graph.hip
@@ -40,39 +40,68 @@
   if (tim && tid == 0) tim[15] = (long long)__builtin_amdgcn_s_memtime();
 }
 
+struct Row8 {
+  double v[8];
+};
+__device__ __forceinline__ Row8 load_row8(const double *p) {
+  const double4 a = reinterpret_cast<const double4 *>(p)[0], b = reinterpret_cast<const double4 *>(p)[1];
+  return {{a.x, a.y, a.z, a.w, b.x, b.y, b.z, b.w}};
+}
+typedef unsigned int u32x4 __attribute__((ext_vector_type(4)));
+template <bool SC1>
+__device__ __forceinline__ double ldg(const double *p) {
+  if constexpr (SC1)
+    return __hip_atomic_load(p, __ATOMIC_RELAXED, __HIP_MEMORY_SCOPE_AGENT);
+  else
+    return *p;
+}
+template <bool SC1>
+__device__ __forceinline__ void stg(double *p, double v) {
+  if constexpr (SC1)
+    __hip_atomic_store(p, v, __ATOMIC_RELAXED, __HIP_MEMORY_SCOPE_AGENT);
+  else
+    *p = v;
+}
+template <bool SC1>
+__device__ __forceinline__ Row8 load_row8_g(const double *base, size_t off) {
+  if constexpr (SC1) {
+    const __amdgpu_buffer_rsrc_t rs = __builtin_amdgcn_make_buffer_rsrc(const_cast<double *>(base), 0, 0x7fffffff, 0x00020000);
+    const int o = (int)(off * sizeof(double));
+    constexpr int AUX_SC1 = 16;
+    const u32x4 q0 = __builtin_amdgcn_raw_buffer_load_b128(rs, o, 0, AUX_SC1);
+    const u32x4 q1 = __builtin_amdgcn_raw_buffer_load_b128(rs, o + 16, 0, AUX_SC1);
+    const u32x4 q2 = __builtin_amdgcn_raw_buffer_load_b128(rs, o + 32, 0, AUX_SC1);
+    const u32x4 q3 = __builtin_amdgcn_raw_buffer_load_b128(rs, o + 48, 0, AUX_SC1);
+    const double2 d0 = __builtin_bit_cast(double2, q0), d1 = __builtin_bit_cast(double2, q1);
+    const double2 d2 = __builtin_bit_cast(double2, q2), d3 = __builtin_bit_cast(double2, q3);
+    return {{d0.x, d0.y, d1.x, d1.y, d2.x, d2.y, d3.x, d3.y}};
+  } else {
+    return load_row8(base + off);
+  }
+}
+
+template <bool SC1 = false>
 __device__ __forceinline__ void trsm_tile(const double *Lw, int ld, int j, int T, int nT, const double *Li,
                                           int li, int lk, d4 &xl, d4 &xr) {
-  const double4 *b0p = reinterpret_cast<const double4 *>(Li + (size_t)li * GB + 8 * lk);
-  const double4 *b1p = reinterpret_cast<const double4 *>(Li + (size_t)(16 + li) * GB + 8 * lk);
-  const double4 p0 = b0p[0], p1 = b0p[1], q0 = b1p[0], q1 = b1p[1];
-  double4 a0, a1;
+  const Row8 p = load_row8_g<SC1>(Li, (size_t)li * GB + 8 * lk);
+  const Row8 q = load_row8_g<SC1>(Li, (size_t)(16 + li) * GB + 8 * lk);
+  Row8 a;
   const int e = T - nT;
   if (e >= j / 16) {
     const int k1 = 16 * (e - j / 16) + li - 8 * lk;
-    a0 = make_double4(k1 == 0, k1 == 1, k1 == 2, k1 == 3);
-    a1 = make_double4(k1 == 4, k1 == 5, k1 == 6, k1 == 7);
+#pragma unroll
+    for (int t = 0; t < 8; t++) a.v[t] = k1 == t;
   } else {
-    const double4 *ap = reinterpret_cast<const double4 *>(Lw + (size_t)(16 * T + li) * ld + j + 8 * lk);
-    a0 = ap[0];
-    a1 = ap[1];
+    a = load_row8_g<SC1>(Lw, (size_t)(16 * T + li) * ld + j + 8 * lk);
   }
   d4 x0 = {0, 0, 0, 0}, x1 = {0, 0, 0, 0}, y0 = {0, 0, 0, 0}, y1 = {0, 0, 0, 0};
-  x0 = __builtin_amdgcn_mfma_f64_16x16x4f64(a0.x, p0.x, x0, 0, 0, 0);
-  y0 = __builtin_amdgcn_mfma_f64_16x16x4f64(a0.x, q0.x, y0, 0, 0, 0);
-  x1 = __builtin_amdgcn_mfma_f64_16x16x4f64(a0.y, p0.y, x1, 0, 0, 0);
-  y1 = __builtin_amdgcn_mfma_f64_16x16x4f64(a0.y, q0.y, y1, 0, 0, 0);
-  x0 = __builtin_amdgcn_mfma_f64_16x16x4f64(a0.z, p0.z, x0, 0, 0, 0);
-  y0 = __builtin_amdgcn_mfma_f64_16x16x4f64(a0.z, q0.z, y0, 0, 0, 0);
-  x1 = __builtin_amdgcn_mfma_f64_16x16x4f64(a0.w, p0.w, x1, 0, 0, 0);
-  y1 = __builtin_amdgcn_mfma_f64_16x16x4f64(a0.w, q0.w, y1, 0, 0, 0);
-  x0 = __builtin_amdgcn_mfma_f64_16x16x4f64(a1.x, p1.x, x0, 0, 0, 0);
-  y0 = __builtin_amdgcn_mfma_f64_16x16x4f64(a1.x, q1.x, y0, 0, 0, 0);
-  x1 = __builtin_amdgcn_mfma_f64_16x16x4f64(a1.y, p1.y, x1, 0, 0, 0);
-  y1 = __builtin_amdgcn_mfma_f64_16x16x4f64(a1.y, q1.y, y1, 0, 0, 0);
-  x0 = __builtin_amdgcn_mfma_f64_16x16x4f64(a1.z, p1.z, x0, 0, 0, 0);
-  y0 = __builtin_amdgcn_mfma_f64_16x16x4f64(a1.z, q1.z, y0, 0, 0, 0);
-  x1 = __builtin_amdgcn_mfma_f64_16x16x4f64(a1.w, p1.w, x1, 0, 0, 0);
-  y1 = __builtin_amdgcn_mfma_f64_16x16x4f64(a1.w, q1.w, y1, 0, 0, 0);
+#pragma unroll
+  for (int t = 0; t < 8; t += 2) {
+    x0 = __builtin_amdgcn_mfma_f64_16x16x4f64(a.v[t], p.v[t], x0, 0, 0, 0);
+    y0 = __builtin_amdgcn_mfma_f64_16x16x4f64(a.v[t], q.v[t], y0, 0, 0, 0);
+    x1 = __builtin_amdgcn_mfma_f64_16x16x4f64(a.v[t + 1], p.v[t + 1], x1, 0, 0, 0);
+    y1 = __builtin_amdgcn_mfma_f64_16x16x4f64(a.v[t + 1], q.v[t + 1], y1, 0, 0, 0);
+  }
   xl = x0 + x1;
   xr = y0 + y1;
 }
@@ -97,13 +126,6 @@
   store_x_tile(Lx, ld, j, T, li, lk, xl, xr);
 }
 
-struct Row8 {
-  double v[8];
-};
-__device__ __forceinline__ Row8 load_row8(const double *p) {
-  const double4 a = reinterpret_cast<const double4 *>(p)[0], b = reinterpret_cast<const double4 *>(p)[1];
-  return {{a.x, a.y, a.z, a.w, b.x, b.y, b.z, b.w}};
-}
 __device__ __forceinline__ d4 update_mfma(d4 c0, const Row8 &a, const Row8 &b) {
   d4 c1 = {0, 0, 0, 0};
 #pragma unroll
@@ -113,17 +135,19 @@
   }
   return c0 + c1;
 }
+template <bool SC1 = false>
 __device__ __forceinline__ d4 load_c_tile(const double *Lw, int ld, int TR, int TC, int li, int lk) {
   d4 c;
 #pragma unroll
-  for (int r = 0; r < 4; r++) c[r] = Lw[(size_t)(16 * TR + lk + 4 * r) * ld + 16 * TC + li];
+  for (int r = 0; r < 4; r++) c[r] = ldg<SC1>(Lw + (size_t)(16 * TR + lk + 4 * r) * ld + 16 * TC + li);
   return c;
 }
+template <bool SC1 = false>
 __device__ __forceinline__ void store_c_tile(double *Lw, int ld, int TR, int TC, int li, int lk, const d4 &c) {
 #pragma unroll
-  for (int r = 0; r < 4; r++) Lw[(size_t)(16 * TR + lk + 4 * r) * ld + 16 * TC + li] = c[r];
-}
-__device__ __forceinline__ bool tile_of_index(long long idx, int T0, int nT, int nId, int &TR, int &TC,
+  for (int r = 0; r < 4; r++) stg<SC1>(Lw + (size_t)(16 * TR + lk + 4 * r) * ld + 16 * TC + li, c[r]);
+}
+__host__ __device__ inline bool tile_of_index(long long idx, int T0, int nT, int nId, int &TR, int &TC,
                                               bool &fresh) {
   const long long M = (nT - 1) - T0;
   const long long ntri = M * (M + 1) / 2;
@@ -155,6 +179,7 @@
   return update_mfma(load_c_tile(Lw, ld, TR, TC, li, lk), a, b);
 }
 
+template <bool SC1 = false>
 __device__ __forceinline__ void factor_next_block(Factor32Lds &s, double *Lx, int ld, int jn, double *linv,
                                             int *status, int tid, bool store_L = true) {
   factor32(s, tid);
@@ -162,7 +187,7 @@
   for (int t = tid; t < GB * GB; t += 256) {
     const int r = t / GB, c = t % GB;
     if (store_L) Lx[(size_t)(jn + r) * ld + jn + c] = f32_L(s, r, c);
-    lio[t] = f32_Linv(s, r, c);
+    stg<SC1>(lio + t, f32_Linv(s, r, c));
   }
   if (tid == 0 && s.fail) status[1] = status[3];
 }
@@ -430,6 +455,78 @@
 }
 
 constexpr int XS = 34;
+template <bool SC1>
+__device__ __forceinline__ void panel_wg0(Factor32Lds &s, double (&sX)[4][2][16][XS], double *Lw, double *Lx, int ld, int j,
+                                          int nId, double *linv, int *status, int factor_next, int tid) {
+  const int lane = tid & 63, wave = tid >> 6;
+  const int li = lane & 15, lk = lane >> 4;
+  const int T0 = (j + GB) / 16;
+  const double *Li = linv + (size_t)(j / GB) * GB * GB;
+  if (tid < 4) s.flag[tid] = 0;
+  if (tid == 4) s.fail = 0;
+  const int tr = (wave > 0), tc = (wave > 1);
+  d4 c = {0, 0, 0, 0};
+  if (wave < 3) c = load_c_tile<SC1>(Lw, ld, T0 + tr, T0 + tc, li, lk);
+  {
+    const int xr = wave >> 1, half = wave & 1;
+    const Row8 a = load_row8_g<SC1>(Lw, (size_t)(16 * (T0 + xr) + li) * ld + j + 8 * lk);
+    const Row8 b = load_row8_g<SC1>(Li, (size_t)(16 * half + li) * GB + 8 * lk);
+    d4 x0 = {0, 0, 0, 0}, x1 = {0, 0, 0, 0};
+#pragma unroll
+    for (int t = 0; t < 8; t += 2) {
+      x0 = __builtin_amdgcn_mfma_f64_16x16x4f64(a.v[t], b.v[t], x0, 0, 0, 0);
+      x1 = __builtin_amdgcn_mfma_f64_16x16x4f64(a.v[t + 1], b.v[t + 1], x1, 0, 0, 0);
+    }
+    const d4 x = x0 + x1;
+#pragma unroll
+    for (int r = 0; r < 4; r++) {
+      sX[0][xr][lk + 4 * r][16 * half + li] = x[r];
+      if (nId == 0) Lx[(size_t)(16 * (T0 + xr) + lk + 4 * r) * ld + j + 16 * half + li] = x[r];
+    }
+  }
+  __syncthreads();
+  if (wave < 3) {
+    const Row8 a = load_row8(&sX[0][tr][li][8 * lk]), b = load_row8(&sX[0][tc][li][8 * lk]);
+    c = update_mfma(c, a, b);
+    if (!factor_next) {
+      store_c_tile<SC1>(Lw, ld, T0 + tr, T0 + tc, li, lk, c);
+    } else {
+#pragma unroll
+      for (int r = 0; r < 4; r++) s.D[16 * tr + lk + 4 * r][16 * tc + li] = c[r];
+    }
+  }
+  if (!factor_next) return;
+  __syncthreads();
+  factor_next_block<SC1>(s, Lx, ld, j + GB, linv, status, tid, nId == 0);
+}
+
+template <bool SC1>
+__device__ __forceinline__ void panel_tile(double (&sX)[4][2][16][XS], double *Lw, double *Lx, int ld, int j, int nT, int nId,
+                                           int TR, int TC, bool fresh, const double *Li, int wave, int li, int lk) {
+  const int T0 = (j + GB) / 16;
+  d4 c = {0, 0, 0, 0};
+  if (!fresh) c = load_c_tile<SC1>(Lw, ld, TR, TC, li, lk);
+  d4 xl, xr;
+  trsm_tile<SC1>(Lw, ld, j, TR, nT, Li, li, lk, xl, xr);
+  if (TC == T0 && (nId == 0 || TR >= nT - 1)) store_x_tile(Lx, ld, j, TR, li, lk, xl, xr);
+#pragma unroll
+  for (int r = 0; r < 4; r++) {
+    sX[wave][0][lk + 4 * r][li] = xl[r];
+    sX[wave][0][lk + 4 * r][16 + li] = xr[r];
+  }
+  if (TC != TR) {
+    trsm_tile<SC1>(Lw, ld, j, TC, nT, Li, li, lk, xl, xr);
+#pragma unroll
+    for (int r = 0; r < 4; r++) {
+      sX[wave][1][lk + 4 * r][li] = xl[r];
+      sX[wave][1][lk + 4 * r][16 + li] = xr[r];
+    }
+  }
+  const Row8 a = load_row8(&sX[wave][0][li][8 * lk]);
+  const Row8 b = load_row8(&sX[wave][TC != TR][li][8 * lk]);
+  store_c_tile<SC1>(Lw, ld, TR, TC, li, lk, update_mfma(c, a, b));
+}
+
 __global__ __launch_bounds__(256) void k_cholg_panel(double *Lw, double *Lx, int ld, int j, int nT, int nId, int TE,
                                                      double *linv, int *status, int factor_next) {
   __shared__ Factor32Lds s;
@@ -439,42 +536,7 @@
   const int T0 = (j + GB) / 16;
   const double *Li = linv + (size_t)(j / GB) * GB * GB;
   if (blockIdx.x == 0) {
-    if (tid < 4) s.flag[tid] = 0;
-    if (tid == 4) s.fail = 0;
-    const int tr = (wave > 0), tc = (wave > 1);
-    d4 c = {0, 0, 0, 0};
-    if (wave < 3) c = load_c_tile(Lw, ld, T0 + tr, T0 + tc, li, lk);
-    {
-      const int xr = wave >> 1, half = wave & 1;
-      const Row8 a = load_row8(Lw + (size_t)(16 * (T0 + xr) + li) * ld + j + 8 * lk);
-      const Row8 b = load_row8(Li + (size_t)(16 * half + li) * GB + 8 * lk);
-      d4 x0 = {0, 0, 0, 0}, x1 = {0, 0, 0, 0};
-#pragma unroll
-      for (int t = 0; t < 8; t += 2) {
-        x0 = __builtin_amdgcn_mfma_f64_16x16x4f64(a.v[t], b.v[t], x0, 0, 0, 0);
-        x1 = __builtin_amdgcn_mfma_f64_16x16x4f64(a.v[t + 1], b.v[t + 1], x1, 0, 0, 0);
-      }
-      const d4 x = x0 + x1;
-#pragma unroll
-      for (int r = 0; r < 4; r++) {
-        sX[0][xr][lk + 4 * r][16 * half + li] = x[r];
-        if (nId == 0) Lx[(size_t)(16 * (T0 + xr) + lk + 4 * r) * ld + j + 16 * half + li] = x[r];
-      }
-    }
-    __syncthreads();
-    if (wave < 3) {
-      const Row8 a = load_row8(&sX[0][tr][li][8 * lk]), b = load_row8(&sX[0][tc][li][8 * lk]);
-      c = update_mfma(c, a, b);
-      if (!factor_next) {
-        store_c_tile(Lw, ld, T0 + tr, T0 + tc, li, lk, c);
-      } else {
-#pragma unroll
-        for (int r = 0; r < 4; r++) s.D[16 * tr + lk + 4 * r][16 * tc + li] = c[r];
-      }
-    }
-    if (!factor_next) return;
-    __syncthreads();
-    factor_next_block(s, Lx, ld, j + GB, linv, status, tid, nId == 0);
+    panel_wg0<false>(s, sX, Lw, Lx, ld, j, nId, linv, status, factor_next, tid);
     return;
   }
   int TR, TC;
@@ -492,27 +554,91 @@
   } else if (!tile_of_index((long long)(blockIdx.x - 1) * 4 + wave + 3, T0, nT, nId, TR, TC, fresh)) {
     return;
   }
-  d4 c = {0, 0, 0, 0};
-  if (!fresh) c = load_c_tile(Lw, ld, TR, TC, li, lk);
-  d4 xl, xr;
-  trsm_tile(Lw, ld, j, TR, nT, Li, li, lk, xl, xr);
-  if (TC == T0 && (nId == 0 || TR >= nT - 1)) store_x_tile(Lx, ld, j, TR, li, lk, xl, xr);
-#pragma unroll
-  for (int r = 0; r < 4; r++) {
-    sX[wave][0][lk + 4 * r][li] = xl[r];
-    sX[wave][0][lk + 4 * r][16 + li] = xr[r];
-  }
-  if (TC != TR) {
-    trsm_tile(Lw, ld, j, TC, nT, Li, li, lk, xl, xr);
-#pragma unroll
-    for (int r = 0; r < 4; r++) {
-      sX[wave][1][lk + 4 * r][li] = xl[r];
-      sX[wave][1][lk + 4 * r][16 + li] = xr[r];
-    }
-  }
-  const Row8 a = load_row8(&sX[wave][0][li][8 * lk]);
-  const Row8 b = load_row8(&sX[wave][TC != TR][li][8 * lk]);
-  store_c_tile(Lw, ld, TR, TC, li, lk, update_mfma(c, a, b));
+  panel_tile<false>(sX, Lw, Lx, ld, j, nT, nId, TR, TC, fresh, Li, wave, li, lk);
+}
+
+constexpr unsigned PERSIST_POISON = 0xffffffffu;
+constexpr int PERSIST_LINV = 0, PERSIST_ALL = 32, PERSIST_SEVEN = 64;
+constexpr long long PERSIST_GIVE_UP = 1000000;
+constexpr int PERSIST_TIM = 32, PERSIST_TIM_STEPS = 32;
+
+__host__ __device__ inline int persist_grid(int n32) {
+  const int nT = n32 / 16 + 1;
+  long long most = 0;
+  for (int j = 0; j + GB < n32; j += GB) {
+    const long long T0 = (j + GB) / 16, M = (nT - 1) - T0;
+    const long long tiles = M * (M + 1) / 2 + M + T0 * M;
+    if (tiles > most) most = tiles;
+  }
+  return 1 + (int)((most - 3 + 3) / 4);
+}
+__host__ __device__ inline int persist_n7(int grid) { return grid - 1 < 2 ? grid - 1 : 2; }
+
+__device__ __forceinline__ int persist_wait(unsigned *linv_word, unsigned need_linv, unsigned *cnt, unsigned need_cnt) {
+  const long long t0 = (long long)wall_clock64();
+  for (;;) {
+    const unsigned f = __hip_atomic_load(linv_word, __ATOMIC_RELAXED, __HIP_MEMORY_SCOPE_AGENT);
+    const unsigned c = __hip_atomic_load(cnt, __ATOMIC_RELAXED, __HIP_MEMORY_SCOPE_AGENT);
+    if (f == PERSIST_POISON) return 1;
+    if (f >= need_linv && c >= need_cnt) return 0;
+    if ((long long)wall_clock64() - t0 > PERSIST_GIVE_UP) return 2;
+    __builtin_amdgcn_s_sleep(2);
+  }
+}
+
+__global__ __launch_bounds__(256) void k_cholg_chain(double *Lw, double *Lx, int ld, int nT, int nsteps, double *linv,
+                                                     int *status, unsigned *sync, long long *tim) {
+  __shared__ Factor32Lds s;
+  __shared__ double sX[4][2][16][XS];
+  __shared__ int s_stop;
+  const int tid = threadIdx.x, lane = tid & 63, wave = tid >> 6;
+  const int li = lane & 15, lk = lane >> 4;
+  const int wg = blockIdx.x, grid = gridDim.x;
+  const unsigned n_all = (unsigned)(grid - 1), n7 = (unsigned)persist_n7(grid);
+  long long *stamp = tim && wg < 2 && tid == 0 ? tim + PERSIST_TIM : nullptr;
+  for (int k = 0; k < nsteps; k++) {
+    const int j = GB * k;
+    if (stamp && k < PERSIST_TIM_STEPS) stamp[(wg ? 2 : 0) * PERSIST_TIM_STEPS + k] = (long long)__builtin_amdgcn_s_memtime();
+    if (k > 0 && wave == 0) {
+      const int r = wg == 0 ? persist_wait(sync + PERSIST_LINV, 0, sync + PERSIST_SEVEN, n7 * (unsigned)k)
+                            : persist_wait(sync + PERSIST_LINV, (unsigned)k, sync + PERSIST_ALL, n_all * (unsigned)k);
+      __builtin_amdgcn_fence(__ATOMIC_ACQUIRE, "wavefront");
+      if (lane == 0) {
+        if (r == 2) {
+          __hip_atomic_store(status + 4, __hip_atomic_load(status + 3, __ATOMIC_RELAXED, __HIP_MEMORY_SCOPE_AGENT),
+                             __ATOMIC_RELAXED, __HIP_MEMORY_SCOPE_AGENT);
+          __hip_atomic_store(sync + PERSIST_LINV, PERSIST_POISON, __ATOMIC_RELAXED, __HIP_MEMORY_SCOPE_AGENT);
+        }
+        s_stop = r;
+      }
+    }
+    __syncthreads();
+    if (k > 0 && s_stop) return;
+    if (stamp && k < PERSIST_TIM_STEPS) stamp[(wg ? 3 : 1) * PERSIST_TIM_STEPS + k] = (long long)__builtin_amdgcn_s_memtime();
+    if (wg == 0) {
+      panel_wg0<true>(s, sX, Lw, Lx, ld, j, (j + GB) / 16, linv, status, 1, tid);
+      asm volatile("s_waitcnt vmcnt(0)" ::: "memory");
+      __syncthreads();
+      const int failed = s.fail;
+      if (tid == 0)
+        __hip_atomic_store(sync + PERSIST_LINV, failed ? PERSIST_POISON : (unsigned)(k + 1), __ATOMIC_RELAXED,
+                           __HIP_MEMORY_SCOPE_AGENT);
+      if (failed) return;
+    } else {
+      const int T0 = (j + GB) / 16;
+      int TR, TC;
+      bool fresh = false;
+      if (tile_of_index((long long)(wg - 1) * 4 + wave + 3, T0, nT, T0, TR, TC, fresh))
+        panel_tile<true>(sX, Lw, Lx, ld, j, nT, T0, TR, TC, fresh, linv + (size_t)k * GB * GB, wave, li, lk);
+      asm volatile("s_waitcnt vmcnt(0)" ::: "memory");
+      __syncthreads();
+      if (tid == 0) {
+        if (wg <= 2) __hip_atomic_fetch_add(sync + PERSIST_SEVEN, 1u, __ATOMIC_RELAXED, __HIP_MEMORY_SCOPE_AGENT);
+        __hip_atomic_fetch_add(sync + PERSIST_ALL, 1u, __ATOMIC_RELAXED, __HIP_MEMORY_SCOPE_AGENT);
+        if (stamp && k < PERSIST_TIM_STEPS) stamp[4 * PERSIST_TIM_STEPS + k] = (long long)__builtin_amdgcn_s_memtime();
+      }
+    }
+  }
 }
 
 template <int NBK>
@@ -832,9 +958,10 @@
 
 template <int NZ>
 __global__ __launch_bounds__(256) void k_cholg_solve(const double *Lw, const double *Lx, int ld, int n, int n32,
-                                                    double *x, const double *linv, int *status) {
+                                                    double *x, const double *linv, int *status, unsigned *sync) {
   __shared__ double sLi[GB][GB + 1], sV[GB], sW[GB];
   const int tid = threadIdx.x, lane = tid & 63, i = blockIdx.x * 4 + (tid >> 6);
+  if (sync && blockIdx.x == 0 && tid < 3) sync[32 * tid] = 0;
   const int jl = n32 - GB;
   const double *Li = linv + (size_t)(jl / GB) * GB * GB;
   stage_block32(sLi, Li, GB, tid);
@@ -1238,6 +1365,101 @@
     buf[t] = *at;
 }
 
+constexpr int PERSIST_LDS_RESERVE = 64 * 1024;
+constexpr int PERSIST_MAX_N32 = 672;
+constexpr bool PERSIST_DEFAULT_ON = false;
+
+static bool persist_legal(psba_ctx *h) {
+  const ChainShape c = chain_shape(h);
+  const int n32 = h->n32;
+  if (!c.fused || n32 < 2 * GB || n32 > PERSIST_MAX_N32 || h->comm || !h->chol_sync) return false;
+  if (h->persist_cus < 0) {
+    h->persist_cus = 0;
+    int per_cu = 0, dev = 0;
+    hipDeviceProp_t prop;
+    if (hipFuncSetAttribute((const void *)k_cholg_chain, hipFuncAttributeMaxDynamicSharedMemorySize, PERSIST_LDS_RESERVE) == hipSuccess &&
+        hipOccupancyMaxActiveBlocksPerMultiprocessor(&per_cu, k_cholg_chain, 256, PERSIST_LDS_RESERVE) == hipSuccess && per_cu >= 1 &&
+        hipGetDevice(&dev) == hipSuccess && hipGetDeviceProperties(&prop, dev) == hipSuccess)
+      h->persist_cus = prop.multiProcessorCount;
+  }
+  long long max_grid = h->persist_cus;
+  if (const char *e = getenv("PSBA_CHOL_PERSIST_MAX_GRID")) max_grid = atoll(e) < max_grid ? atoll(e) : max_grid;
+  return persist_grid(n32) <= max_grid;
+}
+static bool persist_route(psba_ctx *h) {
+  if (!persist_legal(h) || h->persist_latched_off) return false;
+  if (const char *e = getenv("PSBA_CHOL_PERSIST")) return atoi(e) != 0;
+  return PERSIST_DEFAULT_ON;
+}
+int chol_persist_info(psba_ctx *h, int *out) {
+  out[0] = persist_legal(h);
+  out[1] = h->persist_taken;
+  out[2] = h->persist_fallbacks;
+  out[3] = h->n32 >= 2 * GB && h->n32 <= 1024 ? persist_grid(h->n32) : 0;
+  return PSBA_OK;
+}
+void chol_persist_gave_up(psba_ctx *h) {
+  h->persist_latched_off = true;
+  h->persist_fallbacks++;
+}
+
+int chol_persist_plan(int n32, int *out, int cap) {
+  if (n32 < 2 * GB || n32 % GB || n32 > 1024) return 0;
+  const int nT = n32 / 16 + 1, grid = persist_grid(n32), nsteps = n32 / GB - 1;
+  long long n = 0;
+  auto put = [&](int v) {
+    if (n < cap) out[n] = v;
+    n++;
+  };
+  for (int k = 0; k < nsteps; k++) {
+    const int T0 = (GB * k + GB) / 16;
+    for (int wg = 0; wg < grid; wg++) {
+      put(k);
+      put(wg);
+      if (wg == 0) {
+        put(3);
+        put(T0); put(T0); put(T0 + 1); put(T0); put(T0 + 1); put(T0 + 1);
+        if (k > 0) {
+          put(7);
+          put(T0); put(T0); put(T0 + 1); put(T0); put(T0 + 1); put(T0 + 1);
+          put(T0); put(T0 - 2); put(T0); put(T0 - 1); put(T0 + 1); put(T0 - 2); put(T0 + 1); put(T0 - 1);
+          put(1);
+          put(2); put(persist_n7(grid) * k);
+        } else {
+          put(0);
+          put(0);
+        }
+        put(1);
+        put(0);
+      } else {
+        int cnt = 0, t[4][2];
+        for (int wave = 0; wave < 4; wave++) {
+          int TR, TC;
+          bool fresh;
+          if (tile_of_index((long long)(wg - 1) * 4 + wave + 3, T0, nT, T0, TR, TC, fresh)) {
+            t[cnt][0] = TR;
+            t[cnt++][1] = TC;
+          }
+        }
+        put(cnt);
+        for (int q = 0; q < cnt; q++) { put(t[q][0]); put(t[q][1]); }
+        put(0);
+        if (k > 0) {
+          put(2);
+          put(0); put(k);
+          put(1); put((grid - 1) * k);
+        } else {
+          put(0);
+        }
+        put(wg <= 2 ? 2 : 1);
+        put(1);
+        if (wg <= 2) put(2);
+      }
+    }
+  }
+  return n > 0x7fffffff ? -1 : (int)n;
+}
+
 static void enqueue_chain(psba_ctx *h, hipStream_t s, bool skip_diag) {
   const int n32 = h->n32, ld = h->n32, nT = n32 / 16 + 1;
   double *Lw = h->red, *Lx = h->chol_L, *linv = h->chol_ws;
@@ -1248,6 +1470,8 @@
   if (const char *e = getenv("PSBA_CHOL_TAIL")) tail = fused && atoi(e) >= 0 && atoi(e) <= TAIL_MAX && atoi(e) <= n32 / GB ? atoi(e) : 0;
 #endif
   const int jl = n32 - GB * tail;
+  const bool persist = tail == 0 && persist_route(h);
+  h->persist_taken = persist;
   if (!skip_diag && !(tail > 0 && jl == 0))
     hipLaunchKernelGGL(k_cholg_diag, dim3(1), dim3(256), 0, s, Lw, Lx, ld, 0, linv, h->status, h->chol_tim);
   bool look = chain_lookahead(c);
@@ -1283,7 +1507,11 @@
     }
     if (far_prev) (void)hipStreamWaitEvent(s, far_prev, 0);
   }
-  for (int j = 0; !blocked && j < n32; j += GB) {
+  if (persist) {
+    hipLaunchKernelGGL(k_cholg_chain, dim3(persist_grid(n32)), dim3(256), PERSIST_LDS_RESERVE, s, Lw, Lx, ld, nT, n32 / GB - 1,
+                       linv, h->status, h->chol_sync, h->chol_tim);
+  }
+  for (int j = 0; !blocked && !persist && j < n32; j += GB) {
     const bool last = j + GB >= n32;
     const int T0 = (j + GB) / 16;
     const long long M = (nT - 1) - T0;
@@ -1323,10 +1551,10 @@
   if (fused) {
     if (n32 <= 640)
       hipLaunchKernelGGL(k_cholg_solve<10>, dim3((h->d.nA + 3) / 4), dim3(256), 0, s, Lw, Lx, ld, h->d.nA, n32, h->dp,
-                         linv, h->status);
+                         linv, h->status, persist ? h->chol_sync : nullptr);
     else
       hipLaunchKernelGGL(k_cholg_solve<16>, dim3((h->d.nA + 3) / 4), dim3(256), 0, s, Lw, Lx, ld, h->d.nA, n32, h->dp,
-                         linv, h->status);
+                         linv, h->status, persist ? h->chol_sync : nullptr);
   } else {
     enqueue_backward(h, s);
   }
@@ -1452,7 +1680,8 @@
     PSBA_HIP(h, hipGetLastError());
     return PSBA_OK;
   }
-  if (!h->chol_graph[v] || h->chol_graph_n32[v] != h->n32 || h->chol_graph_red[v] != h->red) {
+  const bool persist_now = persist_route(h);
+  if (!h->chol_graph[v] || h->chol_graph_n32[v] != h->n32 || h->chol_graph_red[v] != h->red || h->chol_graph_persist[v] != persist_now) {
     if (h->chol_graph[v]) {
       (void)hipGraphExecDestroy(h->chol_graph[v]);
       h->chol_graph[v] = nullptr;
@@ -1469,6 +1698,7 @@
     }
     h->chol_graph_n32[v] = h->n32;
     h->chol_graph_red[v] = h->red;
+    h->chol_graph_persist[v] = persist_now;
   }
   {
     ProfScope ps(h, PSBA_K_CHOLESKY);
diff --git a/psba_amd/csrc/kernels_freek.hip b/psba_amd/csrc/kernels_freek.hip
--- a/psba_amd/csrc/kernels_freek.hip
+++ b/psba_amd/csrc/kernels_freek.hip
@@ -194,6 +194,7 @@
   if (blockIdx.x == 0 && threadIdx.x == 0) {
     p.scal[SC_STATUS_V] = (p.status[0] == p.status[3]) ? 1.0 : 0.0;
     p.scal[SC_STATUS_SPD] = (p.status[1] == p.status[3]) ? 1.0 : 0.0;
+    p.scal[SC_STATUS_PERSIST] = (p.status[4] == p.status[3]) ? 1.0 : 0.0;
   }
   for (int t = blockIdx.x * blockDim.x + threadIdx.x; t < p.nA; t += gridDim.x * blockDim.x) {
     const double d = p.dp[t], c = p.cams[t] + d;
diff --git a/psba_amd/csrc/lm_loop.cpp b/psba_amd/csrc/lm_loop.cpp
--- a/psba_amd/csrc/lm_loop.cpp
+++ b/psba_amd/csrc/lm_loop.cpp
@@ -67,6 +67,10 @@
       LM_TRY(psba_backsub_async(h, mu));
       if (itno + 1 < opts->max_iter) LM_TRY(psba_linearize_ahead(h));
       LM_TRY(psba_backsub_wait(h, &sc));
+      if (sc.status & PSBA_CHOL_REDO) {
+        tries--;
+        continue;
+      }
       if (!(sc.status & PSBA_NOT_SPD)) {
         dp_L2 = sc.dp_l2;
         if (dp_L2 < p_L2 * STOP * STOP) {
diff --git a/psba_amd/csrc/psba_api.cpp b/psba_amd/csrc/psba_api.cpp
--- a/psba_amd/csrc/psba_api.cpp
+++ b/psba_amd/csrc/psba_api.cpp
@@ -173,6 +173,7 @@
   dev_free(h->trv[1]);
   dev_free(h->jmul_out);
   dev_free(h->chol_ws);
+  dev_free(h->chol_sync);
   dev_free(h->dist_buf);
   dev_free(h->chol_L);
   dev_free(h->dbg_ex);
@@ -526,7 +527,12 @@
   TRY(dev_alloc(h, &h->chol_ws, (size_t)((d.nA + 31) / 32) * 1024));
   TRY(dev_alloc(h, &h->chol_L, dense));
   PSBA_HIP(h, hipMemsetAsync(h->chol_L, 0, sizeof(double) * dense, h->stream));
-  if (getenv("PSBA_CHOL_TIMING") && !h->chol_tim) TRY(dev_alloc(h, &h->chol_tim, 32));
+  if (getenv("PSBA_CHOL_TIMING") && !h->chol_tim) TRY(dev_alloc(h, &h->chol_tim, 192));
+  if (!h->chol_sync) {
+    PSBA_HIP(h, hipMalloc((void **)&h->chol_sync, sizeof(unsigned) * 96));
+    PSBA_HIP(h, hipMemsetAsync(h->chol_sync, 0, sizeof(unsigned) * 96, h->stream));
+    PSBA_HIP(h, hipStreamSynchronize(h->stream));
+  }
   if (sparse) {
     OwnerPlanHost op;
     std::vector<unsigned char> pat;
@@ -913,12 +919,19 @@
   }
   TRY(launch_chol_solve(h));
   if (h->chol_tim) {
-    long long t[32];
+    long long t[192];
     PSBA_HIP(h, hipMemcpyAsync(t, h->chol_tim, sizeof t, hipMemcpyDeviceToHost, h->stream));
     PSBA_HIP(h, hipStreamSynchronize(h->stream));
     fprintf(stderr, "chol stamps (cycles since the first):");
     for (int k = 1; k < 32; k++) fprintf(stderr, " %lld", t[k] ? t[k] - t[0] : 0);
     fprintf(stderr, "\n");
+    if (h->persist_taken) {
+      const long long *b0 = t + 32, *g0 = t + 64, *b1 = t + 96, *g1 = t + 128, *p1 = t + 160;
+      const int ns = h->n32 / 32 - 1 < 32 ? h->n32 / 32 - 1 : 32;
+      fprintf(stderr, "persistent chain, %d steps, shader clocks: step | wg0 begin (since its first), wait | wg1 wait, turn-around\n", ns);
+      for (int k = 0; k < ns; k++)
+        fprintf(stderr, "  %2d | %6lld %5lld | %5lld %5lld\n", k, b0[k] - b0[0], g0[k] - b0[k], g1[k] - b1[k], p1[k] - g1[k]);
+    }
   }
   h->assembled = false;
   h->solved = true;
@@ -1004,9 +1017,11 @@
   }
   const int st0 = h->h_scal[SC_STATUS_V] > 0.0 ? h->try_id : 0;
   const int st1 = h->h_scal[SC_STATUS_SPD] > 0.0 ? h->try_id : 0;
+  const bool redo = !h->comm && h->h_scal[SC_STATUS_PERSIST] > 0.0;
+  if (redo) chol_persist_gave_up(h);
   h->backsubbed = true;
   if (out) {
-    out->status = (st1 == h->try_id ? PSBA_NOT_SPD : 0) | (st0 == h->try_id ? PSBA_SINGULAR_V : 0);
+    out->status = (st1 == h->try_id ? PSBA_NOT_SPD : 0) | (st0 == h->try_id ? PSBA_SINGULAR_V : 0) | (redo ? PSBA_CHOL_REDO : 0);
     out->dp_l2 = h->h_scal[SC_DP_L2];
     out->gain_den = h->h_scal[SC_GAIN_DEN];
     out->new_cost = h->h_scal[SC_NEW_COST];
@@ -1054,6 +1069,16 @@
   NEED(h, h->uploaded, "no problem uploaded");
   if (!out8) return fail(h, PSBA_E_INVALID, "psba_chol_shape: null pointer");
   return chol_shape(h, out8);
+}
+int psba_chol_persist_info(psba_handle h, int *out4) {
+  CHECK_H(h);
+  NEED(h, h->uploaded, "no problem uploaded");
+  if (!out4) return fail(h, PSBA_E_INVALID, "psba_chol_persist_info: null pointer");
+  return chol_persist_info(h, out4);
+}
+int psba_chol_persist_plan(int n32, int *out, int cap) {
+  if (cap > 0 && !out) return PSBA_E_INVALID;
+  return psba::chol_persist_plan(n32, out, cap);
 }
 int psba_chol_dist_exchange_plan(int n32, int NB, int nranks, int JE, long long *out4, int cap) {
   if (!out4 || cap <= 0) return PSBA_E_INVALID;
@@ -1433,6 +1458,10 @@
   h->solved = true;
   TRY(fetch_scalars(h));
   TRY(d2h(h, dpa, h->dp, sizeof(double) * (size_t)h->d.nA));
+  if (h->h_status[4] == h->try_id) {
+    chol_persist_gave_up(h);
+    return PSBA_CHOL_REDO;
+  }
   return h->h_status[1] == h->try_id ? PSBA_NOT_SPD : PSBA_OK;
 }
 
diff --git a/psba_amd/csrc/psba_internal.h b/psba_amd/csrc/psba_internal.h
--- a/psba_amd/csrc/psba_internal.h
+++ b/psba_amd/csrc/psba_internal.h
@@ -26,6 +26,7 @@
   SC_PART = 16,
   SC_STATUS_V = 80,
   SC_STATUS_SPD = 81,
+  SC_STATUS_PERSIST = 82,
   SC_TR_DOTS = 84,
   SC_CHOLMOD = 88,
   SC_SUMS = 96,
@@ -239,6 +240,11 @@
   hipGraphExec_t chol_graph[2] = {nullptr, nullptr};
   int chol_graph_n32[2] = {0, 0};
   double *chol_graph_red[2] = {nullptr, nullptr};
+  bool chol_graph_persist[2] = {false, false};
+  unsigned *chol_sync = nullptr;
+  int persist_cus = -1;
+  bool persist_taken = false, persist_latched_off = false;
+  int persist_fallbacks = 0;
   long long *chol_tim = nullptr;
   double *chol_L = nullptr;
   double *dist_buf = nullptr;
@@ -317,6 +323,9 @@
 int launch_chol_graph(psba_ctx *h);
 int chol_dist_shape(psba_ctx *h, int *NB, int *blocked);
 int chol_shape(psba_ctx *h, int *out8);
+int chol_persist_info(psba_ctx *h, int *out4);
+int chol_persist_plan(int n32, int *out, int cap);
+void chol_persist_gave_up(psba_ctx *h);
 int chol_dist_exchange_plan(int n32, int NB, int nranks, int JE, long long (*out)[4], int cap);
 int chol_dist_begin(psba_ctx *h);
 int chol_dist_superpanel(psba_ctx *h, int J);
diff --git a/psba_amd/csrc/tr_loop.cpp b/psba_amd/csrc/tr_loop.cpp
--- a/psba_amd/csrc/tr_loop.cpp
+++ b/psba_amd/csrc/tr_loop.cpp
@@ -123,6 +123,7 @@
       TR_TRY(psba_schur_reduce(h));
       TR_TRY(psba_schur_solve(h));
       TR_TRY(psba_backsub(h, lambda, &sc));
+      if (sc.status & PSBA_CHOL_REDO) continue;
       if (sc.status & PSBA_NOT_SPD) {
         chol_fail++;
         if (lambda == 0.0) {
```

Measured after the change: 2090 M-obs/s. 1.0% lower.
